# chaeyeongyun/VQ_SEG

Measured on AMD Instinct MI355X. Metric: train images/sec @512x512 vqreptunet1x1 K=512, higher is better.
Workload: dtype bf16; 1 GPU; CPS training iteration (2 x vqreptunet1x1, ResNet-50 encoder, K=[0,0,512,512,512], v1 recipe: 6 forwards + 4 backwards + 2 Adam steps) on 512x512x3 images -- BASELINE configs[2] (the metric's configuration): vqreptunet1x1 512x512, K = 512; labelled_per_gpu=32, unlabelled_per_gpu=32, parallelism=dp1, collectives=none (one process), conv_dtype=bf16

## Files before the change

### include/vqseg.h

```cpp
#ifndef VQSEG_H
#define VQSEG_H

#include <stddef.h>
#include <stdint.h>

#ifdef __cplusplus
extern "C" {
#endif

#define VQSEG_ABI_VERSION 1

#define VQSEG_EINVAL  (-1)
#define VQSEG_ENOSPC  (-2)
#define VQSEG_ENODEV  (-3)

int         vqseg_abi_version(void);
const char* vqseg_last_error(void);
const char* vqseg_kernel_name(const char* entry_point);

int vqseg_set_option(const char* key, int value);

int vqseg_profile_begin(int capacity);
int vqseg_profile_collect(int max_records, int64_t* n_rows_host, int* channels_host,
                          int* n_codes_host, float* ms_host,
                          int* kind_host );

int vqseg_conv_profile_begin(int capacity);
int vqseg_conv_profile_collect(int max_records, double* flops_host, int* kind_host, float* ms_host,
                               int* shape_host );

size_t vqseg_vq_workspace_bytes(int64_t n_rows, int channels, int n_codes);
int vqseg_vq_forward_f32(const float* x, const float* codebook, const void* prepared,
                         int64_t n_rows, int channels, int n_codes, int training,
                         float commitment_weight, float* quant, int64_t* idx, float* loss,
                         float* dead_pct, float* dmin, void* workspace, size_t workspace_bytes,
                         void* stream);

int vqseg_vq_forward_group(int n_levels, int bf16, const void* const* x, const float* const* codebook,
                           const void* const* prepared, const int64_t* n_rows, const int* channels, const int* n_codes,
                           int training, const float* commitment_weight, void* const* quant, int64_t* const* idx,
                           float* const* loss, float* const* dead_pct, void* const* workspace,
                           const size_t* workspace_bytes, void* stream);

size_t vqseg_vq_filter_counter_offset(int64_t n_rows, int channels, int n_codes);

int vqseg_vq_tiles_per_wave(int n_levels, const int64_t* n_rows_host, const int* n_codes_host);

int vqseg_vq_assign_f32(const float* x, const float* codebook, const void* prepared,
                        int64_t n_rows, int channels, int n_codes, int64_t* idx, float* dmin,
                        void* workspace, size_t workspace_bytes, void* stream);
int vqseg_vq_assign_bf16(const void* x, const float* codebook, const void* prepared,
                         int64_t n_rows, int channels, int n_codes, int64_t* idx, float* dmin,
                         void* workspace, size_t workspace_bytes, void* stream);

size_t vqseg_vq_prepared_bytes(int channels, int n_codes);
int vqseg_vq_prepare_f32(const float* codebook, int channels, int n_codes, void* prepared,
                         size_t prepared_bytes, void* stream);

int vqseg_vq_backward_f32(const float* grad_quant, const float* grad_loss, const float* x,
                          const float* quant, int64_t n_rows, int channels,
                          float commitment_weight, float* grad_x, void* stream);

int vqseg_vq_forward_bf16(const void* x, const float* codebook, const void* prepared, int64_t n_rows, int channels,
                          int n_codes, int training, float commitment_weight, void* quant, int64_t* idx, float* loss,
                          float* dead_pct, float* dmin, void* workspace, size_t workspace_bytes, void* stream);
int vqseg_vq_backward_bf16(const void* grad_quant, const float* grad_loss, const void* x, const int64_t* idx,
                           const float* codebook, int64_t n_rows, int channels, float commitment_weight,
                           void* grad_x, void* stream);

size_t vqseg_kmeans_workspace_bytes(int64_t n_rows, int channels, int n_codes);
int vqseg_kmeans_f32(const float* samples, float* means, int64_t* bins, int64_t n_rows,
                     int channels, int n_codes, int iters, void* workspace,
                     size_t workspace_bytes, void* stream);
int vqseg_kmeans_accumulate_f32(const float* samples, const float* means, int64_t n_rows,
                                int channels, int n_codes, float* sums, int64_t* counts,
                                void* workspace, size_t workspace_bytes, void* stream);
int vqseg_kmeans_finalize_f32(const float* sums, const int64_t* counts, float* means,
                              int channels, int n_codes, void* stream);


int vqseg_vq_code_sums(int bf16, const void* x, const int64_t* idx, int64_t n_rows, int channels, int n_codes,
                       float* sums, int64_t* counts, void* workspace, size_t workspace_bytes, void* stream);
int vqseg_vq_ema_update_f32(float* cluster_size, float* embed_avg, float* codebook, const float* sums,
                            const int64_t* counts, int channels, int n_codes, float decay, float eps, float* scratch,
                            void* stream);
int vqseg_vq_revive_candidates(int bf16, const void* x, int64_t n_rows, int channels, int n_codes, uint64_t seed,
                               const int64_t* counter, int rank, int world, float* cand, float* ok, void* stream);
int vqseg_vq_ema_update_revive_f32(float* cluster_size, float* embed_avg, float* codebook, const float* sums,
                                   const int64_t* counts, int channels, int n_codes, float decay, float eps, float* scratch,
                                   const float* cand, const float* ok, float threshold, int64_t* counter, int64_t* revived,
                                   void* stream);


size_t vqseg_conv_packed_elems(int cout, int cin, int kh, int kw, int transpose_flip);
int vqseg_conv_pack_weights_f32(const float* w, int cout, int cin, int kh, int kw, int transpose_flip,
                                void* hi, void* lo, void* stream);

int64_t vqseg_conv_stat_slots(int64_t m_rows, int cout);
int vqseg_conv2d_f(const void* x, const void* x2, int c1, const void* w_hi, const void* w_lo, void* y,
                   float* stat_partial, int n, int h, int w, int cin, int cout, int kh, int kw, int stride,
                   int pad, int reflect, int up, int ho, int wo, int precise, void* stream);

int vqseg_conv2d_affine_f(const void* x, const void* x2, int c1, const void* w_hi, const void* w_lo,
                          const float* scale, const float* shift, const void* res, int relu, void* y,
                          int n, int h, int w, int cin, int cout, int kh, int kw, int stride, int pad, int reflect,
                          int ho, int wo, int precise, void* stream);
int vqseg_conv2d_affine_bits_f(const void* x, const void* w_hi, const float* scale, const float* shift, const void* res,
                               const unsigned char* res_bits, void* y, int n, int h, int w, int cin, int cout, int kh, int kw,
                               int pad, int ho, int wo, void* stream);

size_t vqseg_conv2d_wgrad_workspace_bytes(int n, int h, int w, int cin, int ho, int wo, int cout, int kh, int kw);
int vqseg_conv2d_wgrad_f(const void* gy, const void* x, const void* x2, int c1, int n, int h, int w, int cin,
                         int ho, int wo, int cout, int kh, int kw, int stride, int pad, int reflect, int precise,
                         int cin_out, int im2col, int accumulate, void* workspace, size_t workspace_bytes, float* gw,
                         void* stream);
int vqseg_conv2d_wgrad2_f(const void* gy, const void* x, const void* x2, int n, const void* gy_b, const void* x_b, const void* x2_b,
                          int n_b, int c1, int h, int w, int cin, int ho, int wo, int cout, int kh, int kw, int stride, int pad,
                          int reflect, int precise, int cin_out, int im2col, int accumulate, void* workspace, size_t workspace_bytes,
                          float* gw, void* stream);

int vqseg_bn_sync_ints(int c);
int vqseg_bn_finalize_f(float* partial, int64_t m_rows, int c, const float* gamma, const float* beta,
                        float* run_mean, float* run_var, float momentum, float eps, int training,
                        float* scale, float* shift, float* save_mean, float* save_invstd,
                        int64_t* num_batches_tracked , int* sync, void* stream);
int vqseg_bn_apply_f(int bf16, const void* y, const void* res, const float* scale, const float* shift,
                     int64_t m_rows, int c, int relu, void* out, void* stream);
size_t vqseg_bn_backward_workspace_floats(int64_t m_rows, int c);
int vqseg_bn_backward_f(int bf16, const void* g_out, const void* out, const void* y, const float* mean,
                        const float* invstd, const float* gamma, const float* fwd_scale, const float* fwd_shift,
                        int64_t m_rows, int c, int relu, int training, int accumulate,
                        float* workspace, float* dgamma, float* dbeta, void* g_y, void* g_res, int* sync, void* stream);
int vqseg_bn_apply_bits_f(const void* y, const void* res, const float* scale, const float* shift, int64_t m_rows, int c,
                          void* out, unsigned char* bits, void* stream);
int vqseg_bn_backward_bits_f(const void* g_out, const unsigned char* bits, const void* y, const float* mean,
                             const float* invstd, const float* gamma, int64_t m_rows, int c, int training, int accumulate,
                             float* workspace, float* dgamma, float* dbeta, void* g_y, void* g_res, int* sync, void* stream);

int vqseg_maxpool3x3s2_f(int bf16, int backward, const void* x, const void* g, int n, int h, int w, int c,
                         void* out, unsigned char* idx, void* stream);

int vqseg_bilinear_f(int bf16, int backward, const void* src, int n, int h, int w, int c, int ho, int wo,
                     int align_corners, void* dst, void* stream);

int vqseg_head1x1_forward_f(int bf16, const void* x, const float* w, int64_t m_rows, int cin, int cout,
                            float* y, void* stream);
size_t vqseg_head1x1_backward_workspace_floats(int64_t m_rows, int cin, int cout);
int vqseg_head1x1_backward_f(int bf16, const void* x, const float* w, const float* g, int64_t m_rows, int cin,
                             int cout, void* gx, float* gw, float* workspace, void* stream);
int vqseg_head1x1_backward_add_f(int bf16, const void* x, const float* w, const float* g, int64_t m_rows, int cin,
                                 int cout, void* gx, float* gw, float* workspace, const void* gx_add, void* stream);
int vqseg_maxpool3x3s2_backward_add_f(int bf16, const void* g, const unsigned char* idx, const void* gx_add, int n, int h, int w,
                                      int c, void* gx, void* stream);

int vqseg_im2col_f(int out_bf16, const float* x, int n, int h, int w, int cin, int kh, int kw, int stride,
                   int pad, int reflect, int ho, int wo, int kp, void* out, void* stream);
int vqseg_reflect_fold_f(int bf16, const void* gp, int n, int h, int w, int c, void* gx, void* stream);
int vqseg_stem7_conv_f(int s3, const float* x, const void* w_img, void* y, float* stat_partial, const float* scale, const float* shift, int relu,
                       int n, int h, int w, int reflect, void* stream);
int vqseg_reflect_ring_f(const void* gy, const void* t_hi, void* ring, void* gx, int n, int h, int w, int cgy, int cgx, void* stream);

int vqseg_conv_pack_weights_s3_f32(const float* w, int cout, int cin, int c1, int kh, int kw, void* out, void* stream);

int vqseg_conv_pack_all_f32(const float* w, int cout, int cin, int k, int c1, void* fwd, void* tr, void* s3, void* stream);
size_t vqseg_conv_packed_s2_elems(int cout, int cin, int k);
int vqseg_conv_pack_weights_s2_f32(const float* w, int cout, int cin, int k, void* hi, void* lo, void* stream);
int vqseg_conv2d_dgrad_s2_f(const void* gy, const void* w_hi, const void* w_lo, void* gx, int n, int ho, int wo, int cout, int cin,
                            int k, int oh, int ow, int precise, int accumulate, void* stream);
int64_t vqseg_conv2d_dgrad_s2_fold_rows(int n, int h, int w, int reflect);
int vqseg_conv2d_dgrad_s2_fold_f(const void* gy, const void* w_hi, void* gx, int n, int ho, int wo, int cout, int cin, int h, int w,
                                 int reflect, void* stream);
int vqseg_s3_split_f(const float* x, int64_t rows, int channels, void* y, void* stream);
int vqseg_s3_merge_f(const void* x, int64_t rows, int channels, float* y, void* stream);
int vqseg_s3_maxpool3x3s2_f(const void* x, int n, int h, int w, int c, void* y, void* stream);
int vqseg_s3_bilinear_f(const void* x, int n, int h, int w, int c, int ho, int wo, int align_corners, void* y, void* stream);
int vqseg_cast_f(int to_bf16, const void* x, int64_t n, void* y, void* stream);

size_t vqseg_proto_loss_workspace_bytes(int64_t m_rows, int c, int k);
int vqseg_proto_loss_forward_f(int bf16, const void* x, const float* proto, const int64_t* labels,
                               const unsigned char* keep, const float* conf, int64_t m_rows, int c, int k,
                               int variant, float scale, float margin, int easy_margin,
                               void* workspace, size_t workspace_bytes, double* loss, void* stream);
int vqseg_proto_loss_backward_f(int bf16, const void* x, const float* proto, const int64_t* labels,
                                const unsigned char* keep, const float* conf, int64_t m_rows, int c, int k,
                                int variant, float scale, float margin, int easy_margin, const float* g_loss,
                                void* gx, float* gproto, void* workspace, size_t workspace_bytes, void* stream);

size_t vqseg_dice_workspace_bytes(int b, int c, int64_t hw);
int vqseg_dice_sums_forward_f(const float* logits, int64_t stride_b, int64_t stride_c, int64_t stride_px,
                              const int64_t* target, int b, int c, int64_t hw, int64_t ignore_index,
                              void* workspace, size_t workspace_bytes, float* inter, float* sets, void* stream);
int vqseg_dice_sums_backward_f(const float* logits, int64_t stride_b, int64_t stride_c, int64_t stride_px,
                               const int64_t* target, int b, int c, int64_t hw, int64_t ignore_index,
                               const float* g_inter, const float* g_sets, float* g_logits, void* stream);

int vqseg_dice_ce_sums_forward_f(const float* logits, int64_t stride_b, int64_t stride_c, int64_t stride_px,
                                 const int64_t* target, int b, int c, int64_t hw, int64_t ignore_index,
                                 void* workspace, size_t workspace_bytes, float* inter, float* sets, float* ce,
                                 void* stream);
int vqseg_dice_ce_sums_backward_f(const float* logits, int64_t stride_b, int64_t stride_c, int64_t stride_px,
                                  const int64_t* target, int b, int c, int64_t hw, int64_t ignore_index,
                                  const float* g_inter, const float* g_sets, const float* g_ce, float* g_logits,
                                  void* stream);

int vqseg_softmax_stats_f(const float* logits, int64_t stride_b, int64_t stride_c, int64_t stride_px, int b, int c,
                          int64_t hw, int64_t* label, float* entropy, float* top, void* stream);
// ... 79 lines not shown
```

### vq_seg_amd/_hip.py

```python
from __future__ import annotations

import ctypes
import os
from ctypes import c_char_p, c_double, c_float, c_int, c_int64, c_size_t, c_void_p
from typing import Optional, Tuple

import numpy as np
import torch

_HERE = os.path.dirname(os.path.abspath(__file__))
LIB_PATH = os.environ.get("VQSEG_LIB") or os.path.join(_HERE, "libvqseg_hip.so")

SYMBOLS = {
    "vqseg_abi_version": (c_int, []),
    "vqseg_last_error": (c_char_p, []),
    "vqseg_kernel_name": (c_char_p, [c_char_p]),
    "vqseg_set_option": (c_int, [c_char_p, c_int]),
    "vqseg_profile_begin": (c_int, [c_int]),
    "vqseg_profile_collect": (c_int, [c_int, c_void_p, c_void_p, c_void_p, c_void_p, c_void_p]),
    "vqseg_conv_profile_begin": (c_int, [c_int]),
    "vqseg_conv_profile_collect": (c_int, [c_int, c_void_p, c_void_p, c_void_p, c_void_p]),
    "vqseg_vq_workspace_bytes": (c_size_t, [c_int64, c_int, c_int]),
    "vqseg_vq_filter_counter_offset": (c_size_t, [c_int64, c_int, c_int]),
    "vqseg_vq_tiles_per_wave": (c_int, [c_int, c_void_p, c_void_p]),
    "vqseg_vq_forward_f32": (c_int, [c_void_p, c_void_p, c_void_p, c_int64, c_int, c_int, c_int, c_float, c_void_p,
                                     c_void_p, c_void_p, c_void_p, c_void_p, c_void_p, c_size_t, c_void_p]),
    "vqseg_vq_forward_bf16": (c_int, [c_void_p, c_void_p, c_void_p, c_int64, c_int, c_int, c_int, c_float, c_void_p,
                                      c_void_p, c_void_p, c_void_p, c_void_p, c_void_p, c_size_t, c_void_p]),
    "vqseg_vq_forward_group": (c_int, [c_int, c_int] + [c_void_p] * 6 + [c_int, c_void_p] + [c_void_p] * 6 + [c_void_p]),
    "vqseg_vq_backward_bf16": (c_int, [c_void_p, c_void_p, c_void_p, c_void_p, c_void_p, c_int64, c_int, c_float, c_void_p, c_void_p]),
    "vqseg_vq_assign_f32": (c_int, [c_void_p, c_void_p, c_void_p, c_int64, c_int, c_int, c_void_p, c_void_p, c_void_p,
                                    c_size_t, c_void_p]),
    "vqseg_vq_assign_bf16": (c_int, [c_void_p, c_void_p, c_void_p, c_int64, c_int, c_int, c_void_p, c_void_p, c_void_p,
                                     c_size_t, c_void_p]),
    "vqseg_vq_prepared_bytes": (c_size_t, [c_int, c_int]),
    "vqseg_vq_prepare_f32": (c_int, [c_void_p, c_int, c_int, c_void_p, c_size_t, c_void_p]),
    "vqseg_vq_backward_f32": (c_int, [c_void_p, c_void_p, c_void_p, c_void_p, c_int64, c_int, c_float, c_void_p,
                                      c_void_p]),
    "vqseg_kmeans_workspace_bytes": (c_size_t, [c_int64, c_int, c_int]),
    "vqseg_kmeans_f32": (c_int, [c_void_p, c_void_p, c_void_p, c_int64, c_int, c_int, c_int, c_void_p, c_size_t,
                                 c_void_p]),
    "vqseg_kmeans_accumulate_f32": (c_int, [c_void_p, c_void_p, c_int64, c_int, c_int, c_void_p, c_void_p, c_void_p,
                                            c_size_t, c_void_p]),
    "vqseg_kmeans_finalize_f32": (c_int, [c_void_p, c_void_p, c_void_p, c_int, c_int, c_void_p]),
    "vqseg_vq_code_sums": (c_int, [c_int, c_void_p, c_void_p, c_int64, c_int, c_int, c_void_p, c_void_p, c_void_p, c_size_t, c_void_p]),
    "vqseg_vq_ema_update_f32": (c_int, [c_void_p, c_void_p, c_void_p, c_void_p, c_void_p, c_int, c_int, c_float, c_float, c_void_p,
                                        c_void_p]),
    "vqseg_vq_revive_candidates": (c_int, [c_int, c_void_p, c_int64, c_int, c_int, ctypes.c_uint64, c_void_p, c_int, c_int, c_void_p, c_void_p,
                                           c_void_p]),
    "vqseg_vq_ema_update_revive_f32": (c_int, [c_void_p, c_void_p, c_void_p, c_void_p, c_void_p, c_int, c_int, c_float, c_float, c_void_p,
                                               c_void_p, c_void_p, c_float, c_void_p, c_void_p, c_void_p]),
    "vqseg_conv_packed_elems": (c_size_t, [c_int] * 5),
    "vqseg_conv_pack_weights_f32": (c_int, [c_void_p] + [c_int] * 5 + [c_void_p, c_void_p, c_void_p]),
    "vqseg_conv_stat_slots": (c_int64, [c_int64, c_int]),
    "vqseg_conv2d_f": (c_int, [c_void_p, c_void_p, c_int, c_void_p, c_void_p, c_void_p, c_void_p] + [c_int] * 14 + [c_void_p]),
    "vqseg_conv2d_affine_f": (c_int, [c_void_p, c_void_p, c_int, c_void_p, c_void_p, c_void_p, c_void_p, c_void_p, c_int, c_void_p] +
                              [c_int] * 13 + [c_void_p]),
    "vqseg_conv2d_wgrad_workspace_bytes": (c_size_t, [c_int] * 9),
    "vqseg_conv2d_wgrad_f": (c_int, [c_void_p, c_void_p, c_void_p] + [c_int] * 17 + [c_void_p, c_size_t, c_void_p, c_void_p]),
    "vqseg_conv2d_wgrad2_f": (c_int, [c_void_p, c_void_p, c_void_p, c_int, c_void_p, c_void_p, c_void_p, c_int] + [c_int] * 16 +
                              [c_void_p, c_size_t, c_void_p, c_void_p]),
    "vqseg_bn_sync_ints": (c_int, [c_int]),
    "vqseg_bn_finalize_f": (c_int, [c_void_p, c_int64, c_int, c_void_p, c_void_p, c_void_p, c_void_p, c_float, c_float, c_int,
                                   c_void_p, c_void_p, c_void_p, c_void_p, c_void_p, c_void_p, c_void_p]),
    "vqseg_bn_apply_f": (c_int, [c_int, c_void_p, c_void_p, c_void_p, c_void_p, c_int64, c_int, c_int, c_void_p, c_void_p]),
    "vqseg_bn_backward_workspace_floats": (c_size_t, [c_int64, c_int]),
    "vqseg_bn_backward_f": (c_int, [c_int] + [c_void_p] * 8 + [c_int64, c_int, c_int, c_int, c_int] + [c_void_p] * 7),
    "vqseg_conv2d_affine_bits_f": (c_int, [c_void_p] * 7 + [c_int] * 10 + [c_void_p]),
    "vqseg_bn_apply_bits_f": (c_int, [c_void_p] * 4 + [c_int64, c_int, c_void_p, c_void_p, c_void_p]),
    "vqseg_bn_backward_bits_f": (c_int, [c_void_p] * 6 + [c_int64, c_int, c_int, c_int] + [c_void_p] * 7),
    "vqseg_maxpool3x3s2_f": (c_int, [c_int, c_int, c_void_p, c_void_p, c_int, c_int, c_int, c_int, c_void_p, c_void_p, c_void_p]),
    "vqseg_bilinear_f": (c_int, [c_int, c_int, c_void_p] + [c_int] * 7 + [c_void_p, c_void_p]),
    "vqseg_head1x1_forward_f": (c_int, [c_int, c_void_p, c_void_p, c_int64, c_int, c_int, c_void_p, c_void_p]),
    "vqseg_head1x1_backward_workspace_floats": (c_size_t, [c_int64, c_int, c_int]),
    "vqseg_head1x1_backward_f": (c_int, [c_int, c_void_p, c_void_p, c_void_p, c_int64, c_int, c_int, c_void_p, c_void_p,
                                        c_void_p, c_void_p]),
    "vqseg_proto_loss_workspace_bytes": (c_size_t, [c_int64, c_int, c_int]),
    "vqseg_proto_loss_forward_f": (c_int, [c_int, c_void_p, c_void_p, c_void_p, c_void_p, c_void_p, c_int64, c_int, c_int, c_int,
                                           c_float, c_float, c_int, c_void_p, c_size_t, c_void_p, c_void_p]),
    "vqseg_proto_loss_backward_f": (c_int, [c_int, c_void_p, c_void_p, c_void_p, c_void_p, c_void_p, c_int64, c_int, c_int, c_int,
                                            c_float, c_float, c_int, c_void_p, c_void_p, c_void_p, c_void_p, c_size_t, c_void_p]),
    "vqseg_dice_workspace_bytes": (c_size_t, [c_int, c_int, c_int64]),
    "vqseg_dice_sums_forward_f": (c_int, [c_void_p, c_int64, c_int64, c_int64, c_void_p, c_int, c_int, c_int64, c_int64, c_void_p, c_size_t,
                                          c_void_p, c_void_p, c_void_p]),
    "vqseg_dice_sums_backward_f": (c_int, [c_void_p, c_int64, c_int64, c_int64, c_void_p, c_int, c_int, c_int64, c_int64, c_void_p,
                                           c_void_p, c_void_p, c_void_p]),
    "vqseg_dice_ce_sums_forward_f": (c_int, [c_void_p, c_int64, c_int64, c_int64, c_void_p, c_int, c_int, c_int64, c_int64, c_void_p,
                                             c_size_t, c_void_p, c_void_p, c_void_p, c_void_p]),
    "vqseg_dice_ce_sums_backward_f": (c_int, [c_void_p, c_int64, c_int64, c_int64, c_void_p, c_int, c_int, c_int64, c_int64, c_void_p,
                                              c_void_p, c_void_p, c_void_p, c_void_p]),
    "vqseg_focal_workspace_bytes": (c_size_t, [c_int, c_int64]),
    "vqseg_focal_forward_f": (c_int, [c_void_p, c_int64, c_int64, c_int64, c_void_p, c_int, c_int, c_int64, c_int64, c_void_p, c_float, c_float,
                                      c_int, c_void_p, c_size_t, c_void_p, c_void_p, c_void_p, c_void_p]),
    "vqseg_focal_backward_f": (c_int, [c_void_p, c_int64, c_int64, c_int64, c_void_p, c_int, c_int, c_int64, c_int64, c_void_p, c_float, c_float,
                                       c_int, c_void_p, c_float, c_void_p, c_void_p, c_void_p]),
    "vqseg_wce_sums_forward_f": (c_int, [c_void_p, c_int64, c_int64, c_int64, c_void_p, c_int, c_int, c_int64, c_int64, c_void_p, c_void_p,
                                         c_size_t, c_void_p, c_void_p]),
    "vqseg_wce_sums_backward_f": (c_int, [c_void_p, c_int64, c_int64, c_int64, c_void_p, c_int, c_int, c_int64, c_int64, c_void_p, c_void_p,
                                          c_void_p, c_void_p]),
    "vqseg_class_weight_f": (c_int, [c_void_p, c_int64, c_int, c_void_p, c_void_p, c_void_p]),
    "vqseg_softmax_stats_f": (c_int, [c_void_p, c_int64, c_int64, c_int64, c_int, c_int, c_int64, c_void_p, c_void_p, c_void_p, c_void_p]),
    "vqseg_confusion_counts_f": (c_int, [c_void_p, c_int64, c_int64, c_int64, c_void_p, c_int, c_int, c_int64, c_void_p, c_void_p]),
    "vqseg_order_stats_workspace_bytes": (c_size_t, []),
    "vqseg_order_stats_f": (c_int, [c_void_p, c_int64, c_int64, c_void_p, c_size_t, c_void_p, c_void_p]),
    "vqseg_im2col_f": (c_int, [c_int, c_void_p] + [c_int] * 12 + [c_void_p, c_void_p]),
    "vqseg_reflect_fold_f": (c_int, [c_int, c_void_p, c_int, c_int, c_int, c_int, c_void_p, c_void_p]),
    "vqseg_reflect_ring_f": (c_int, [c_void_p, c_void_p, c_void_p, c_void_p, c_int, c_int, c_int, c_int, c_int, c_void_p]),
    "vqseg_cast_f": (c_int, [c_int, c_void_p, c_int64, c_void_p, c_void_p]),
    "vqseg_conv_pack_all_f32": (c_int, [c_void_p, c_int, c_int, c_int, c_int, c_void_p, c_void_p, c_void_p, c_void_p]),
    "vqseg_conv_packed_s2_elems": (c_size_t, [c_int, c_int, c_int]),
    "vqseg_conv_pack_weights_s2_f32": (c_int, [c_void_p, c_int, c_int, c_int, c_void_p, c_void_p, c_void_p]),
    "vqseg_conv2d_dgrad_s2_f": (c_int, [c_void_p, c_void_p, c_void_p, c_void_p] + [c_int] * 10 + [c_void_p]),
    "vqseg_stem7_conv_f": (c_int, [c_int, c_void_p, c_void_p, c_void_p, c_void_p, c_void_p, c_void_p] + [c_int] * 5 + [c_void_p]),
    "vqseg_conv2d_dgrad_s2_fold_rows": (ctypes.c_int64, [c_int] * 4),
    "vqseg_cps_loss_combine_f": (c_int, [c_int, c_int, c_int, c_void_p, c_void_p, c_void_p, c_void_p, c_float, c_float, c_float, c_void_p, c_int, c_int,
                                         c_float, c_void_p, c_int, c_float, c_void_p, c_void_p, c_void_p, c_void_p, c_void_p]),
    "vqseg_conv2d_dgrad_s2_fold_f": (c_int, [c_void_p, c_void_p, c_void_p] + [c_int] * 8 + [c_void_p]),
    "vqseg_head1x1_backward_add_f": (c_int, [c_int, c_void_p, c_void_p, c_void_p, c_int64, c_int, c_int, c_void_p, c_void_p,
                                            c_void_p, c_void_p, c_void_p]),
    "vqseg_maxpool3x3s2_backward_add_f": (c_int, [c_int, c_void_p, c_void_p, c_void_p, c_int, c_int, c_int, c_int, c_void_p, c_void_p]),
    "vqseg_conv_pack_weights_s3_f32": (c_int, [c_void_p] + [c_int] * 5 + [c_void_p, c_void_p]),
    "vqseg_s3_split_f": (c_int, [c_void_p, c_int64, c_int, c_void_p, c_void_p]),
    "vqseg_s3_merge_f": (c_int, [c_void_p, c_int64, c_int, c_void_p, c_void_p]),
    "vqseg_s3_maxpool3x3s2_f": (c_int, [c_void_p, c_int, c_int, c_int, c_int, c_void_p, c_void_p]),
    "vqseg_s3_bilinear_f": (c_int, [c_void_p] + [c_int] * 7 + [c_void_p, c_void_p]),
    "vqseg_adam_work_items": (c_int64, [c_int64, c_int, c_int, c_int]),
    "vqseg_adam_step_f32": (c_int, [c_void_p, c_void_p, c_int, c_double, c_double, c_double, c_double, c_int64, c_void_p]),
    "vqseg_adam_ema_step_f32": (c_int, [c_void_p, c_void_p, c_void_p, c_int, c_double, c_double, c_double, c_double, c_int64, c_double, c_int,
                                        c_void_p]),
    "vqseg_batch_u8_f": (c_int, [c_int, c_void_p, c_void_p, c_void_p, c_void_p] + [c_int] * 4 + [c_void_p] * 6),
    "vqseg_box_mix_f": (c_int, [c_int, c_int, c_void_p, c_void_p] + [c_int] * 4 + [c_int64] * 3 + [c_void_p, ctypes.c_uint64, c_void_p]),
    "vqseg_affine_warp_f": (c_int, [c_int, c_int, c_void_p, c_void_p] + [c_int] * 4 + [c_int64] * 4 + [c_void_p, ctypes.c_uint64, c_void_p]),
    "vqseg_resize_argmax_f": (c_int, [c_void_p, c_void_p, c_int] + [c_int64] * 3 + [c_int] * 6 + [c_void_p] * 5),
}

_lib: Optional[ctypes.CDLL] = None


class HipLibraryError(RuntimeError):
    pass


def _bind_symbols(handle: ctypes.CDLL) -> ctypes.CDLL:
    for name, (res, args) in SYMBOLS.items():
        fn = getattr(handle, name)
        fn.restype, fn.argtypes = res, args
    return handle


def lib() -> ctypes.CDLL:
    global _lib
    if _lib is None:
        if not os.path.exists(LIB_PATH):
            raise HipLibraryError(
                f"{LIB_PATH} not found: build it with `python -c 'import __graft_entry__ as g; g.build()'` "
                f"(or `make -C vq_seg_amd/csrc`). There is no CPU fallback.")
        handle = _bind_symbols(ctypes.CDLL(LIB_PATH))
        if handle.vqseg_abi_version() != 1:
            raise HipLibraryError("libvqseg_hip.so ABI version mismatch")
        for kv in filter(None, os.environ.get("VQSEG_OPTS", "").split(",")):
            key, _, val = kv.partition("=")
            if key.strip().startswith("py_"):
                PY_OPTS[key.strip()] = int(val)
                continue
            if handle.vqseg_set_option(key.strip().encode(), int(val)) < 0:
                raise HipLibraryError(f"VQSEG_OPTS: unknown option {key!r}")
        _lib = handle
    return _lib


PY_OPTS: dict = {}
FILTER_DIAG = None


_BF_DTYPE = {0: torch.float32, 1: torch.bfloat16, 2: torch.bfloat16}


def tptr(t, name: str, dtype=None, numel: Optional[int] = None, bf: Optional[int] = None, at_least: bool = False, dense: bool = True):
    if t is None:
        return None
    if bf is not None:
        dtype = _BF_DTYPE[bf]
    try:
        if (dtype is None or t.dtype is dtype or (type(dtype) is tuple and t.dtype in dtype)) and t.is_cuda and \
                (numel is None or (t.numel() >= numel if at_least else t.numel() == numel)) and \
                (not dense or t.is_contiguous() or (t.dim() == 4 and t.is_contiguous(memory_format=torch.channels_last))):
            return t.data_ptr()
    except AttributeError:
        pass
    return _tptr_report(t, name, dtype, numel, at_least, dense)


def _tptr_report(t, name, dtype, numel, at_least, dense):
    def bad(msg):
        return HipLibraryError(f"{name}: {msg}")
    if not isinstance(t, torch.Tensor):
        raise bad(f"expected a tensor, got {type(t).__name__}")
    if dtype is not None and (t.dtype not in dtype if isinstance(dtype, tuple) else t.dtype != dtype):
        if dense:
            raise bad(f"expected {dtype}, got {t.dtype}")
        names = " or ".join(str(d).removeprefix("torch.") for d in (dtype if isinstance(dtype, tuple) else (dtype,)))
        raise bad(f"expected a {names} tensor, got {t.dtype}")
    if dense and not t.is_contiguous() and not (t.dim() == 4 and t.is_contiguous(memory_format=torch.channels_last)):
        raise bad(f"expected a dense (contiguous) tensor, got strides {tuple(t.stride())} for shape {tuple(t.shape)}")
    if numel is not None and (t.numel() < numel if at_least else t.numel() != numel):
        raise bad(f"the sizes passed along need {'at least ' if at_least else ''}{numel} elements, the tensor has {t.numel()} (shape {tuple(t.shape)})")
    if not t.is_cuda:
        return _NotOnGpu(f"{name}: the HIP path needs a tensor on a 'cuda' (ROCm) device; got {t.device}. There is no CPU fallback.")
    return t.data_ptr()


class _NotOnGpu:
    __slots__ = ("msg",)

    def __init__(self, msg: str):
        self.msg = msg

    def __add__(self, _offset):
        return self


def on_gpu(ptr):
    if type(ptr) is _NotOnGpu:
        raise HipLibraryError(ptr.msg)
    return ptr


def _dev(t: torch.Tensor, dtype: torch.dtype, name: str, numel: Optional[int] = None):
    if t is None:
        raise HipLibraryError(f"{name}: expected a tensor, got None")
    return tptr(t, name, dtype=dtype, numel=numel)


def _stream() -> int:
    return torch.cuda.current_stream().cuda_stream


def _failed(L, name: str, rc: int) -> HipLibraryError:
    return HipLibraryError(f"{name} failed (code {rc}): {L.vqseg_last_error().decode(errors='replace')}")


def launch(name: str, dev, *args, handle=None) -> None:
    L = handle or lib()
    if type(dev) is not torch.device:
        dev = torch.device(dev)
    if dev.type == "cuda":
        try:
            with torch.cuda.device(dev):
                rc = getattr(L, name)(*args, _stream())
        except ctypes.ArgumentError:
            for a in args:
                on_gpu(a)
            raise
        if rc != 0:
            raise _failed(L, name, rc)
        return
    for a in args:
        on_gpu(a)
    raise HipLibraryError(f"{name}: the HIP path needs tensors on a 'cuda' (ROCm) device; got {dev}. There is no CPU fallback.")


def _workspace(nbytes: int, device) -> torch.Tensor:
    return torch.empty(int(nbytes), dtype=torch.uint8, device=device)


def vq_prepare(codebook: torch.Tensor) -> torch.Tensor:
    L = lib()
    k, c = codebook.shape
    wp = _dev(codebook, torch.float32, "codebook")
    nbytes = L.vqseg_vq_prepared_bytes(c, k)
    blob = _workspace(nbytes, codebook.device)
    launch("vqseg_vq_prepare_f32", codebook.device, wp, c, k, blob.data_ptr(), nbytes)
    return blob


def vq_forward(rows: torch.Tensor, codebook: torch.Tensor, training: bool, commitment_weight: float,
               want_dmin: bool = False, prepared: Optional[torch.Tensor] = None):
    L = lib()
    n, c = rows.shape
    k = codebook.shape[0]
    bf16 = rows.dtype == torch.bfloat16
    xp, wp = tptr(rows, "rows", bf=int(bf16), numel=n * c), _dev(codebook, torch.float32, "codebook", k * c)
    dev = rows.device
    quant = torch.empty_like(rows)
    idx = torch.empty(n, dtype=torch.int64, device=dev)
    scal = torch.empty(2, dtype=torch.float32, device=dev)
    dmin = torch.empty(n, dtype=torch.float32, device=dev) if want_dmin else None
    nbytes = L.vqseg_vq_workspace_bytes(n, c, k)
    ws = _workspace(nbytes, dev)
    launch("vqseg_vq_forward_bf16" if bf16 else "vqseg_vq_forward_f32", dev, xp, wp,
           tptr(prepared, "prepared codebook", dtype=torch.uint8, numel=L.vqseg_vq_prepared_bytes(c, k)), n, c, k,
           int(bool(training)), float(commitment_weight), quant.data_ptr(), idx.data_ptr(), scal.data_ptr(), scal.data_ptr() + 4,
           dmin.data_ptr() if want_dmin else None, ws.data_ptr(), nbytes)
    out = (quant, idx, scal[0:1], scal[1])
    return out + (dmin,) if want_dmin else out


def bind(path: str) -> ctypes.CDLL:
    return _bind_symbols(ctypes.CDLL(path))


def vq_forward_group(rows_list, codebooks, prepared_list, training: bool, commitment_weights, handle=None):
    L = handle or lib()
    nl = len(rows_list)
    bf16 = rows_list[0].dtype == torch.bfloat16
    dev = rows_list[0].device
    ptr = lambda ps: (c_void_p * nl)(*map(on_gpu, ps))
    ns = np.array([r.shape[0] for r in rows_list], dtype=np.int64)
    cs = np.array([r.shape[1] for r in rows_list], dtype=np.int32)
    ks = np.array([w.shape[0] for w in codebooks], dtype=np.int32)
    cw = np.array([float(w) for w in commitment_weights], dtype=np.float32)
    xs, wps, preps, quants, idxs, scals, wss = [], [], [], [], [], [], []
    for r, w in zip(rows_list, codebooks):
        if r.dtype != rows_list[0].dtype:
            raise HipLibraryError("vq_forward_group: one row type per call")
        xs.append(tptr(r, "rows", bf=int(bf16)))
        wps.append(_dev(w, torch.float32, "codebook", w.shape[0] * r.shape[1]))
        quants.append(torch.empty_like(r))
        idxs.append(torch.empty(r.shape[0], dtype=torch.int64, device=dev))
        scals.append(torch.empty(2, dtype=torch.float32, device=dev))
        wss.append(_workspace(L.vqseg_vq_workspace_bytes(r.shape[0], r.shape[1], w.shape[0]), dev))
    for w, p_ in zip(codebooks, prepared_list):
        preps.append(tptr(p_, "prepared codebook", dtype=torch.uint8, numel=L.vqseg_vq_prepared_bytes(w.shape[1], w.shape[0])))
    wsb = (c_size_t * nl)(*[w.numel() for w in wss])
    launch("vqseg_vq_forward_group", dev, nl, int(bf16), ptr(xs), ptr(wps), ptr(preps), ns.ctypes.data, cs.ctypes.data, ks.ctypes.data,
           int(bool(training)), cw.ctypes.data, ptr(q.data_ptr() for q in quants), ptr(i.data_ptr() for i in idxs),
           ptr(s.data_ptr() for s in scals), ptr(s.data_ptr() + 4 for s in scals), ptr(w.data_ptr() for w in wss),
           ctypes.cast(wsb, c_void_p), handle=handle)
    if FILTER_DIAG is not None and bf16:
        for r, w, ws_ in zip(rows_list, codebooks, wss):
            off = L.vqseg_vq_filter_counter_offset(r.shape[0], r.shape[1], w.shape[0])
            FILTER_DIAG.append((r.shape[0], r.shape[1], w.shape[0], ws_[off:off + 256].view(torch.int32) if off else None))
    return [(q, i, s[0:1], s[1]) for q, i, s in zip(quants, idxs, scals)]


def set_option(key: str, value: int) -> int:
    prev = lib().vqseg_set_option(key.encode(), int(value))
    if prev < 0:
        raise HipLibraryError(f"vqseg_set_option: unknown option {key!r} or bad value {value}")
    return prev


def vq_tiles_per_wave(n_rows, n_codes) -> int:
    rows = [n_rows] if isinstance(n_rows, int) else list(n_rows)
    codes = [n_codes] if isinstance(n_codes, int) else list(n_codes)
    if len(rows) != len(codes):
        raise ValueError("vq_tiles_per_wave: one code count per row count")
    t = lib().vqseg_vq_tiles_per_wave(len(rows), (ctypes.c_int64 * len(rows))(*rows), (c_int * len(codes))(*codes))
    if t < 0:
        raise _failed(lib(), "vqseg_vq_tiles_per_wave", t)
    return t


def vq_assign(rows: torch.Tensor, codebook: torch.Tensor, want_dmin: bool = False,
              prepared: Optional[torch.Tensor] = None, want_filter_count: bool = False):
    L = lib()
    n, c = rows.shape
    k = codebook.shape[0]
    bf16 = rows.dtype == torch.bfloat16
    xp, wp = tptr(rows, "rows", bf=int(bf16), numel=n * c), _dev(codebook, torch.float32, "codebook", k * c)
    dev = rows.device
    idx = torch.empty(n, dtype=torch.int64, device=dev)
    dmin = torch.empty(n, dtype=torch.float32, device=dev) if want_dmin else None
    nbytes = L.vqseg_vq_workspace_bytes(n, c, k)
    ws = _workspace(nbytes, dev)
    launch("vqseg_vq_assign_bf16" if bf16 else "vqseg_vq_assign_f32", dev, xp, wp,
           tptr(prepared, "prepared codebook", dtype=torch.uint8, numel=L.vqseg_vq_prepared_bytes(c, k)), n, c, k,
           idx.data_ptr(), dmin.data_ptr() if want_dmin else None, ws.data_ptr(), nbytes)
    if want_filter_count:
        off = L.vqseg_vq_filter_counter_offset(n, c, k) if bf16 else 0
        amb = ws[off:off + 256].view(torch.int32).sum() if off else None
        return (idx, dmin, amb) if want_dmin else (idx, amb)
    return (idx, dmin) if want_dmin else idx


def vq_backward(grad_quant: torch.Tensor, grad_loss: Optional[torch.Tensor], rows: torch.Tensor, quant: torch.Tensor,
                commitment_weight: float) -> torch.Tensor:
    n, c = rows.shape
    gq = _dev(grad_quant, torch.float32, "grad_quant", n * c)
    gl = _dev(grad_loss, torch.float32, "grad_loss", 1) if grad_loss is not None else None
    gx = torch.empty_like(rows)
    launch("vqseg_vq_backward_f32", rows.device, gq, gl, _dev(rows, torch.float32, "rows", n * c), _dev(quant, torch.float32, "quant", n * c),
           n, c, float(commitment_weight), gx.data_ptr())
    return gx


def vq_backward_bf16(grad_quant: torch.Tensor, grad_loss: Optional[torch.Tensor], rows: torch.Tensor, idx: torch.Tensor,
                     codebook: torch.Tensor, commitment_weight: float) -> torch.Tensor:
    n, c = rows.shape
    gq = _dev(grad_quant, torch.bfloat16, "grad_quant", n * c)
    gl = _dev(grad_loss, torch.float32, "grad_loss", 1) if grad_loss is not None else None
    gx = torch.empty_like(rows)
    if codebook.dim() != 2 or codebook.shape[1] != c:
        raise HipLibraryError(f"codebook: expected (K, {c}), got {tuple(codebook.shape)}")
    launch("vqseg_vq_backward_bf16", rows.device, gq, gl, _dev(rows, torch.bfloat16, "rows", n * c), _dev(idx, torch.int64, "idx", n),
           _dev(codebook, torch.float32, "codebook"), n, c, float(commitment_weight), gx.data_ptr())
    return gx


def kmeans(samples: torch.Tensor, means: torch.Tensor, iters: int) -> Tuple[torch.Tensor, torch.Tensor]:
    L = lib()
    n, c = samples.shape
    k = means.shape[0]
    sp, mp = _dev(samples, torch.float32, "samples", n * c), _dev(means, torch.float32, "means", k * c)
    bins = torch.zeros(k, dtype=torch.int64, device=samples.device)
    nbytes = L.vqseg_kmeans_workspace_bytes(n, c, k)
    ws = _workspace(nbytes, samples.device)
    launch("vqseg_kmeans_f32", samples.device, sp, mp, bins.data_ptr(), n, c, k, int(iters), ws.data_ptr(), nbytes)
    return means, bins


def kmeans_accumulate(samples: torch.Tensor, means: torch.Tensor) -> Tuple[torch.Tensor, torch.Tensor]:
    L = lib()
    n, c = samples.shape
    k = means.shape[0]
    sp, mp = _dev(samples, torch.float32, "samples", n * c), _dev(means, torch.float32, "means", k * c)
    sums = torch.empty(k, c, dtype=torch.float32, device=samples.device)
    counts = torch.empty(k, dtype=torch.int64, device=samples.device)
    nbytes = L.vqseg_kmeans_workspace_bytes(n, c, k)
    ws = _workspace(nbytes, samples.device)
    launch("vqseg_kmeans_accumulate_f32", samples.device, sp, mp, n, c, k, sums.data_ptr(), counts.data_ptr(), ws.data_ptr(), nbytes)
    return sums, counts


def kmeans_finalize(sums: torch.Tensor, counts: torch.Tensor, means: torch.Tensor) -> torch.Tensor:
    k, c = means.shape
    launch("vqseg_kmeans_finalize_f32", means.device, _dev(sums, torch.float32, "sums", k * c), _dev(counts, torch.int64, "counts", k),
           _dev(means, torch.float32, "means", k * c), c, k)
    return means


def vq_code_sums(rows: torch.Tensor, idx: torch.Tensor, k: int, out: Optional[torch.Tensor] = None) -> Tuple[torch.Tensor, torch.Tensor]:
    L = lib()
    n, c = rows.shape
    if rows.dtype not in (torch.float32, torch.bfloat16):
        raise HipLibraryError(f"rows: expected torch.float32 or torch.bfloat16, got {rows.dtype}")
    ip = _dev(idx, torch.int64, "idx", n)
    sums = torch.empty(k, c, dtype=torch.float32, device=rows.device) if out is None else out
    counts = torch.empty(k, dtype=torch.int64, device=rows.device)
    nbytes = L.vqseg_kmeans_workspace_bytes(n, c, k)
    ws = _workspace(nbytes, rows.device)
    bf = int(rows.dtype == torch.bfloat16)
    launch("vqseg_vq_code_sums", rows.device, bf, tptr(rows, "rows", bf=bf, numel=n * c), ip, n, c, k,
           sums.data_ptr() if out is None else _dev(out, torch.float32, "out", k * c), counts.data_ptr(), ws.data_ptr(), nbytes)
    return sums, counts


def vq_revive_candidates(rows: torch.Tensor, seed: int, counter: torch.Tensor, k: int, rank: int, world: int, out=None):
    n, c = rows.shape
    if rows.dtype not in (torch.float32, torch.bfloat16):
        raise HipLibraryError(f"rows: expected torch.float32 or torch.bfloat16, got {rows.dtype}")
    bf = int(rows.dtype == torch.bfloat16)
    xp, tp = tptr(rows, "rows", bf=bf, numel=n * c), _dev(counter, torch.int64, "counter", 1)
    if out is None:
        out = (torch.empty(k, c, dtype=torch.float32, device=rows.device), torch.empty(k, dtype=torch.float32, device=rows.device))
    cand, ok = out
    launch("vqseg_vq_revive_candidates", rows.device, bf, xp, n, c, k, int(seed) & 0xFFFFFFFFFFFFFFFF, tp, int(rank), int(world),
           _dev(cand, torch.float32, "candidates", k * c), _dev(ok, torch.float32, "ok", k))
    return cand, ok


def vq_ema_update(cluster_size: torch.Tensor, embed_avg: torch.Tensor, codebook: torch.Tensor, sums: torch.Tensor,
                  counts: torch.Tensor, decay: float, eps: float, candidates: Optional[torch.Tensor] = None,
                  ok: Optional[torch.Tensor] = None, threshold: float = 0.0, counter: Optional[torch.Tensor] = None,
                  revived: Optional[torch.Tensor] = None) -> None:
    k, c = codebook.shape
    if cluster_size.shape != (k,) or embed_avg.shape != (k, c) or sums.shape != (k, c) or counts.shape != (k,):
        raise ValueError("vq_ema_update: shapes must be (K,), (K, C), (K, C), (K, C), (K,)")
    if threshold == 0:
        scratch = torch.empty(1, dtype=torch.float32, device=codebook.device)
        launch("vqseg_vq_ema_update_f32", codebook.device, _dev(cluster_size, torch.float32, "cluster_size"),
               _dev(embed_avg, torch.float32, "embed_avg"), _dev(codebook, torch.float32, "codebook"), _dev(sums, torch.float32, "sums"),
               _dev(counts, torch.int64, "counts"), c, k, float(decay), float(eps), scratch.data_ptr())
        return
    scratch = torch.empty(1 + k, dtype=torch.float32, device=codebook.device)
    launch("vqseg_vq_ema_update_revive_f32", codebook.device, _dev(cluster_size, torch.float32, "cluster_size"),
           _dev(embed_avg, torch.float32, "embed_avg"), _dev(codebook, torch.float32, "codebook"), _dev(sums, torch.float32, "sums"),
           _dev(counts, torch.int64, "counts"), c, k, float(decay), float(eps), scratch.data_ptr(),
           _dev(candidates, torch.float32, "candidates", k * c), _dev(ok, torch.float32, "ok", k), float(threshold),
           _dev(counter, torch.int64, "counter", 1), _dev(revived, torch.int64, "revived", 1))


def batch_u8(img_cache: torch.Tensor, img_offsets, hw: Tuple[int, int], f32_lut: torch.Tensor, img_out: torch.Tensor,
             mask_cache: Optional[torch.Tensor] = None, mask_offsets=None, mask_hw: Tuple[int, int] = (0, 0),
             label_lut: Optional[torch.Tensor] = None, target_out: Optional[torch.Tensor] = None,
             label_out: Optional[torch.Tensor] = None) -> None:
    n = len(img_offsets)
    (h, w), (mh, mw) = hw, mask_hw
    io = np.ascontiguousarray(img_offsets, dtype=np.int64)
    mo = np.ascontiguousarray(mask_offsets, dtype=np.int64) if mask_offsets is not None else None
    if n and (int(io.min()) < 0 or int(io.max()) + h * w * 3 > img_cache.numel()):
        raise HipLibraryError("batch_u8: an image offset lies outside the image cache")
    if mask_cache is not None:
        if mo is None or len(mo) != n:
            raise HipLibraryError("batch_u8: one mask offset per sample required")
        if n and (int(mo.min()) < 0 or int(mo.max()) + mh * mw > mask_cache.numel()):
            raise HipLibraryError("batch_u8: a mask offset lies outside the mask cache")
    if img_out.dim() != 4 or not img_out.is_contiguous(memory_format=torch.channels_last):
        raise HipLibraryError("batch_u8: img_out must be a channels_last (n, 3, h, w) tensor")
    launch("vqseg_batch_u8_f", img_out.device, n, tptr(img_cache, "img_cache", dtype=torch.uint8), tptr(mask_cache, "mask_cache", dtype=torch.uint8),
           io.ctypes.data, mo.ctypes.data if mo is not None else None, h, w, mh, mw,
           tptr(f32_lut, "f32_lut", dtype=torch.float32, numel=256), tptr(label_lut, "label_lut", dtype=torch.int64, numel=256),
           tptr(img_out, "img_out", dtype=torch.float32, numel=n * 3 * h * w),
           tptr(target_out, "target_out", dtype=torch.uint8, numel=n * mh * mw),
           tptr(label_out, "label_out", dtype=torch.int64, numel=n * mh * mw))


BOX_MIX_DTYPES = (torch.uint8, torch.bfloat16, torch.float32, torch.int64)
BOX_MIX_CALLS = 0


def box_mix(src: torch.Tensor, boxes, mode: str = "mix", fill=0, out: Optional[torch.Tensor] = None) -> torch.Tensor:
    global BOX_MIX_CALLS
    if mode not in ("mix", "fill"):
        raise HipLibraryError(f"box_mix: mode must be 'mix' or 'fill', got {mode!r}")
    if not isinstance(src, torch.Tensor) or src.dim() not in (3, 4):
        raise HipLibraryError("box_mix: src must be a (n, P, h, w) or (n, h, w) tensor")
    n, (h, w) = src.shape[0], src.shape[-2:]
    planes = src.shape[1] if src.dim() == 4 else 1
    bx = np.ascontiguousarray(boxes, dtype=np.int32)
    if bx.shape != (n, 4):
        raise HipLibraryError(f"box_mix: one (y1, x1, cut_h, cut_w) box per sample required: {n} samples, boxes of shape {bx.shape}")
    if n and (int(bx.min()) < 0 or int((bx[:, 0] + bx[:, 2]).max()) > h or int((bx[:, 1] + bx[:, 3]).max()) > w):
        raise HipLibraryError(f"box_mix: a box lies outside the {h} x {w} image")
    if out is None:
# ... 105 lines not shown
```

### vq_seg_amd/csrc/vq_assign.hip

```cpp
#include <hip/hip_runtime.h>
#include <stdint.h>

#include "vq_internal.h"

namespace vqseg {

constexpr int ROWS_PER_WAVE = 32;
constexpr int WAVES = 4;
static_assert(ROWS_PER_WG == ROWS_PER_WAVE * WAVES, "the host's workgroup count (vq_internal.h) is this kernel's row tile");
#ifndef VQ_TIMELINE
#define VQ_TIMELINE 0
#endif
struct VqGroup {
    VqLevel lv[VQ_MAX_LEVELS];
    int n;
#if VQ_TIMELINE
    unsigned long long* tl;
#endif
};
#ifndef VQ_BIG_STAGE
#define VQ_BIG_STAGE 0
#endif
#ifndef VQ_SHAPE16
#define VQ_SHAPE16 0
#endif
constexpr int stage_floats(int T) { return (VQ_BIG_STAGE && T >= 4) ? 8192 : 4096; }

__device__ __forceinline__ void glds16(const float* g, float* lds_wave_base) {
    __builtin_amdgcn_global_load_lds((const __attribute__((address_space(1))) void*)g,
                                     (__attribute__((address_space(3))) void*)lds_wave_base, 16, 0, 0);
}

template <typename TX> struct RawFrag { typedef f32x4 type; };
template <> struct RawFrag<__bf16> { typedef u32x2 type; };

#if VQ_TIMELINE
#define TL_STAMP(k_)                                                          \
    if (g.tl && threadIdx.x == 0) {                                           \
        tl_rt[k_] = __builtin_amdgcn_s_memrealtime();                         \
        tl_ck[k_] = __builtin_amdgcn_s_memtime();                             \
    }
#else
#define TL_STAMP(k_)
#endif

template <int T, typename TX = float>
__global__ __launch_bounds__(256, 2) void vq_assign_f32_kernel(const VqGroup g) {
#if VQ_TIMELINE
    unsigned long long tl_rt[6] = {0, 0, 0, 0, 0, 0}, tl_ck[6] = {0, 0, 0, 0, 0, 0};
    TL_STAMP(0)
#endif
    int lvl = 0;
    while (lvl + 1 < g.n && blockIdx.x >= g.lv[lvl].wg_end) ++lvl;
    const unsigned bid = blockIdx.x - (lvl ? g.lv[lvl - 1].wg_end : 0u);
    const TX* __restrict__ x = static_cast<const TX*>(g.lv[lvl].x);
    const float* __restrict__ E4 = g.lv[lvl].E4;
    const float* __restrict__ enorm = g.lv[lvl].enorm;
    unsigned long long* __restrict__ keys = g.lv[lvl].keys;
    if (g.lv[lvl].gate && *g.lv[lvl].gate <= g.lv[lvl].gate_cap) return;
    const long N = g.lv[lvl].N;
    const int C = g.lv[lvl].C, Cp = g.lv[lvl].C, Kp = g.lv[lvl].Kp;
    constexpr int CODES = 32 * T;
    constexpr int STAGE_FLOATS = stage_floats(T);
    constexpr int BK = STAGE_FLOATS / (32 * T);
    constexpr int JB = BK / 8;
    extern __shared__ __attribute__((aligned(16))) char smem[];
    float* Bs = reinterpret_cast<float*>(smem);
    float* xn_s = Bs + 2 * STAGE_FLOATS + 256;

    const int tid = threadIdx.x;
    const int lane = tid & 63;
    const int wave = __builtin_amdgcn_readfirstlane(tid >> 6);
    const int r = lane & 31, h = lane >> 5;
    const int n_stage = (Cp + BK - 1) / BK;
    const int chunks = Kp / CODES;
    const unsigned within = bid % (8u * chunks);
    const long row_tile = (long)(bid / (8u * chunks)) * 8 + (within & 7u);
    if (row_tile * ROWS_PER_WG >= N) return;
    const int code0 = (int)(within >> 3) * CODES;
    const long row0 = row_tile * ROWS_PER_WG + wave * ROWS_PER_WAVE;
    long row = row0 + r;
    if (row > N - 1) row = N - 1;
    const TX* xrow = x + row * (long)C + 4 * h;

    f32x16 acc[T];
#pragma unroll
    for (int t = 0; t < T; ++t)
#pragma unroll
        for (int i = 0; i < 16; ++i) acc[t][i] = 0.0f;
    float xn_part = 0.0f;

    auto fill = [&](int stage, int buf) {
        float* dst = Bs + buf * STAGE_FLOATS;
#pragma unroll
        for (int q = 0; q < STAGE_FLOATS / 1024; ++q) {
            const int piece = wave * (STAGE_FLOATS / 1024) + q;
            const int fl = piece * 256 + lane * 4;
            const int c4 = fl / (CODES * 4);
            const int code = (fl % (CODES * 4)) >> 2;
            int slab = stage * (BK / 4) + c4;
            if (slab > Cp / 4 - 1) slab = Cp / 4 - 1;
            const float* src = E4 + ((size_t)slab * Kp + code0 + code) * 4;
            glds16(src, dst + piece * 256);
        }
    };
    using RawA = typename RawFrag<TX>::type;
    auto load_a = [&](int stage, RawA (&a)[JB]) {
#pragma unroll
        for (int j = 0; j < JB; ++j) {
            const int col = stage * BK + 8 * j + 4 * h;
            if (col >= C) {
                a[j] = RawA{};
            } else {
                a[j] = *reinterpret_cast<const RawA*>(xrow + stage * BK + 8 * j);
            }
        }
    };

    f32x4 a_cur[JB];
    RawA a_nxt[JB];
    fill(0, 0);
    if (n_stage > 1) fill(1, 1);
    auto widen_a = [&](f32x4 (&dst)[JB], const RawA (&src)[JB]) {
#pragma unroll
        for (int j = 0; j < JB; ++j) {
            if constexpr (sizeof(TX) == 4) {
                dst[j] = src[j];
            } else {
                const unsigned lo = src[j][0], hi = src[j][1];
                dst[j] = f32x4{__builtin_bit_cast(float, lo << 16), __builtin_bit_cast(float, lo & 0xFFFF0000u),
                               __builtin_bit_cast(float, hi << 16), __builtin_bit_cast(float, hi & 0xFFFF0000u)};
            }
        }
    };
    load_a(0, a_nxt);
    widen_a(a_cur, a_nxt);
#pragma unroll
    for (int j = 0; j < JB; ++j) a_nxt[j] = RawA{};
    __syncthreads();
    TL_STAMP(1)

    const float* bs_lane = Bs + (h * CODES + r) * 4;
    f32x4 b_cur[T], b_nxt[T];
#pragma unroll
    for (int t = 0; t < T; ++t) b_cur[t] = *reinterpret_cast<const f32x4*>(bs_lane + t * 128);

    auto mfma_block = [&](int j) {
#pragma unroll
        for (int e = 0; e < 4; ++e) {
            const float a = a_cur[j][e];
            xn_part = __builtin_fmaf(a, a, xn_part);
#if VQ_SHAPE16
#pragma unroll
            for (int t = 0; t < T; ++t) {
                f32x4 q0 = {acc[t][0], acc[t][1], acc[t][2], acc[t][3]}, q1 = {acc[t][8], acc[t][9], acc[t][10], acc[t][11]};
                q0 = __builtin_amdgcn_mfma_f32_16x16x4f32(a, b_cur[t][e], q0, 0, 0, 0);
                q1 = __builtin_amdgcn_mfma_f32_16x16x4f32(a, b_cur[t][e], q1, 0, 0, 0);
                acc[t][0] = q0[0], acc[t][1] = q0[1], acc[t][2] = q0[2], acc[t][3] = q0[3];
                acc[t][8] = q1[0], acc[t][9] = q1[1], acc[t][10] = q1[2], acc[t][11] = q1[3];
            }
#else
#pragma unroll
            for (int t = 0; t < T; ++t) acc[t] = __builtin_amdgcn_mfma_f32_32x32x2f32(a, b_cur[t][e], acc[t], 0, 0, 0);
#endif
        }
#pragma unroll
        for (int t = 0; t < T; ++t) {
            __builtin_amdgcn_sched_group_barrier(0x008, 4, 0);
            __builtin_amdgcn_sched_group_barrier(0x100, 1, 0);
        }
    };

    for (int s = 0; s < n_stage; ++s) {
        const float* bsrc = bs_lane + (s & 1) * STAGE_FLOATS;
        if (s + 1 < n_stage) load_a(s + 1, a_nxt);
#pragma unroll
        for (int j = 0; j < JB - 1; ++j) {
#pragma unroll
            for (int t = 0; t < T; ++t)
                b_nxt[t] = *reinterpret_cast<const f32x4*>(bsrc + (2 * (j + 1)) * CODES * 4 + t * 128);
            mfma_block(j);
#pragma unroll
            for (int t = 0; t < T; ++t) b_cur[t] = b_nxt[t];
        }
        __syncthreads();
        if (s + 2 < n_stage) fill(s + 2, s & 1);
        if (s + 1 < n_stage) {
            const float* bnext = bs_lane + ((s + 1) & 1) * STAGE_FLOATS;
#pragma unroll
            for (int t = 0; t < T; ++t) b_nxt[t] = *reinterpret_cast<const f32x4*>(bnext + t * 128);
        }
        mfma_block(JB - 1);
#pragma unroll
        for (int t = 0; t < T; ++t) b_cur[t] = b_nxt[t];
        widen_a(a_cur, a_nxt);
    }

    float en[T];
#pragma unroll
    for (int t = 0; t < T; ++t) en[t] = enorm[code0 + t * 32 + r];
    float floor_t[T];
#pragma unroll
    for (int t = 0; t < T; ++t) floor_t[t] = code0 + t * 32 + r < g.lv[lvl].K ? 0.0f : __builtin_inff();
    TL_STAMP(2)
    {
        const float xn = xn_part + __shfl_xor(xn_part, 32);
        if (h == 0) xn_s[wave * 32 + r] = xn;
    }
    __builtin_amdgcn_s_waitcnt(0xc07f);
    __builtin_amdgcn_wave_barrier();
    float xnr[16];
#pragma unroll
    for (int g = 0; g < 4; ++g) {
        const f32x4 v = *reinterpret_cast<const f32x4*>(xn_s + wave * 32 + 8 * g + 4 * h);
#pragma unroll
        for (int e = 0; e < 4; ++e) xnr[4 * g + e] = v[e];
    }
    float best2[16];
    int best_i[16];
    const int code_r = code0 + r;
#pragma unroll
    for (int i = 0; i < 16; ++i) {
        float b2 = __builtin_inff(), thr = __builtin_inff();
        int bi = code_r;
        bool band = false;
#pragma unroll
        for (int t = 0; t < T; ++t) {
            float d2 = __builtin_fmaf(-2.0f, acc[t][i], xnr[i]);
            d2 = d2 + en[t];
            d2 = __builtin_fmaxf(d2, floor_t[t]);
            const bool clear = d2 < thr;
            band = band || (!clear && d2 < b2);
            bi = clear ? code_r + 32 * t : bi;
            b2 = clear ? d2 : b2;
            thr = clear ? d2 * 0.99999905f : thr;
        }
        if (__builtin_expect(__any(band), 0)) {
            b2 = __builtin_inff();
            thr = __builtin_inff();
            bi = code_r;
#pragma unroll
            for (int t = 0; t < T; ++t) {
                float d2 = __builtin_fmaf(-2.0f, acc[t][i], xnr[i]);
                d2 = d2 + en[t];
                d2 = __builtin_fmaxf(d2, floor_t[t]);
                const bool clear = d2 < thr;
                const bool near = !clear && d2 < b2;
                if (near) {
                    const bool better = __builtin_sqrtf(d2) < __builtin_sqrtf(b2);
                    bi = better ? code_r + 32 * t : bi;
                    b2 = d2;
                    thr = d2 * 0.99999905f;
                }
                bi = clear ? code_r + 32 * t : bi;
                b2 = clear ? d2 : b2;
                thr = clear ? d2 * 0.99999905f : thr;
            }
        }
        best2[i] = b2;
        best_i[i] = bi;
    }
    TL_STAMP(3)
    unsigned long long* ks = reinterpret_cast<unsigned long long*>(Bs) + wave * (32 * 33);
#pragma unroll
    for (int i = 0; i < 16; ++i) {
        const unsigned long long key =
            ((unsigned long long)__float_as_uint(__builtin_sqrtf(best2[i])) << 32) | (unsigned int)best_i[i];
        ks[(h * 16 + i) * 33 + r] = key;
    }
    __builtin_amdgcn_s_waitcnt(0xc07f);
    __builtin_amdgcn_wave_barrier();
    {
        const int rw = lane >> 1, part = lane & 1;
        unsigned long long m = ~0ull;
#pragma unroll
        for (int j = 0; j < 16; ++j) {
            const unsigned long long v = ks[rw * 33 + part * 16 + j];
            m = v < m ? v : m;
        }
        const unsigned long long o = __shfl_xor(m, 1);
        m = o < m ? o : m;
        const int hh = rw >> 4, ii = rw & 15;
        const long orow = row0 + (ii & 3) + 8 * (ii >> 2) + 4 * hh;
        TL_STAMP(4)
        if (part == 0 && orow < N) atomicMin(keys + orow, m);
    }
#if VQ_TIMELINE
    TL_STAMP(5)
    if (g.tl && threadIdx.x == 0) {
        unsigned long long* o = g.tl + (size_t)blockIdx.x * 16;
#pragma unroll
        for (int k = 0; k < 6; ++k) {
            o[2 * k] = tl_rt[k];
            o[2 * k + 1] = tl_ck[k];
        }
        o[12] = __builtin_amdgcn_s_getreg((31 << 11) | 4);
        o[13] = __builtin_amdgcn_s_getreg((31 << 11) | 20);
        o[14] = (unsigned long long)lvl;
        o[15] = (unsigned long long)row_tile;
    }
#endif
}

#if VQ_TIMELINE
static unsigned long long* g_timeline = nullptr;
#endif

template <int T, typename TX>
static void launch_assign_t(const VqGroup& g, hipStream_t st) {
    constexpr int STAGE_FLOATS = stage_floats(T);
    static_assert((size_t)WAVES * 32 * 33 * sizeof(unsigned long long) <= (2 * STAGE_FLOATS + 256) * sizeof(float), "key scratch aliases the B stages");
    const size_t lds = (size_t)(2 * STAGE_FLOATS + 256 + WAVES * 32) * sizeof(float);
    hipLaunchKernelGGL((vq_assign_f32_kernel<T, TX>), dim3(g.lv[g.n - 1].wg_end), dim3(256), lds, st, g);
}

void launch_assign_levels(const VqLevel* lv, int n, int T, int x_bf16, hipStream_t st) {
    VqGroup g;
    g.n = n;
    for (int q = 0; q < n; ++q) g.lv[q] = lv[q];
#if VQ_TIMELINE
    g.tl = g_timeline;
#endif
#define VQ_ASSIGN(T_)                                                 \
    if (x_bf16) launch_assign_t<T_, __bf16>(g, st);                   \
    else launch_assign_t<T_, float>(g, st)
    switch (T) {
        case 8: VQ_ASSIGN(8); break;
        case 4: VQ_ASSIGN(4); break;
        case 2: VQ_ASSIGN(2); break;
        default: VQ_ASSIGN(1); break;
    }
#undef VQ_ASSIGN
}

}

#if VQ_TIMELINE
extern "C" int vqseg_debug_timeline(void* buf) {
    vqseg::g_timeline = static_cast<unsigned long long*>(buf);
    return 0;
}
#endif
```

### vq_seg_amd/csrc/vq_filter.hip

```cpp
#include <hip/hip_runtime.h>
#include <math.h>
#include <stdint.h>

#include "vq_internal.h"

namespace vqseg {

typedef __bf16 bf16x8 __attribute__((ext_vector_type(8)));
constexpr int F_BK = 32;
constexpr int F_STAGE_BYTES = 2 * (F_BK / 8) * F_CODES * 16;

__device__ __forceinline__ void glds16b(const void* g, void* lds_wave_base) {
    __builtin_amdgcn_global_load_lds((const __attribute__((address_space(1))) void*)g, (__attribute__((address_space(3))) void*)lds_wave_base,
                                     16, 0, 0);
}

__device__ __forceinline__ int wave_excl_scan(int v, int& total) {
    int inc = v;
#pragma unroll
    for (int d = 1; d < 64; d <<= 1) {
        const int o = __shfl_up(inc, d);
        if ((int)(threadIdx.x & 63) >= d) inc += o;
    }
    total = __shfl(inc, 63);
    return inc - v;
}

struct FilterConsts {
    float c_s, c_r;
};

__global__ __launch_bounds__(256, 2) void vq_filter_bf16_kernel(const VqFilterGroup g, const FilterConsts fc0, const FilterConsts fc1,
                                                                const FilterConsts fc2, const FilterConsts fc3) {
    int lvl = 0;
    while (lvl + 1 < g.n && blockIdx.x >= g.lv[lvl].wg_end) ++lvl;
    const unsigned bid = blockIdx.x - (lvl ? g.lv[lvl - 1].wg_end : 0u);
    const FilterConsts fc = lvl == 0 ? fc0 : (lvl == 1 ? fc1 : (lvl == 2 ? fc2 : fc3));
    const unsigned short* __restrict__ x = static_cast<const unsigned short*>(g.lv[lvl].x);
    const unsigned short* __restrict__ Eb = g.lv[lvl].Eb;
    const long N = g.lv[lvl].N;
    const int C = g.lv[lvl].C, Kp = g.lv[lvl].Kp;
    extern __shared__ __attribute__((aligned(16))) char fsm[];
    char* Bs = fsm;
    float* en_s = reinterpret_cast<float*>(fsm + 2 * F_STAGE_BYTES);

    const int tid = threadIdx.x, lane = tid & 63;
    const int wave = __builtin_amdgcn_readfirstlane(tid >> 6);
    const int wp = wave & 1, wc = wave >> 1;
    const int r = lane & 31, h = lane >> 5;
    const int n_stage = C / F_BK;
    const int chunks = Kp / F_CODES;
    const unsigned within = bid % (8u * chunks);
    const long row_tile = (long)(bid / (8u * chunks)) * 8 + (within & 7u);
    if (row_tile * F_ROWS >= N) return;
    const int chunk = (int)(within >> 3);
    const int code0 = chunk * F_CODES;

    en_s[tid] = g.lv[lvl].enorm[code0 + tid];

    const unsigned short* xrow[2];
#pragma unroll
    for (int p = 0; p < 2; ++p) {
        long row = row_tile * F_ROWS + wp * 64 + p * 32 + r;
        if (row > N - 1) row = N - 1;
        xrow[p] = x + row * (long)C + 8 * h;
    }

    f32x16 acc[2][4];
#pragma unroll
    for (int p = 0; p < 2; ++p)
#pragma unroll
        for (int t = 0; t < 4; ++t)
#pragma unroll
            for (int i = 0; i < 16; ++i) acc[p][t][i] = 0.0f;
    float xn_part[2] = {0.0f, 0.0f};

    auto fill = [&](int stage, int buf) {
        char* dst = Bs + buf * F_STAGE_BYTES;
#pragma unroll
        for (int q = 0; q < 8; ++q) {
            const int piece = wave * 8 + q;
            const int hlslab = piece >> 2, quarter = piece & 3;
            const int hl = hlslab >> 2, slab = hlslab & 3;
            const unsigned short* src = Eb + (((size_t)hl * (C / 8) + (size_t)stage * 4 + slab) * Kp + code0 + quarter * 64 + lane) * 8;
            glds16b(src, dst + (hlslab * F_CODES + quarter * 64) * 16);
        }
    };
    auto load_x = [&](int stage, u32x4 (&xf)[2][2]) {
#pragma unroll
        for (int p = 0; p < 2; ++p)
#pragma unroll
            for (int q = 0; q < 2; ++q) xf[p][q] = *reinterpret_cast<const u32x4*>(xrow[p] + stage * F_BK + q * 16);
    };

    u32x4 xcur[2][2], xnxt[2][2];
    fill(0, 0);
    if (n_stage > 1) fill(1, 1);
    load_x(0, xcur);
#pragma unroll
    for (int p = 0; p < 2; ++p)
#pragma unroll
        for (int q = 0; q < 2; ++q) xnxt[p][q] = u32x4{0u, 0u, 0u, 0u};
    __syncthreads();

    const char* a_lane = Bs + ((h * F_CODES) + wc * 128 + r) * 16;
    for (int s = 0; s < n_stage; ++s) {
        const char* abase = a_lane + (s & 1) * F_STAGE_BYTES;
        if (s + 1 < n_stage) load_x(s + 1, xnxt);
#pragma unroll
        for (int q = 0; q < 2; ++q) {
            bf16x8 ah[4], al[4];
#pragma unroll
            for (int t = 0; t < 4; ++t) {
                ah[t] = *reinterpret_cast<const bf16x8*>(abase + ((0 * 4 + 2 * q) * F_CODES + 32 * t) * 16);
                al[t] = *reinterpret_cast<const bf16x8*>(abase + ((1 * 4 + 2 * q) * F_CODES + 32 * t) * 16);
            }
#pragma unroll
            for (int p = 0; p < 2; ++p) {
                const bf16x8 xb = __builtin_bit_cast(bf16x8, xcur[p][q]);
#pragma unroll
                for (int e = 0; e < 4; ++e) {
                    const float lo = __builtin_bit_cast(float, xcur[p][q][e] << 16), hi = __builtin_bit_cast(float, xcur[p][q][e] & 0xFFFF0000u);
                    xn_part[p] = __builtin_fmaf(lo, lo, xn_part[p]);
                    xn_part[p] = __builtin_fmaf(hi, hi, xn_part[p]);
                }
#pragma unroll
                for (int t = 0; t < 4; ++t) {
                    acc[p][t] = __builtin_amdgcn_mfma_f32_32x32x16_bf16(ah[t], xb, acc[p][t], 0, 0, 0);
                    acc[p][t] = __builtin_amdgcn_mfma_f32_32x32x16_bf16(al[t], xb, acc[p][t], 0, 0, 0);
                }
            }
        }
        __syncthreads();
        if (s + 2 < n_stage) fill(s + 2, s & 1);
#pragma unroll
        for (int p = 0; p < 2; ++p)
#pragma unroll
            for (int q = 0; q < 2; ++q) xcur[p][q] = xnxt[p][q];
    }

    const float en_max = *g.lv[lvl].en_max;
    const int sub = chunk * 2 + wc, n_sub = Kp / F_SUB;
    const float* en_l = en_s + wc * 128 + 4 * h;
#pragma unroll
    for (int p = 0; p < 2; ++p) {
        float m = __builtin_inff();
        int bi = 0;
#pragma unroll
        for (int t = 0; t < 4; ++t)
#pragma unroll
            for (int gq = 0; gq < 4; ++gq) {
                const f32x4 en4 = *reinterpret_cast<const f32x4*>(en_l + 32 * t + 8 * gq);
#pragma unroll
                for (int e = 0; e < 4; ++e) {
                    const float sc = __builtin_fmaf(-2.0f, acc[p][t][4 * gq + e], en4[e]);
                    acc[p][t][4 * gq + e] = sc;
                    const bool better = sc < m;
                    bi = better ? 32 * t + 8 * gq + e : bi;
                    m = better ? sc : m;
                }
            }
        bi += 4 * h;
        {
            const float mo = __shfl_xor(m, 32);
            const int bo = __shfl_xor(bi, 32);
            const bool take = mo < m || (mo == m && bo < bi);
            m = take ? mo : m;
            bi = take ? bo : bi;
        }
        const float xn = xn_part[p] + __shfl_xor(xn_part[p], 32);
        const float band = __builtin_fmaf(fc.c_s, __builtin_sqrtf(xn * en_max), fc.c_r * (xn + en_max));
        const float thr = m + band;
        unsigned lo = 0u, hi = 0u;
#pragma unroll
        for (int t = 0; t < 2; ++t)
#pragma unroll
            for (int i = 0; i < 16; ++i) lo |= acc[p][t][i] <= thr ? (1u << (16 * t + i)) : 0u;
#pragma unroll
        for (int t = 2; t < 4; ++t)
#pragma unroll
            for (int i = 0; i < 16; ++i) hi |= acc[p][t][i] <= thr ? (1u << (16 * (t - 2) + i)) : 0u;
        const int mine = __popc(lo) + __popc(hi);
        const int cnt = mine + __shfl_xor(mine, 32);
        const long row = row_tile * F_ROWS + wp * 64 + p * 32 + r;
        const bool live = row < N;
        if (h == 0 && live) {
            const unsigned hiw = (unsigned)(code0 + wc * 128 + bi) | ((unsigned)(cnt > 0xffff ? 0xffff : cnt) << 16);
            g.lv[lvl].summary[row * n_sub + sub] = ((unsigned long long)hiw << 32) | __float_as_uint(m);
            if (sub == 0) g.lv[lvl].brow[row] = band;
        }
        if ((bi & 4) == 4 * h) {
            const int bb = 16 * (bi >> 5) + 4 * ((bi >> 3) & 3) + (bi & 3);
            if (bb < 32) lo &= ~(1u << bb);
            else hi &= ~(1u << (bb - 32));
        }
        const int extra = live ? __popc(lo) + __popc(hi) : 0;
        if (__any(extra > 0)) {
            int total;
            const int before = wave_excl_scan(extra, total);
            const int list = blockIdx.x & (F_LISTS - 1), cap = g.lv[lvl].pair_cap;
            int base = 0;
            if (lane == 0) {
                base = atomicAdd(g.lv[lvl].pair_count + list, total);
                if (base + total > cap) g.lv[lvl].pair_count[F_LISTS] = 1;
            }
            base = __shfl(base, 0);
            if (extra > 0) {
                int slot = base + before;
                unsigned long long* out = g.lv[lvl].pair_rc + (size_t)list * cap;
                unsigned long long bits = ((unsigned long long)hi << 32) | lo;
                while (bits) {
                    const int b = __ffsll((long long)bits) - 1;
                    bits &= bits - 1;
                    const int cl = 32 * (b >> 4) + 8 * ((b >> 2) & 3) + 4 * h + (b & 3);
                    if (slot < cap) out[slot] = ((unsigned long long)row << 32) | (unsigned)(code0 + wc * 128 + cl);
                    ++slot;
                }
            }
        }
    }
}

constexpr int F_MAX_SUB = 16;
__global__ __launch_bounds__(256) void vq_resolve_kernel(const VqFilterGroup g, int force_all) {
    int lvl = 0;
    while (lvl + 1 < g.n && blockIdx.x >= g.lv[lvl].rblk_end) ++lvl;
    const VqFilterLevel& L = g.lv[lvl];
    const long N = L.N;
    const int n_sub = L.Kp / F_SUB;
    long row = (long)(blockIdx.x - (lvl ? g.lv[lvl - 1].rblk_end : 0u)) * 256 + threadIdx.x;
    const bool valid = row < N;
    if (!valid) row = N - 1;
    const unsigned long long* sm = L.summary + row * n_sub;
    unsigned long long v[F_MAX_SUB];
#pragma unroll
    for (int j = 0; j < F_MAX_SUB; j += 2)
        if (j < n_sub) {
            const u32x4 w = *reinterpret_cast<const u32x4*>(sm + j);
            v[j] = ((unsigned long long)w[1] << 32) | w[0];
            v[j + 1] = ((unsigned long long)w[3] << 32) | w[2];
        }
    float m = __builtin_inff();
    unsigned best = 0;
#pragma unroll
    for (int j = 0; j < F_MAX_SUB; ++j)
        if (j < n_sub) {
            const float mj = __uint_as_float((unsigned)(v[j] & 0xffffffffull));
            const unsigned cj = (unsigned)(v[j] >> 32) & 0xffffu;
            if (mj < m || (mj == m && cj < best)) m = mj, best = cj;
        }
    for (int j = F_MAX_SUB; j < n_sub; ++j) {
        const float mj = __uint_as_float((unsigned)(sm[j] & 0xffffffffull));
        const unsigned cj = (unsigned)(sm[j] >> 32) & 0xffffu;
        if (mj < m || (mj == m && cj < best)) m = mj, best = cj;
    }
    const float thr = m + L.brow[row];
    unsigned cnt = 0;
    int alive = 0;
#pragma unroll
    for (int j = 0; j < F_MAX_SUB; ++j)
        if (j < n_sub && __uint_as_float((unsigned)(v[j] & 0xffffffffull)) <= thr) cnt += (unsigned)(v[j] >> 48), ++alive;
    for (int j = F_MAX_SUB; j < n_sub; ++j)
        if (__uint_as_float((unsigned)(sm[j] & 0xffffffffull)) <= thr) cnt += (unsigned)(sm[j] >> 48), ++alive;
    const bool bad = valid && !(__builtin_fabsf(thr) < __builtin_inff());
    if (__any(bad) && (threadIdx.x & 63) == 0) L.pair_count[F_LISTS] = 1;
    const bool open = valid && (bad || !(cnt == 1 && !force_all));
    if (valid) {
        if (!open) L.keys[row] = (unsigned long long)best;
        L.brow[row] = open ? thr : -__builtin_inff();
    }
    if (!__any(open)) return;
    int total;
    const int before = wave_excl_scan(open ? alive : 0, total);
    const int list = blockIdx.x & (F_LISTS - 1), cap = L.pair_cap;
    int base = 0;
    if ((threadIdx.x & 63) == 0) {
        base = atomicAdd(L.pair_count + list, total);
        if (base + total > cap) L.pair_count[F_LISTS] = 1;
    }
    base = __shfl(base, 0);
    if (open) {
        int slot = base + before;
        unsigned long long* out = L.pair_rc + (size_t)list * cap;
        for (int j = 0; j < n_sub; ++j) {
            const unsigned long long vj = sm[j];
            if (__uint_as_float((unsigned)(vj & 0xffffffffull)) <= thr) {
                if (slot < cap) out[slot] = ((unsigned long long)row << 32) | ((unsigned)(vj >> 32) & 0xffffu);
                ++slot;
            }
        }
    }
}

struct RescoreTrip {
    u32x4 xw[4];
    f32x4 e0[4], e1[4];
};

template <bool ROWMAJOR>
__device__ __forceinline__ void rescore_load(RescoreTrip& t, const unsigned short* xr, const float* er, int c, int Kp) {
#pragma unroll
    for (int u = 0; u < 4; ++u) {
        t.xw[u] = *reinterpret_cast<const u32x4*>(xr + c + 8 * u);
        if (ROWMAJOR) {
            t.e0[u] = *reinterpret_cast<const f32x4*>(er + c + 8 * u);
            t.e1[u] = *reinterpret_cast<const f32x4*>(er + c + 8 * u + 4);
        } else {
            t.e0[u] = *reinterpret_cast<const f32x4*>(er + (size_t)((c + 8 * u) / 4) * Kp * 4);
            t.e1[u] = *reinterpret_cast<const f32x4*>(er + (size_t)((c + 8 * u) / 4 + 1) * Kp * 4);
        }
    }
}

__device__ __forceinline__ void rescore_fma(const RescoreTrip& t, float& dot, float& xa, float& xb) {
#pragma unroll
    for (int u = 0; u < 4; ++u) {
        const float xv[8] = {__builtin_bit_cast(float, t.xw[u][0] << 16), __builtin_bit_cast(float, t.xw[u][0] & 0xFFFF0000u),
                             __builtin_bit_cast(float, t.xw[u][1] << 16), __builtin_bit_cast(float, t.xw[u][1] & 0xFFFF0000u),
                             __builtin_bit_cast(float, t.xw[u][2] << 16), __builtin_bit_cast(float, t.xw[u][2] & 0xFFFF0000u),
                             __builtin_bit_cast(float, t.xw[u][3] << 16), __builtin_bit_cast(float, t.xw[u][3] & 0xFFFF0000u)};
#pragma unroll
        for (int e = 0; e < 4; ++e) {
            dot = __builtin_fmaf(xv[e], t.e0[u][e], dot);
            dot = __builtin_fmaf(xv[4 + e], t.e1[u][e], dot);
            xa = __builtin_fmaf(xv[e], xv[e], xa);
            xb = __builtin_fmaf(xv[4 + e], xv[4 + e], xb);
        }
    }
}

template <bool ROWMAJOR>
__device__ __forceinline__ void rescore_pairs(const VqFilterLevel& L, int list, int tid, int nthreads) {
    int n = L.pair_count[list];
    if (n > L.pair_cap) n = L.pair_cap;
    const int C = L.C, Kp = L.Kp;
    const unsigned short* __restrict__ x = static_cast<const unsigned short*>(L.x);
    const unsigned long long* pairs = L.pair_rc + (size_t)list * L.pair_cap;
    for (int i = tid; i < n; i += nthreads) {
        const unsigned long long rc = pairs[i];
        const long row = (long)(rc >> 32);
        const unsigned k = (unsigned)(rc & 0xffffffffull);
        if (L.brow[row] == -__builtin_inff()) continue;
        const unsigned short* xr = x + row * (long)C;
        const float* er = ROWMAJOR ? L.W + (size_t)k * C : L.E4 + (size_t)k * 4;
        float dot = 0.0f, xa = 0.0f, xb = 0.0f;
        RescoreTrip t0, t1, t2;
        rescore_load<ROWMAJOR>(t0, xr, er, 0, Kp);
        if (C > 32) rescore_load<ROWMAJOR>(t1, xr, er, 32, Kp);
        int c = 0;
        for (; c + 96 <= C; c += 96) {
            if (c + 64 < C) rescore_load<ROWMAJOR>(t2, xr, er, c + 64, Kp);
            rescore_fma(t0, dot, xa, xb);
            if (c + 96 < C) rescore_load<ROWMAJOR>(t0, xr, er, c + 96, Kp);
            rescore_fma(t1, dot, xa, xb);
            if (c + 128 < C) rescore_load<ROWMAJOR>(t1, xr, er, c + 128, Kp);
            rescore_fma(t2, dot, xa, xb);
        }
        if (c < C) {
            rescore_fma(t0, dot, xa, xb);
            if (c + 32 < C) rescore_fma(t1, dot, xa, xb);
        }
        float d2 = __builtin_fmaf(-2.0f, dot, xa + xb) + L.enorm[k];
        d2 = __builtin_fmaxf(d2, 0.0f);
        atomicMin(L.keys + row, ((unsigned long long)__float_as_uint(__builtin_sqrtf(d2)) << 32) | k);
    }
}

__global__ __launch_bounds__(256) void vq_rescore_kernel(const VqFilterGroup g) {
    int lvl = 0;
    while (lvl + 1 < g.n && blockIdx.x >= g.lv[lvl].sblk_end) ++lvl;
    const unsigned first = lvl ? g.lv[lvl - 1].sblk_end : 0u;
    const unsigned b = blockIdx.x - first, per_list = (g.lv[lvl].sblk_end - first) / F_LISTS;
    const int list = (int)(b % F_LISTS), tid = (int)(b / F_LISTS) * 256 + threadIdx.x, nthreads = (int)per_list * 256;
    if (g.lv[lvl].W) rescore_pairs<true>(g.lv[lvl], list, tid, nthreads);
    else rescore_pairs<false>(g.lv[lvl], list, tid, nthreads);
}

__global__ __launch_bounds__(256) void vq_exact_dist_kernel(const unsigned short* __restrict__ x, const float* __restrict__ E4, int Kp,
                                                            const float* __restrict__ enorm, const long long* __restrict__ idx, long N, int C,
                                                            float* __restrict__ dmin) {
    const long row = (long)blockIdx.x * 256 + threadIdx.x;
    if (row >= N) return;
    const unsigned short* xr = x + row * (long)C;
    const long long k = idx[row];
    float dot = 0.0f, xa = 0.0f, xb = 0.0f;
    for (int c = 0; c + 8 <= C; c += 8) {
        float xv[8];
#pragma unroll
        for (int e = 0; e < 8; ++e) xv[e] = __builtin_bit_cast(float, (unsigned)xr[c + e] << 16);
        const f32x4 e0 = *reinterpret_cast<const f32x4*>(E4 + ((size_t)(c / 4) * Kp + k) * 4);
        const f32x4 e1 = *reinterpret_cast<const f32x4*>(E4 + ((size_t)(c / 4 + 1) * Kp + k) * 4);
#pragma unroll
        for (int e = 0; e < 4; ++e) {
            dot = __builtin_fmaf(xv[e], e0[e], dot);
            dot = __builtin_fmaf(xv[4 + e], e1[e], dot);
            xa = __builtin_fmaf(xv[e], xv[e], xa);
            xb = __builtin_fmaf(xv[4 + e], xv[4 + e], xb);
        }
    }
    float d2 = __builtin_fmaf(-2.0f, dot, xa + xb) + enorm[k];
    d2 = __builtin_fmaxf(d2, 0.0f);
    dmin[row] = __builtin_sqrtf(d2);
}

__global__ __launch_bounds__(256) void vq_pack_codebook_bf16(const float* __restrict__ W, int K, int C, int Kp, unsigned short* __restrict__ Eb) {
    const long total = (long)(C / 8) * Kp;
    const size_t half = (size_t)C * Kp;
    for (long i = (long)blockIdx.x * 256 + threadIdx.x; i < total; i += (long)gridDim.x * 256) {
        const int k = (int)(i % Kp);
        const int c = (int)(i / Kp) * 8;
        u32x4 hi = {0u, 0u, 0u, 0u}, lo = {0u, 0u, 0u, 0u};
        if (k < K) {
            const f32x4 v0 = *reinterpret_cast<const f32x4*>(W + (size_t)k * C + c), v1 = *reinterpret_cast<const f32x4*>(W + (size_t)k * C + c + 4);
            const float v[8] = {v0[0], v0[1], v0[2], v0[3], v1[0], v1[1], v1[2], v1[3]};
#pragma unroll
            for (int e = 0; e < 4; ++e) {
                const __bf16 h0 = (__bf16)v[2 * e], h1 = (__bf16)v[2 * e + 1];
                const __bf16 l0 = (__bf16)(v[2 * e] - (float)h0), l1 = (__bf16)(v[2 * e + 1] - (float)h1);
                hi[e] = (unsigned)__builtin_bit_cast(unsigned short, h0) | ((unsigned)__builtin_bit_cast(unsigned short, h1) << 16);
                lo[e] = (unsigned)__builtin_bit_cast(unsigned short, l0) | ((unsigned)__builtin_bit_cast(unsigned short, l1) << 16);
            }
        }
        *reinterpret_cast<u32x4*>(Eb + (size_t)i * 8) = hi;
        *reinterpret_cast<u32x4*>(Eb + half + (size_t)i * 8) = lo;
    }
}

__device__ __forceinline__ float max_keep_nan(float a, float b) { return a != a ? a : (!(b <= a) ? b : a); }

__global__ __launch_bounds__(256) void vq_enorm_max(const float* __restrict__ enorm, int K, float* __restrict__ out) {
    __shared__ float sh[256];
    float m = 0.0f;
    for (int k = threadIdx.x; k < K; k += 256) m = max_keep_nan(m, enorm[k]);
    sh[threadIdx.x] = m;
    __syncthreads();
    for (int w = 128; w > 0; w >>= 1) {
        if ((int)threadIdx.x < w) sh[threadIdx.x] = max_keep_nan(sh[threadIdx.x], sh[threadIdx.x + w]);
        __syncthreads();
    }
    if (threadIdx.x == 0) out[0] = sh[0];
}

void launch_prepare_filter(const float* W, int K, int C, int Kp, const float* enorm, unsigned short* Eb, float* en_max, hipStream_t st) {
    long b2 = ((long)(C / 8) * Kp + 255) / 256;
    if (b2 > 4096) b2 = 4096;
    hipLaunchKernelGGL(vq_pack_codebook_bf16, dim3((unsigned)b2), dim3(256), 0, st, W, K, C, Kp, Eb);
    hipLaunchKernelGGL(vq_enorm_max, dim3(1), dim3(256), 0, st, enorm, K, en_max);
}

void launch_filter(const VqFilterGroup& fg, int force_all, hipStream_t st) {
    FilterConsts fc[VQ_MAX_LEVELS] = {};
    for (int q = 0; q < fg.n; ++q) {
        const double u = ldexp(1.0, -24), cc = (double)fg.lv[q].C;
        const double per_s = 2.0 * (cc * u + ldexp(1.0, -18) + (cc / 8.0) * 17.0 * u);
        const double tail = 2.0 * ldexp(1.0, -22) + ldexp(1.0, -20);
        fc[q].c_s = (float)(1.25 * (2.0 * per_s + 2.0 * tail));
        fc[q].c_r = (float)(1.25 * tail);
    }
    const VqFilterLevel& last = fg.lv[fg.n - 1];
    hipLaunchKernelGGL(vq_filter_bf16_kernel, dim3(last.wg_end), dim3(256), (size_t)(2 * F_STAGE_BYTES + F_CODES * sizeof(float)), st, fg, fc[0],
                       fc[1], fc[2], fc[3]);
    hipLaunchKernelGGL(vq_resolve_kernel, dim3(last.rblk_end), dim3(256), 0, st, fg, force_all);
    hipLaunchKernelGGL(vq_rescore_kernel, dim3(last.sblk_end), dim3(256), 0, st, fg);
}

void launch_exact_dist(const void* x, const float* E4, int Kp, const float* enorm, const int64_t* idx, int64_t N, int C, float* dmin,
                       hipStream_t st) {
    hipLaunchKernelGGL(vq_exact_dist_kernel, dim3((unsigned)((N + 255) / 256)), dim3(256), 0, st, static_cast<const unsigned short*>(x), E4, Kp,
                       enorm, reinterpret_cast<const long long*>(idx), (long)N, C, dmin);
}

}
```

### vq_seg_amd/csrc/vq_host.hip

```cpp
#include <hip/hip_runtime.h>
#include <stdint.h>

#include <vector>

#include "options.h"
#include "vq_internal.h"

namespace vqseg {

static inline int round_up(int v, int m) { return (v + m - 1) / m * m; }

static inline size_t up256(size_t v) { return (v + 255) & ~(size_t)255; }

static bool filter_shape_ok(int C, int K) { return K % 256 == 0 && C % 32 == 0 && K <= 65536; }

PreparedLayout prepared_layout(int C, int K) {
    const int Kp = round_up(K, 32);
    PreparedLayout l;
    l.off_e4 = 0;
    l.off_enorm = (size_t)C * Kp * sizeof(float);
    l.off_enmax = up256(l.off_enorm + (size_t)Kp * sizeof(float));
    l.off_eb = l.off_enmax + 256;
    l.bytes = filter_shape_ok(C, K) ? up256(l.off_eb + (size_t)2 * C * Kp * sizeof(unsigned short)) : l.off_eb;
    return l;
}

PreparedView prepared_view(const void* prepared, int C, int K) {
    const PreparedLayout l = prepared_layout(C, K);
    char* base = const_cast<char*>(static_cast<const char*>(prepared));
    return {reinterpret_cast<float*>(base + l.off_e4), reinterpret_cast<float*>(base + l.off_enorm),
            reinterpret_cast<float*>(base + l.off_enmax), reinterpret_cast<unsigned short*>(base + l.off_eb)};
}

size_t prepared_bytes(int C, int K) { return prepared_layout(C, K).bytes; }

static int g_vq_max_tiles = 8;
static int g_vq_fine_split = 1;
static int g_vq_bf16_filter = 1;
static int g_vq_filter_force_all = 0;
static int g_vq_filter_launches = 0;
static const Option VQ_OPTIONS[] = {
    {"vq_max_tiles_per_wave", &g_vq_max_tiles, OPT_POW2_FAIL, 1, 8},
    {"vq_fine_split", &g_vq_fine_split, OPT_FLAG},
    {"vq_bf16_filter", &g_vq_bf16_filter, OPT_FLAG},
    {"vq_filter_force_all", &g_vq_filter_force_all, OPT_FLAG},
    {"vq_filter_launches", &g_vq_filter_launches},
};

int vq_set_option(const char* key, int value) { return apply_option(VQ_OPTIONS, key, value); }

VqPlan vq_plan(int64_t N, int C, int K) {
    VqPlan p;
    p.Cp = C;
    p.Kp = round_up(K, 32);
    size_t off = 0;
    p.off_prepared = off;
    off += prepared_bytes(C, K);
    p.off_keys = off;
    off += up256((size_t)N * sizeof(unsigned long long));
    p.off_hist = off;
    off += up256((size_t)p.Kp * sizeof(int));
    p.off_partial = off;
    off += (size_t)GATHER_BLOCKS_MAX * sizeof(float);
    off = up256(off);
    p.off_summary = p.off_brow = p.off_amb = p.off_pair_rc = off;
    p.pair_cap = 0;
    if (filter_shape_ok(C, K)) {
        p.off_summary = off;
        off += up256((size_t)N * (p.Kp / F_SUB) * sizeof(unsigned long long));
        p.off_brow = off;
        off += up256((size_t)N * sizeof(float));
        p.off_amb = off;
        off += 512;
        const long total_cap = 4 * N < (1L << 30) ? 4 * N : (1L << 30);
        p.pair_cap = (int)((total_cap + F_LISTS - 1) / F_LISTS);
        if (p.pair_cap < 1024) p.pair_cap = 1024;
        p.off_pair_rc = off;
        off += up256((size_t)p.pair_cap * F_LISTS * sizeof(unsigned long long));
    }
    p.bytes = up256(off);
    long blocks = (N + GATHER_ROWS_PER_BLOCK - 1) / GATHER_ROWS_PER_BLOCK;
    p.gather_blocks = (int)(blocks < GATHER_BLOCKS_MAX ? (blocks > 0 ? blocks : 1) : GATHER_BLOCKS_MAX);
    const int k1 = K;
    p.T = vq_group_tiles(1, &N, &k1);
    return p;
}

hipError_t launch_prepare(const float* W, int K, int C, void* prepared, hipStream_t st) {
    const int Kp = round_up(K, 32);
    const PreparedView pv = prepared_view(prepared, C, K);
    launch_prepare_exact(W, K, C, Kp, pv.E4, pv.enorm, st);
    if (filter_shape_ok(C, K)) launch_prepare_filter(W, K, C, Kp, pv.enorm, pv.Eb, pv.en_max, st);
    return hipGetLastError();
}

struct ProfShape {
    int64_t n;
    int c, k;
    int slot, group;
    int kind;
};
struct Profile {
    bool enabled = false;
    int capacity = 0;
    std::vector<hipEvent_t> ev;
    std::vector<ProfShape> shape;
};
static Profile g_prof;

hipError_t profile_begin(int capacity) {
    profile_release();
    g_prof.ev.resize((size_t)capacity * 2);
    for (auto& e : g_prof.ev) {
        hipError_t rc = hipEventCreate(&e);
        if (rc != hipSuccess) return rc;
    }
    g_prof.shape.clear();
    g_prof.capacity = capacity;
    g_prof.enabled = true;
    return hipSuccess;
}

void profile_release() {
    for (auto& e : g_prof.ev) (void)hipEventDestroy(e);
    g_prof.ev.clear();
    g_prof.shape.clear();
    g_prof.enabled = false;
    g_prof.capacity = 0;
}

int profile_collect(int max_records, int64_t* n, int* c, int* k, float* ms, int* kind) {
    g_prof.enabled = false;
    const int cnt = (int)g_prof.shape.size();
    int out = 0;
    for (int i = 0; i < cnt && out < max_records; ++i) {
        const ProfShape& sh = g_prof.shape[i];
        if (hipEventSynchronize(g_prof.ev[2 * sh.slot + 1]) != hipSuccess) break;
        float t = 0.f;
        if (hipEventElapsedTime(&t, g_prof.ev[2 * sh.slot], g_prof.ev[2 * sh.slot + 1]) != hipSuccess) break;
        double mine = 2.0 * (double)sh.n * sh.c * sh.k, all = 0.0;
        for (int j = sh.slot; j < sh.slot + sh.group && j < cnt; ++j) all += 2.0 * (double)g_prof.shape[j].n * g_prof.shape[j].c * g_prof.shape[j].k;
        n[out] = sh.n;
        c[out] = sh.c;
        k[out] = sh.k;
        ms[out] = (float)(t * (all > 0 ? mine / all : 1.0));
        if (kind) kind[out] = sh.kind;
        ++out;
    }
    profile_release();
    return out;
}


static unsigned assign_workgroups(int64_t N, int Kp, int T) {
    const long row_tiles = (N + ROWS_PER_WG - 1) / ROWS_PER_WG;
    return (unsigned)((row_tiles + 7) / 8 * 8 * (Kp / (32 * T)));
}

constexpr long VQ_FINE_WGS = 4096;
static long vq_group_wgs(int n, const int64_t* N, const int* K, int t) {
    long wgs = 0;
    for (int i = 0; i < n; ++i) {
        const int tiles = round_up(K[i], 32) / 32;
        if (tiles % t) return -1;
        wgs += ((N[i] + ROWS_PER_WG - 1) / ROWS_PER_WG) * (tiles / t);
    }
    return wgs;
}
int vq_group_tiles(int n, const int64_t* N, const int* K) {
    if (g_vq_fine_split)
        for (int t = g_vq_max_tiles; t >= 4; t >>= 1)
            if (vq_group_wgs(n, N, K, t) >= VQ_FINE_WGS) return t;
    for (int t = g_vq_max_tiles; t >= 1; t >>= 1) {
        const long wgs = vq_group_wgs(n, N, K, t);
        if (wgs >= 0 && (wgs >= 512 || t == 1)) return t;
    }
    return 1;
}

hipError_t launch_assign_group(int n, const void* const* x, int x_bf16, const int64_t* N, const int* C, const int* K,
                               const void* const* prepared, const VqPlan* plans, char* const* ws, int64_t* const* idx,
                               float* const* dmin, int T, hipStream_t st, const float* const* codebooks) {
    if (n < 1 || n > VQ_MAX_LEVELS) return hipErrorInvalidValue;
    int order[VQ_MAX_LEVELS];
    for (int i = 0; i < n; ++i) order[i] = i;
    for (int i = 0; i < n; ++i)
        for (int j = i + 1; j < n; ++j)
            if (C[order[j]] > C[order[i]]) { const int t = order[i]; order[i] = order[j]; order[j] = t; }
    bool filter = x_bf16 && g_vq_bf16_filter;
    for (int i = 0; i < n; ++i) filter = filter && filter_shape_ok(C[i], K[i]);
    VqLevel lv[VQ_MAX_LEVELS];
    VqFilterGroup fg;
    fg.n = n;
    unsigned end = 0, fend = 0, rend = 0, send = 0, iend = 0;
    VqInitGroup ig;
    ig.n = n;
    for (int q = 0; q < n; ++q) {
        const int i = order[q];
        const PreparedView pv = prepared_view(prepared[i], C[i], K[i]);
        unsigned long long* keys = reinterpret_cast<unsigned long long*>(ws[i] + plans[i].off_keys);
        {
            long ib = (N[i] + 4095) / 4096;
            ib = ib < 1 ? 1 : (ib > 256 ? 256 : ib);
            iend += (unsigned)ib;
            ig.lv[q] = VqInitLevel{keys, (long)N[i], nullptr, reinterpret_cast<int*>(ws[i] + plans[i].off_hist), plans[i].Kp, iend};
        }
        end += assign_workgroups(N[i], plans[i].Kp, T);
        lv[q] = VqLevel{x[i], pv.E4, pv.enorm, keys, (long)N[i], C[i], plans[i].Kp, end};
        lv[q].K = K[i];
        if (filter) {
            int* amb = reinterpret_cast<int*>(ws[i] + plans[i].off_amb);
            ig.lv[q].amb = amb;
            lv[q].gate = amb + F_LISTS;
            lv[q].gate_cap = 0;
            const long row_tiles = (N[i] + F_ROWS - 1) / F_ROWS;
            fend += (unsigned)((row_tiles + 7) / 8 * 8 * (plans[i].Kp / F_CODES));
            rend += (unsigned)((N[i] + 255) / 256);
            {
                long per = (N[i] / 256 + F_LISTS - 1) / F_LISTS;
                if (per < 4) per = 4;
                if (per > 16) per = 16;
                send += (unsigned)(per * F_LISTS);
            }
            fg.lv[q] = VqFilterLevel{x[i], pv.Eb, pv.enorm, pv.en_max,
                                     reinterpret_cast<unsigned long long*>(ws[i] + plans[i].off_summary),
                                     reinterpret_cast<float*>(ws[i] + plans[i].off_brow),
                                     reinterpret_cast<unsigned long long*>(ws[i] + plans[i].off_pair_rc), amb, plans[i].pair_cap, keys,
                                     codebooks ? codebooks[i] : nullptr, pv.E4, (long)N[i], C[i], plans[i].Kp, fend, rend, send};
        }
    }
    launch_group_init(ig, st);
    const bool rec = g_prof.enabled && (int)g_prof.shape.size() + n <= g_prof.capacity;
    const size_t slot = g_prof.shape.size();
    if (rec) {
        for (int i = 0; i < n; ++i) g_prof.shape.push_back({N[i], C[i], K[i], (int)slot, n, filter ? 2 : (x_bf16 ? 1 : 0)});
        (void)hipEventRecord(g_prof.ev[2 * slot], st);
    }
    if (filter) {
        ++g_vq_filter_launches;
        launch_filter(fg, g_vq_filter_force_all, st);
    }
    launch_assign_levels(lv, n, T, x_bf16, st);
    if (rec) (void)hipEventRecord(g_prof.ev[2 * slot + 1], st);
    hipError_t e = hipGetLastError();
    if (e != hipSuccess) return e;
    for (int i = 0; i < n; ++i) {
        launch_unpack_level(i, N, K, plans, ws, idx, dmin, st);
        if (filter && dmin && dmin[i]) {
            const PreparedView pv = prepared_view(prepared[i], C[i], K[i]);
            launch_exact_dist(x[i], pv.E4, plans[i].Kp, pv.enorm, idx[i], N[i], C[i], dmin[i], st);
        }
    }
    return hipGetLastError();
}

hipError_t launch_assign(const void* x, int x_bf16, int64_t N, int C, int K, const void* prepared, const VqPlan& p, char* ws,
                         int64_t* idx, float* dmin, hipStream_t st, const float* codebook) {
    return launch_assign_group(1, &x, x_bf16, &N, &C, &K, &prepared, &p, &ws, &idx, &dmin, p.T, st, codebook ? &codebook : nullptr);
}

KmPlan km_plan(int64_t N, int C, int K) {
    KmPlan p;
    p.vq = vq_plan(N, C, K);
    size_t off = p.vq.bytes;
    p.off_idx = off;
    off += (size_t)N * sizeof(int64_t);
    p.off_counts = off;
    off += (size_t)round_up(K + 1, 64) * sizeof(int);
    p.off_offsets = off;
    off += (size_t)round_up(K + 1, 64) * sizeof(int);
    p.off_members = off;
    off += (size_t)N * sizeof(int);
    p.off_sums = off;
    off += (size_t)K * C * sizeof(float);
    p.off_counts64 = off;
    off += (size_t)round_up(K, 32) * sizeof(int64_t);
    p.row_blocks = (int)((N + KM_RB - 1) / KM_RB);
    p.max_segments = (int)(N / KM_SEG + K);
    p.off_hist = off;
    off += (size_t)round_up(p.row_blocks * K, 64) * sizeof(int);
    p.off_segoff = off;
    off += (size_t)round_up(K + 1, 64) * sizeof(int);
    p.off_partial = off;
    off += (size_t)p.max_segments * C * sizeof(float);
    p.bytes = up256(off);
    return p;
}

hipError_t launch_km_accumulate(const float* samples, const float* means, int64_t N, int C, int K, const KmPlan& p,
                                char* ws, float* sums, int64_t* counts64, hipStream_t st) {
    hipError_t e = launch_prepare(means, K, C, ws + p.vq.off_prepared, st);
    if (e != hipSuccess) return e;
    int64_t* idx = reinterpret_cast<int64_t*>(ws + p.off_idx);
    e = launch_assign(samples, 0, N, C, K, ws + p.vq.off_prepared, p.vq, ws, idx, nullptr, st);
    if (e != hipSuccess) return e;
    return launch_code_sums(samples, 0, idx, N, C, K, p, ws, sums, counts64, st);
}

}
```

### vq_seg_amd/csrc/vq_internal.h

```cpp
#pragma once
#include "vq_kernels.h"

namespace vqseg {

typedef float f32x16 __attribute__((ext_vector_type(16)));
typedef float f32x4 __attribute__((ext_vector_type(4)));
typedef unsigned int u32x2 __attribute__((ext_vector_type(2)));
typedef unsigned int u32x4 __attribute__((ext_vector_type(4)));

constexpr int ROWS_PER_WG = 128;
constexpr int F_ROWS = 128, F_CODES = 256, F_SUB = 128;
constexpr int F_LISTS = 64;
constexpr int GATHER_BLOCKS_MAX = 2048;
constexpr int GATHER_ROWS_PER_BLOCK = 16;
constexpr int KM_RB = 1024;
constexpr int KM_SEG = 128;

struct VqLevel {
    const void* x;
    const float* E4;
    const float* enorm;
    unsigned long long* keys;
    long N;
    int C, Kp;
    unsigned wg_end;
    const int* gate = nullptr;
    int gate_cap = 0;
    int K = 0;
};
struct VqFilterLevel {
    const void* x;
    const unsigned short* Eb;
    const float* enorm;
    const float* en_max;
    unsigned long long* summary;
    float* brow;
    unsigned long long* pair_rc;
    int* pair_count;
    int pair_cap;
    unsigned long long* keys;
    const float* W;
    const float* E4;
    long N;
    int C, Kp;
    unsigned wg_end;
    unsigned rblk_end;
    unsigned sblk_end;
};
struct VqFilterGroup {
    VqFilterLevel lv[VQ_MAX_LEVELS];
    int n;
};
struct VqInitLevel {
    unsigned long long* keys;
    long n;
    int* amb;
    int* hist;
    int kp;
    unsigned end;
};
struct VqInitGroup {
    VqInitLevel lv[VQ_MAX_LEVELS];
    int n;
};

struct PreparedView {
    float* E4;
    float* enorm;
    float* en_max;
    unsigned short* Eb;
};
PreparedView prepared_view(const void* prepared, int C, int K);

void launch_assign_levels(const VqLevel* lv, int n, int T, int x_bf16, hipStream_t st);
void launch_prepare_filter(const float* W, int K, int C, int Kp, const float* enorm, unsigned short* Eb, float* en_max, hipStream_t st);
void launch_filter(const VqFilterGroup& fg, int force_all, hipStream_t st);
void launch_exact_dist(const void* x, const float* E4, int Kp, const float* enorm, const int64_t* idx, int64_t N, int C, float* dmin,
                       hipStream_t st);
void launch_group_init(const VqInitGroup& ig, hipStream_t st);
void launch_unpack_level(int i, const int64_t* N, const int* K, const VqPlan* plans, char* const* ws, int64_t* const* idx,
                         float* const* dmin, hipStream_t st);
void launch_prepare_exact(const float* W, int K, int C, int Kp, float* E4, float* enorm, hipStream_t st);

}
```

### vq_seg_amd/csrc/vq_tail.hip

```cpp
#include <hip/hip_runtime.h>
#include <stdint.h>

#include "vq_internal.h"

namespace vqseg {

static_assert(F_LISTS + 1 <= 128, "the init launch zeroes 128 ints of a level's counter block");
__global__ __launch_bounds__(256) void vq_group_init_kernel(const VqInitGroup g) {
    int q = 0;
    while (q + 1 < g.n && blockIdx.x >= g.lv[q].end) ++q;
    const VqInitLevel& L = g.lv[q];
    const unsigned first = q ? g.lv[q - 1].end : 0u, nb = L.end - first, b = blockIdx.x - first;
    for (long i = (long)b * 256 + threadIdx.x; i < L.n; i += (long)nb * 256) L.keys[i] = ~0ull;
    if (b == 0) {
        if (L.amb && threadIdx.x < 128) L.amb[threadIdx.x] = 0;
        for (int k = threadIdx.x; k < L.kp; k += 256) L.hist[k] = 0;
    }
}

__global__ __launch_bounds__(256) void vq_unpack_keys(const unsigned long long* __restrict__ keys, long N,
                                                      long long* __restrict__ idx, float* __restrict__ dmin,
                                                      int* __restrict__ hist, int K, int lds_hist) {
    extern __shared__ int lh[];
    if (hist && lds_hist)
        for (int k = threadIdx.x; k < K; k += 256) lh[k] = 0;
    __syncthreads();
    for (long i = (long)blockIdx.x * 256 + threadIdx.x; i < N; i += (long)gridDim.x * 256) {
        const unsigned long long k = keys[i];
        unsigned code = (unsigned)(k & 0xffffffffull);
        if (code >= (unsigned)K) code = 0u;
        idx[i] = (long long)code;
        if (dmin) dmin[i] = __uint_as_float((unsigned int)(k >> 32));
        if (hist && code < (unsigned)K) atomicAdd((lds_hist ? lh : hist) + code, 1);
    }
    if (hist && lds_hist) {
        __syncthreads();
        for (int k = threadIdx.x; k < K; k += 256) {
            const int c = lh[k];
            if (c) atomicAdd(hist + k, c);
        }
    }
}

template <typename TA>
__device__ __forceinline__ f32x4 ld4(const TA* p, long v) {
    if constexpr (sizeof(TA) == 4) {
        return reinterpret_cast<const f32x4*>(p)[v];
    } else {
        const u32x2 r = reinterpret_cast<const u32x2*>(p)[v];
        return f32x4{__builtin_bit_cast(float, r[0] << 16), __builtin_bit_cast(float, r[0] & 0xFFFF0000u),
                     __builtin_bit_cast(float, r[1] << 16), __builtin_bit_cast(float, r[1] & 0xFFFF0000u)};
    }
}
template <typename TA>
__device__ __forceinline__ void st4(TA* p, long v, const f32x4& q) {
    if constexpr (sizeof(TA) == 4) {
        reinterpret_cast<f32x4*>(p)[v] = q;
    } else {
        u32x2 r;
#pragma unroll
        for (int e = 0; e < 2; ++e) {
            const __bf16 lo = (__bf16)q[2 * e], hi = (__bf16)q[2 * e + 1];
            r[e] = (unsigned)__builtin_bit_cast(unsigned short, lo) | ((unsigned)__builtin_bit_cast(unsigned short, hi) << 16);
        }
        reinterpret_cast<u32x2*>(p)[v] = r;
    }
}

template <typename TA>
__global__ __launch_bounds__(256) void vq_gather_kernel(const TA* __restrict__ x, const float* __restrict__ W,
                                                        const long long* __restrict__ idx, long N, int C,
                                                        int training, TA* __restrict__ quant,
                                                        float* __restrict__ partial) {
    const int lane = threadIdx.x & 63, wave = threadIdx.x >> 6;
    const int c4 = C >> 2;
    float sq = 0.0f;
    constexpr int RG = 4;
    for (long row0 = ((long)blockIdx.x * 4 + wave) * RG; row0 < N; row0 += (long)gridDim.x * 4 * RG) {
        long long k[RG];
#pragma unroll
        for (int j = 0; j < RG; ++j) k[j] = row0 + j < N ? idx[row0 + j] : 0;
        for (int v = lane; v < c4; v += 64) {
            f32x4 e[RG], xv[RG];
#pragma unroll
            for (int j = 0; j < RG; ++j) {
                if (row0 + j < N) {
                    e[j] = reinterpret_cast<const f32x4*>(W + k[j] * (long)C)[v];
                    if (training) xv[j] = ld4<TA>(x + (row0 + j) * (long)C, v);
                }
            }
#pragma unroll
            for (int j = 0; j < RG; ++j) {
                if (row0 + j < N) {
                    TA* qr = quant + (row0 + j) * (long)C;
                    if (training) {
                        f32x4 q;
#pragma unroll
                        for (int i = 0; i < 4; ++i) {
                            q[i] = xv[j][i] + (e[j][i] - xv[j][i]);
                            const float dlt = q[i] - xv[j][i];
                            sq = __builtin_fmaf(dlt, dlt, sq);
                        }
                        st4<TA>(qr, v, q);
                    } else {
                        st4<TA>(qr, v, e[j]);
                    }
                }
            }
        }
    }
#pragma unroll
    for (int m = 32; m >= 1; m >>= 1) sq += __shfl_xor(sq, m);
    __shared__ float wsum[4];
    if (lane == 0) wsum[wave] = sq;
    __syncthreads();
    if (threadIdx.x == 0) partial[blockIdx.x] = (wsum[0] + wsum[1]) + (wsum[2] + wsum[3]);
}

__global__ __launch_bounds__(256) void vq_finalize_kernel(const float* __restrict__ partial, int n_partial,
                                                          const int* __restrict__ hist, int K, int training,
                                                          float commitment_weight, double numel,
                                                          float* __restrict__ loss, float* __restrict__ dead_pct) {
    __shared__ double sd[256];
    __shared__ int sz[256];
    double s = 0.0;
    for (int i = threadIdx.x; i < n_partial; i += 256) s += (double)partial[i];
    int z = 0;
    for (int k = threadIdx.x; k < K; k += 256) z += (hist[k] == 0);
    sd[threadIdx.x] = s;
    sz[threadIdx.x] = z;
    __syncthreads();
    for (int m = 128; m >= 1; m >>= 1) {
        if (threadIdx.x < m) {
            sd[threadIdx.x] += sd[threadIdx.x + m];
            sz[threadIdx.x] += sz[threadIdx.x + m];
        }
        __syncthreads();
    }
    if (threadIdx.x == 0) {
        float l = 0.0f;
        if (training && commitment_weight > 0.0f) l = (float)(sd[0] / numel) * commitment_weight;
        loss[0] = l;
        dead_pct[0] = 100.0f * ((float)sz[0] / (float)K);
    }
}

__global__ __launch_bounds__(256) void vq_backward_kernel(const float* __restrict__ gq, const float* __restrict__ gloss,
                                                          const float* __restrict__ x, const float* __restrict__ q,
                                                          long n4, float coef, float* __restrict__ gx) {
    const float k = gloss ? gloss[0] * coef : 0.0f;
    for (long i = (long)blockIdx.x * 256 + threadIdx.x; i < n4; i += (long)gridDim.x * 256) {
        const f32x4 g = reinterpret_cast<const f32x4*>(gq)[i];
        const f32x4 xv = reinterpret_cast<const f32x4*>(x)[i];
        const f32x4 qv = reinterpret_cast<const f32x4*>(q)[i];
        f32x4 o;
#pragma unroll
        for (int j = 0; j < 4; ++j) o[j] = __builtin_fmaf(k, xv[j] - qv[j], g[j]);
        reinterpret_cast<f32x4*>(gx)[i] = o;
    }
}

__global__ __launch_bounds__(256) void vq_backward_idx_kernel(const __bf16* __restrict__ gq, const float* __restrict__ gloss,
                                                              const __bf16* __restrict__ x, const long long* __restrict__ idx,
                                                              const float* __restrict__ W, long N, int C, float coef,
                                                              __bf16* __restrict__ gx) {
    const float k = gloss ? gloss[0] * coef : 0.0f;
    const int c4 = C >> 2;
    const long n4 = N * c4;
    for (long i = (long)blockIdx.x * 256 + threadIdx.x; i < n4; i += (long)gridDim.x * 256) {
        const long row = i / c4;
        const int v = (int)(i - row * c4);
        const f32x4 g = ld4<__bf16>(gq, i), xv = ld4<__bf16>(x, i);
        const f32x4 e = reinterpret_cast<const f32x4*>(W + idx[row] * (long)C)[v];
        f32x4 o;
#pragma unroll
        for (int j = 0; j < 4; ++j) o[j] = __builtin_fmaf(k, xv[j] - e[j], g[j]);
        st4<__bf16>(gx, i, o);
    }
}

void launch_group_init(const VqInitGroup& ig, hipStream_t st) {
    hipLaunchKernelGGL(vq_group_init_kernel, dim3(ig.lv[ig.n - 1].end), dim3(256), 0, st, ig);
}

void launch_unpack_level(int i, const int64_t* N, const int* K, const VqPlan* plans, char* const* ws, int64_t* const* idx,
                         float* const* dmin, hipStream_t st) {
    int* hist = reinterpret_cast<int*>(ws[i] + plans[i].off_hist);
    long blocks = (N[i] + 1023) / 1024;
    if (blocks > 512) blocks = 512;
    if (blocks < 1) blocks = 1;
    const int lds_hist = K[i] <= 8192;
    hipLaunchKernelGGL(vq_unpack_keys, dim3((unsigned)blocks), dim3(256), lds_hist ? (size_t)K[i] * sizeof(int) : 0, st,
                       reinterpret_cast<unsigned long long*>(ws[i] + plans[i].off_keys), (long)N[i],
                       reinterpret_cast<long long*>(idx[i]), dmin ? dmin[i] : nullptr, hist, K[i], lds_hist);
}

hipError_t launch_gather(const void* x, int bf16, const float* W, const int64_t* idx, int64_t N, int C, int K, int training,
                         float cw, const VqPlan& p, char* ws, void* quant, float* loss, float* dead, hipStream_t st) {
    int* hist = reinterpret_cast<int*>(ws + p.off_hist);
    float* partial = reinterpret_cast<float*>(ws + p.off_partial);
    if (bf16)
        hipLaunchKernelGGL(vq_gather_kernel<__bf16>, dim3(p.gather_blocks), dim3(256), 0, st, static_cast<const __bf16*>(x), W,
                           reinterpret_cast<const long long*>(idx), (long)N, C, training, static_cast<__bf16*>(quant), partial);
    else
        hipLaunchKernelGGL(vq_gather_kernel<float>, dim3(p.gather_blocks), dim3(256), 0, st, static_cast<const float*>(x), W,
                           reinterpret_cast<const long long*>(idx), (long)N, C, training, static_cast<float*>(quant), partial);
    hipLaunchKernelGGL(vq_finalize_kernel, dim3(1), dim3(256), 0, st, partial, p.gather_blocks, hist, K, training, cw,
                       (double)N * (double)C, loss, dead);
    return hipGetLastError();
}

hipError_t launch_backward(const float* gq, const float* gloss, const float* x, const float* q, int64_t N, int C,
                           float cw, float* gx, hipStream_t st) {
    const long n4 = (long)N * C / 4;
    const float coef = (float)((double)cw * 2.0 / ((double)N * (double)C));
    long blocks = (n4 + 255) / 256;
    if (blocks > 4096) blocks = 4096;
    if (blocks < 1) blocks = 1;
    hipLaunchKernelGGL(vq_backward_kernel, dim3((unsigned)blocks), dim3(256), 0, st, gq, gloss, x, q, n4, coef, gx);
    return hipGetLastError();
}

hipError_t launch_backward_idx(const void* gq, const float* gloss, const void* x, const int64_t* idx, const float* W, int64_t N,
                               int C, float cw, void* gx, hipStream_t st) {
    const long n4 = (long)N * C / 4;
    const float coef = (float)((double)cw * 2.0 / ((double)N * (double)C));
    long blocks = (n4 + 255) / 256;
    if (blocks > 4096) blocks = 4096;
    if (blocks < 1) blocks = 1;
    hipLaunchKernelGGL(vq_backward_idx_kernel, dim3((unsigned)blocks), dim3(256), 0, st, static_cast<const __bf16*>(gq), gloss,
                       static_cast<const __bf16*>(x), reinterpret_cast<const long long*>(idx), W, (long)N, C, coef,
                       static_cast<__bf16*>(gx));
    return hipGetLastError();
}

}
```

### vq_seg_amd/csrc/vqseg_abi.hip

```cpp
#include <hip/hip_runtime.h>
#include <stdarg.h>
#include <stdio.h>
#include <string.h>

#include "../../include/vqseg.h"
#include "vq_kernels.h"

namespace {
thread_local char g_err[512] = "";

int fail(int code, const char* fmt, ...) {
    va_list ap;
    va_start(ap, fmt);
    vsnprintf(g_err, sizeof(g_err), fmt, ap);
    va_end(ap);
    return code;
}
int hip_fail(hipError_t e, const char* where) {
    snprintf(g_err, sizeof(g_err), "%s: %s", where, hipGetErrorString(e));
    return (int)e;
}
bool aligned16(const void* p) { return (reinterpret_cast<uintptr_t>(p) & 15u) == 0; }

int check_shape(int64_t n, int c, int k) {
    if (n <= 0 || c <= 0 || k <= 0) return fail(VQSEG_EINVAL, "n_rows, channels and n_codes must be positive (got %lld, %d, %d)", (long long)n, c, k);
    if (c % 4) return fail(VQSEG_EINVAL, "channels must be a multiple of 4 (got %d)", c);
    if (n > (int64_t)1 << 31) return fail(VQSEG_EINVAL, "n_rows too large (%lld)", (long long)n);
    return 0;
}
}

extern "C" {

int vqseg_set_error(int code, const char* msg) {
    snprintf(g_err, sizeof(g_err), "%s", msg);
    return code;
}

int vqseg_abi_version(void) { return VQSEG_ABI_VERSION; }
const char* vqseg_last_error(void) { return g_err; }

const char* vqseg_kernel_name(const char* entry) {
    if (!entry) return "";
    if (!strcmp(entry, "vqseg_vq_forward_f32") || !strcmp(entry, "vqseg_vq_assign_f32") ||
        !strcmp(entry, "vqseg_kmeans_f32") || !strcmp(entry, "vqseg_kmeans_accumulate_f32"))
        return "vq_assign_f32_kernel";
    if (!strcmp(entry, "vqseg_vq_backward_f32")) return "vq_backward_kernel";
    if (!strcmp(entry, "vqseg_kmeans_finalize_f32")) return "km_finalize_kernel";
    return "";
}

int vqseg_profile_begin(int capacity) {
    if (capacity <= 0 || capacity > (1 << 20)) return fail(VQSEG_EINVAL, "capacity out of range");
    hipError_t e = vqseg::profile_begin(capacity);
    if (e != hipSuccess) return hip_fail(e, "profile_begin");
    return 0;
}

int vqseg_profile_collect(int max_records, int64_t* n_rows_host, int* channels_host, int* n_codes_host, float* ms_host, int* kind_host) {
    if (max_records <= 0 || !n_rows_host || !channels_host || !n_codes_host || !ms_host)
        return fail(VQSEG_EINVAL, "bad argument");
    return vqseg::profile_collect(max_records, n_rows_host, channels_host, n_codes_host, ms_host, kind_host);
}

size_t vqseg_vq_workspace_bytes(int64_t n, int c, int k) {
    if (n <= 0 || c <= 0 || k <= 0) return 0;
    return vqseg::vq_plan(n, c, k).bytes;
}

size_t vqseg_vq_filter_counter_offset(int64_t n, int c, int k) {
    if (n <= 0 || c <= 0 || k <= 0) return 0;
    const vqseg::VqPlan p = vqseg::vq_plan(n, c, k);
    return p.off_amb == p.off_summary ? 0 : p.off_amb;
}

int vqseg_vq_tiles_per_wave(int n_levels, const int64_t* n_rows_host, const int* n_codes_host) {
    if (n_levels < 1 || n_levels > vqseg::VQ_MAX_LEVELS || !n_rows_host || !n_codes_host) return fail(VQSEG_EINVAL, "tiles_per_wave: bad argument");
    for (int i = 0; i < n_levels; ++i)
        if (n_rows_host[i] <= 0 || n_codes_host[i] <= 0) return fail(VQSEG_EINVAL, "tiles_per_wave: non-positive size");
    return vqseg::vq_group_tiles(n_levels, n_rows_host, n_codes_host);
}

size_t vqseg_vq_prepared_bytes(int c, int k) {
    if (c <= 0 || k <= 0) return 0;
    return vqseg::prepared_bytes(c, k);
}

int vqseg_vq_prepare_f32(const float* codebook, int c, int k, void* prepared, size_t prepared_bytes, void* stream) {
    if (int rc = check_shape(1, c, k)) return rc;
    if (!codebook || !prepared) return fail(VQSEG_EINVAL, "null pointer argument");
    if (!aligned16(codebook) || !aligned16(prepared)) return fail(VQSEG_EINVAL, "codebook and prepared must be 16-byte aligned");
    if (prepared_bytes < vqseg::prepared_bytes(c, k))
        return fail(VQSEG_ENOSPC, "prepared buffer %zu < %zu bytes", prepared_bytes, vqseg::prepared_bytes(c, k));
    hipError_t e = vqseg::launch_prepare(codebook, k, c, prepared, static_cast<hipStream_t>(stream));
    if (e != hipSuccess) return hip_fail(e, "vq codebook prepare");
    return 0;
}

static int vq_assign_any(const void* x, int x_bf16, const float* codebook, const void* prepared, int64_t n, int c, int k,
                         int64_t* idx, float* dmin, void* ws, size_t ws_bytes, void* stream) {
    if (int rc = check_shape(n, c, k)) return rc;
    if (x_bf16 && c % 8) return fail(VQSEG_EINVAL, "bf16 rows need channels %% 8 == 0");
    if (!x || !idx || !ws || (!codebook && !prepared)) return fail(VQSEG_EINVAL, "null pointer argument");
    if (!aligned16(x) || !aligned16(ws) || !aligned16(prepared) || !aligned16(codebook))
        return fail(VQSEG_EINVAL, "x, codebook, prepared and workspace must be 16-byte aligned");
    const vqseg::VqPlan p = vqseg::vq_plan(n, c, k);
    if (ws_bytes < p.bytes) return fail(VQSEG_ENOSPC, "workspace %zu < %zu bytes", ws_bytes, p.bytes);
    hipStream_t st = static_cast<hipStream_t>(stream);
    char* w = static_cast<char*>(ws);
    if (!prepared) {
        hipError_t e = vqseg::launch_prepare(codebook, k, c, w + p.off_prepared, st);
        if (e != hipSuccess) return hip_fail(e, "vq codebook prepare");
        prepared = w + p.off_prepared;
    }
    hipError_t e = vqseg::launch_assign(x, x_bf16, n, c, k, prepared, p, w, idx, dmin, st, codebook);
    if (e != hipSuccess) return hip_fail(e, "vq_assign_f32_kernel");
    return 0;
}

int vqseg_vq_assign_f32(const float* x, const float* codebook, const void* prepared, int64_t n, int c, int k,
                        int64_t* idx, float* dmin, void* ws, size_t ws_bytes, void* stream) {
    return vq_assign_any(x, 0, codebook, prepared, n, c, k, idx, dmin, ws, ws_bytes, stream);
}

int vqseg_vq_assign_bf16(const void* x, const float* codebook, const void* prepared, int64_t n, int c, int k,
                         int64_t* idx, float* dmin, void* ws, size_t ws_bytes, void* stream) {
    return vq_assign_any(x, 1, codebook, prepared, n, c, k, idx, dmin, ws, ws_bytes, stream);
}

static int vq_forward_any(const void* x, int bf16, const float* codebook, const void* prepared, int64_t n, int c, int k,
                          int training, float cw, void* quant, int64_t* idx, float* loss, float* dead_pct, float* dmin,
                          void* ws, size_t ws_bytes, void* stream) {
    if (!quant || !loss || !dead_pct || !codebook) return fail(VQSEG_EINVAL, "null pointer argument");
    if (!aligned16(quant)) return fail(VQSEG_EINVAL, "quant must be 16-byte aligned");
    if (int rc = vq_assign_any(x, bf16, codebook, prepared, n, c, k, idx, dmin, ws, ws_bytes, stream)) return rc;
    const vqseg::VqPlan p = vqseg::vq_plan(n, c, k);
    hipError_t e = vqseg::launch_gather(x, bf16, codebook, idx, n, c, k, training, cw, p, static_cast<char*>(ws), quant, loss,
                                        dead_pct, static_cast<hipStream_t>(stream));
    if (e != hipSuccess) return hip_fail(e, "vq_gather_kernel");
    return 0;
}

int vqseg_vq_forward_f32(const float* x, const float* codebook, const void* prepared, int64_t n, int c, int k,
                         int training, float cw, float* quant, int64_t* idx, float* loss, float* dead_pct, float* dmin,
                         void* ws, size_t ws_bytes, void* stream) {
    return vq_forward_any(x, 0, codebook, prepared, n, c, k, training, cw, quant, idx, loss, dead_pct, dmin, ws, ws_bytes, stream);
}

int vqseg_vq_forward_bf16(const void* x, const float* codebook, const void* prepared, int64_t n, int c, int k,
                          int training, float cw, void* quant, int64_t* idx, float* loss, float* dead_pct, float* dmin,
                          void* ws, size_t ws_bytes, void* stream) {
    return vq_forward_any(x, 1, codebook, prepared, n, c, k, training, cw, quant, idx, loss, dead_pct, dmin, ws, ws_bytes, stream);
}

int vqseg_vq_forward_group(int n_levels, int bf16, const void* const* x, const float* const* codebook, const void* const* prepared,
                           const int64_t* n, const int* c, const int* k, int training, const float* cw, void* const* quant,
                           int64_t* const* idx, float* const* loss, float* const* dead_pct, void* const* ws, const size_t* ws_bytes,
                           void* stream) {
    if (n_levels < 1 || n_levels > vqseg::VQ_MAX_LEVELS) return fail(VQSEG_EINVAL, "1 .. %d levels per grouped launch", vqseg::VQ_MAX_LEVELS);
    if (!x || !codebook || !n || !c || !k || !cw || !quant || !idx || !loss || !dead_pct || !ws || !ws_bytes)
        return fail(VQSEG_EINVAL, "null pointer argument");
    vqseg::VqPlan plans[vqseg::VQ_MAX_LEVELS];
    const void* prep[vqseg::VQ_MAX_LEVELS];
    char* wsp[vqseg::VQ_MAX_LEVELS];
    hipStream_t st = static_cast<hipStream_t>(stream);
    for (int i = 0; i < n_levels; ++i) {
        if (int rc = check_shape(n[i], c[i], k[i])) return rc;
        if (bf16 && c[i] % 8) return fail(VQSEG_EINVAL, "bf16 rows need channels %% 8 == 0");
        if (!x[i] || !codebook[i] || !quant[i] || !idx[i] || !loss[i] || !dead_pct[i] || !ws[i]) return fail(VQSEG_EINVAL, "null pointer argument");
        if (!aligned16(x[i]) || !aligned16(ws[i]) || !aligned16(codebook[i]) || !aligned16(quant[i]) || (prepared && !aligned16(prepared[i])))
            return fail(VQSEG_EINVAL, "x, codebook, prepared, quant and workspace must be 16-byte aligned");
        plans[i] = vqseg::vq_plan(n[i], c[i], k[i]);
        if (ws_bytes[i] < plans[i].bytes) return fail(VQSEG_ENOSPC, "workspace %zu < %zu bytes", ws_bytes[i], plans[i].bytes);
        wsp[i] = static_cast<char*>(ws[i]);
        prep[i] = prepared ? prepared[i] : nullptr;
        if (!prep[i]) {
            hipError_t e = vqseg::launch_prepare(codebook[i], k[i], c[i], wsp[i] + plans[i].off_prepared, st);
            if (e != hipSuccess) return hip_fail(e, "vq codebook prepare");
            prep[i] = wsp[i] + plans[i].off_prepared;
        }
    }
    const int T = vqseg::vq_group_tiles(n_levels, n, k);
    hipError_t e = vqseg::launch_assign_group(n_levels, x, bf16, n, c, k, prep, plans, wsp, idx, nullptr, T, st, codebook);
    if (e != hipSuccess) return hip_fail(e, "vq_assign_f32_kernel (grouped)");
    for (int i = 0; i < n_levels; ++i) {
        e = vqseg::launch_gather(x[i], bf16, codebook[i], idx[i], n[i], c[i], k[i], training, cw[i], plans[i], wsp[i], quant[i], loss[i],
                                 dead_pct[i], st);
        if (e != hipSuccess) return hip_fail(e, "vq_gather_kernel");
    }
    return 0;
}

int vqseg_vq_backward_bf16(const void* gq, const float* gloss, const void* x, const int64_t* idx, const float* codebook,
                           int64_t n, int c, float cw, void* gx, void* stream) {
    if (int rc = check_shape(n, c, 1)) return rc;
    if (!gq || !x || !idx || !codebook || !gx) return fail(VQSEG_EINVAL, "null pointer argument");
    if (c % 8) return fail(VQSEG_EINVAL, "bf16 rows need channels %% 8 == 0");
    if (!aligned16(gq) || !aligned16(x) || !aligned16(codebook) || !aligned16(gx)) return fail(VQSEG_EINVAL, "tensors must be 16-byte aligned");
    hipError_t e = vqseg::launch_backward_idx(gq, gloss, x, idx, codebook, n, c, cw, gx, static_cast<hipStream_t>(stream));
    if (e != hipSuccess) return hip_fail(e, "vq_backward_idx_kernel");
    return 0;
}

int vqseg_vq_backward_f32(const float* gq, const float* gloss, const float* x, const float* quant, int64_t n, int c,
                          float cw, float* gx, void* stream) {
    if (int rc = check_shape(n, c, 1)) return rc;
    if (!gq || !x || !quant || !gx) return fail(VQSEG_EINVAL, "null pointer argument");
    if (!aligned16(gq) || !aligned16(x) || !aligned16(quant) || !aligned16(gx))
        return fail(VQSEG_EINVAL, "tensors must be 16-byte aligned");
    hipError_t e = vqseg::launch_backward(gq, gloss, x, quant, n, c, cw, gx, static_cast<hipStream_t>(stream));
    if (e != hipSuccess) return hip_fail(e, "vq_backward_kernel");
    return 0;
}

size_t vqseg_kmeans_workspace_bytes(int64_t n, int c, int k) {
    if (n <= 0 || c <= 0 || k <= 0) return 0;
    return vqseg::km_plan(n, c, k).bytes;
}

int vqseg_kmeans_accumulate_f32(const float* samples, const float* means, int64_t n, int c, int k, float* sums,
                                int64_t* counts, void* ws, size_t ws_bytes, void* stream) {
    if (int rc = check_shape(n, c, k)) return rc;
    if (!samples || !means || !sums || !counts || !ws) return fail(VQSEG_EINVAL, "null pointer argument");
    if (!aligned16(samples) || !aligned16(ws)) return fail(VQSEG_EINVAL, "samples and workspace must be 16-byte aligned");
    const vqseg::KmPlan p = vqseg::km_plan(n, c, k);
    if (ws_bytes < p.bytes) return fail(VQSEG_ENOSPC, "workspace %zu < %zu bytes", ws_bytes, p.bytes);
    hipError_t e = vqseg::launch_km_accumulate(samples, means, n, c, k, p, static_cast<char*>(ws), sums, counts,
                                               static_cast<hipStream_t>(stream));
    if (e != hipSuccess) return hip_fail(e, "kmeans accumulate");
    return 0;
}

int vqseg_vq_code_sums(int bf16, const void* x, const int64_t* idx, int64_t n, int c, int k, float* sums, int64_t* counts, void* ws,
                       size_t ws_bytes, void* stream) {
    if (int rc = check_shape(n, c, k)) return rc;
    if (!x || !idx || !sums || !counts || !ws) return fail(VQSEG_EINVAL, "null pointer argument");
    if (!aligned16(ws)) return fail(VQSEG_EINVAL, "workspace must be 16-byte aligned");
    const vqseg::KmPlan p = vqseg::km_plan(n, c, k);
    if (ws_bytes < p.bytes) return fail(VQSEG_ENOSPC, "workspace %zu < %zu bytes", ws_bytes, p.bytes);
    hipError_t e = vqseg::launch_code_sums(x, bf16 != 0, idx, n, c, k, p, static_cast<char*>(ws), sums, counts,
                                           static_cast<hipStream_t>(stream));
    if (e != hipSuccess) return hip_fail(e, "code sums");
    return 0;
}

int vqseg_vq_ema_update_f32(float* cluster_size, float* embed_avg, float* codebook, const float* sums, const int64_t* counts, int c,
                            int k, float decay, float eps, float* scratch, void* stream) {
    if (c <= 0 || k <= 0 || !cluster_size || !embed_avg || !codebook || !sums || !counts || !scratch)
        return fail(VQSEG_EINVAL, "bad argument");
    if (!(decay >= 0.0f && decay <= 1.0f) || !(eps >= 0.0f)) return fail(VQSEG_EINVAL, "need 0 <= decay <= 1, eps >= 0");
    hipError_t e = vqseg::launch_ema_update(cluster_size, embed_avg, codebook, sums, counts, k, c, decay, eps, scratch,
                                            static_cast<hipStream_t>(stream));
    if (e != hipSuccess) return hip_fail(e, "ema_embed_kernel");
    return 0;
}

int vqseg_vq_revive_candidates(int bf16, const void* x, int64_t n, int c, int k, uint64_t seed, const int64_t* counter, int rank,
                               int world, float* cand, float* ok, void* stream) {
    if (!x || !counter || !cand || !ok) return fail(VQSEG_EINVAL, "revive candidates: null pointer argument");
    if (n < 1 || k < 1) return fail(VQSEG_EINVAL, "revive candidates: n_rows and n_codes must be positive (got %lld, %d)", (long long)n, k);
    if (n > (int64_t)1 << 31) return fail(VQSEG_EINVAL, "n_rows too large (%lld)", (long long)n);
    if (world < 1) return fail(VQSEG_EINVAL, "revive candidates: world must be >= 1 (got %d)", world);
    if (rank < 0 || rank >= world) return fail(VQSEG_EINVAL, "revive candidates: rank %d outside [0, %d)", rank, world);
    if (c <= 0 || c % 4) return fail(VQSEG_EINVAL, "channels must be a multiple of 4 (got %d)", c);
    if (bf16 && c % 8) return fail(VQSEG_EINVAL, "bf16 rows need channels %% 8 == 0");
    if (!aligned16(x) || !aligned16(cand)) return fail(VQSEG_EINVAL, "rows and cand must be 16-byte aligned");
    hipError_t e = vqseg::launch_revive_candidates(x, bf16 != 0, n, c, k, seed, counter, rank, world, cand, ok,
                                                   static_cast<hipStream_t>(stream));
    if (e != hipSuccess) return hip_fail(e, "revive_candidates_kernel");
    return 0;
}

int vqseg_vq_ema_update_revive_f32(float* cluster_size, float* embed_avg, float* codebook, const float* sums, const int64_t* counts,
                                   int c, int k, float decay, float eps, float* scratch, const float* cand, const float* ok,
                                   float threshold, int64_t* counter, int64_t* revived, void* stream) {
    if (c <= 0 || k <= 0 || !cluster_size || !embed_avg || !codebook || !sums || !counts || !scratch)
        return fail(VQSEG_EINVAL, "bad argument");
    if (!cand || !ok || !counter || !revived) return fail(VQSEG_EINVAL, "ema update with revival: null pointer argument");
    if (!(decay >= 0.0f && decay <= 1.0f) || !(eps >= 0.0f)) return fail(VQSEG_EINVAL, "need 0 <= decay <= 1, eps >= 0");
    if (!(threshold >= 0.0f) || threshold > 3.0e38f) return fail(VQSEG_EINVAL, "need a finite threshold >= 0");
    hipError_t e = vqseg::launch_ema_update_revive(cluster_size, embed_avg, codebook, sums, counts, k, c, decay, eps, scratch, cand, ok,
                                                   threshold, counter, revived, static_cast<hipStream_t>(stream));
    if (e != hipSuccess) return hip_fail(e, "ema_embed_revive_kernel");
    return 0;
}

int vqseg_kmeans_finalize_f32(const float* sums, const int64_t* counts, float* means, int c, int k, void* stream) {
    if (c <= 0 || k <= 0 || !sums || !counts || !means) return fail(VQSEG_EINVAL, "bad argument");
    hipError_t e = vqseg::launch_km_finalize(sums, counts, means, c, k, static_cast<hipStream_t>(stream));
    if (e != hipSuccess) return hip_fail(e, "km_finalize_kernel");
    return 0;
}

int vqseg_kmeans_f32(const float* samples, float* means, int64_t* bins, int64_t n, int c, int k, int iters, void* ws,
                     size_t ws_bytes, void* stream) {
    if (int rc = check_shape(n, c, k)) return rc;
    if (!samples || !means || !bins || !ws) return fail(VQSEG_EINVAL, "null pointer argument");
    if (iters < 0) return fail(VQSEG_EINVAL, "iters must be >= 0");
    const vqseg::KmPlan p = vqseg::km_plan(n, c, k);
    if (ws_bytes < p.bytes) return fail(VQSEG_ENOSPC, "workspace %zu < %zu bytes", ws_bytes, p.bytes);
    char* w = static_cast<char*>(ws);
    float* sums = reinterpret_cast<float*>(w + p.off_sums);
    hipStream_t st = static_cast<hipStream_t>(stream);
    for (int it = 0; it < iters; ++it) {
        if (int rc = vqseg_kmeans_accumulate_f32(samples, means, n, c, k, sums, bins, ws, ws_bytes, stream)) return rc;
        hipError_t e = vqseg::launch_km_finalize(sums, bins, means, c, k, st);
        if (e != hipSuccess) return hip_fail(e, "km_finalize_kernel");
    }
    return 0;
}

}
```

### vq_seg_amd/models/networks/modified_vqunet/net.py

```python
import torch
from torch import nn

from .... import nnf
from ....vector_quantizer import make_vq_module, Identity as _IdentityVQ, quantize_group as _quantize_group
from ...encoders import make_encoder
from ...modules.prototype import ReliablePrototypeLoss, ReliablePrototypeLossv2
from ..unet.decoder import UnetDecoder
from ..unet.net import _to_device_layout


class _Upsampling(nn.Module):

    def __init__(self, scale_factor):
        super().__init__()
        self.scale_factor = scale_factor

    def forward(self, x):
        return nnf.upsample_bilinear(x, scale_factor=self.scale_factor, align_corners=True)


class _Head1x1(nn.Conv2d):
    def forward(self, x):
        return nnf.head_conv1x1(x, self.weight)


class _VQRePTUnet1x1Base(nn.Module):
    _proto_cls = None

    def __init__(self, encoder_name: str, num_classes: int, vq_cfg: dict, margin=1.5, scale=1., use_feature=False,
                 encoder_weights=None, in_channels: int = 3, decoder_channels=None, depth: int = 5,
                 activation=nn.Identity, upsampling=2, pt_init="kmeans"):
        super().__init__()
        self.encoder = make_encoder(encoder_name, in_channels, depth, weights=encoder_weights, padding_mode="reflect")
        enc_ch = self.encoder.out_channels()
        self.codebook = make_vq_module(vq_cfg, enc_ch, depth)
        if decoder_channels is None:
            decoder_channels = [c // 2 for c in enc_ch[1:]][::-1]
        self.decoder = UnetDecoder(enc_ch, decoder_channels)
        self.segmentation_head = _Head1x1(decoder_channels[-1], num_classes, 1, bias=False)
        self.prototype_loss = self._proto_cls(num_classes, decoder_channels[-1], margin=margin, scale=scale, init=pt_init,
                                              use_feature=use_feature)
        self.device = None
        self.upsampling = _Upsampling(upsampling) if upsampling > 1 else nn.Identity()

    def encode(self, x):
        if self.device is None:
            self.device = x.device
        with nnf.s3_scope(not self.training and not torch.is_grad_enabled()):
            feats = self.encoder(_to_device_layout(x))[1:]
        if len(feats) != len(self.codebook):
            raise NotImplementedError
        return feats

    def quantize(self, feats):
        loss = torch.zeros(1, device=feats[0].device)
        usage = []
        levels = [i for i, vq in enumerate(self.codebook) if not isinstance(vq, _IdentityVQ)]
        for i in levels:
            if isinstance(feats[i], nnf.S3):
                feats[i] = feats[i].float()
        grouped = _quantize_group([self.codebook[i] for i in levels], [feats[i] for i in levels]) if nnf.py_opt("py_vq_group", 1) else None
        grouped = dict(zip(levels, grouped)) if grouped is not None else {}
        for i, vq in enumerate(self.codebook):
            quantize, _idx, commitment, dead = grouped[i] if i in grouped else vq(feats[i])
            feats[i] = quantize
            if commitment is not None:
                loss = loss + commitment
            if dead is not None:
                usage.append(dead.detach())
        return feats, loss / len(feats), usage

    def decode(self, feats):
        decoder_out = self.decoder(*feats)
        if self.training:
            nnf.fanin_tag(decoder_out)
        return decoder_out, self.segmentation_head(decoder_out)

    def _trunk(self, x):
        feats, loss, usage = self.quantize(self.encode(x))
        decoder_out, logits = self.decode(feats)
        return decoder_out, logits, loss, usage

    async_code_usage = False

    def _usage_to_host(self, usage, like):
        if not usage:
            return torch.tensor([])
        stacked = torch.stack(usage)
        if not (self.async_code_usage and stacked.is_cuda):
            return stacked.cpu()
        ring = self.__dict__.setdefault("_usage_ring", [])
        if len(ring) < 8:
            ring.append(torch.empty(stacked.shape, dtype=stacked.dtype, pin_memory=True))
        buf = ring[self.__dict__.setdefault("_usage_i", 0) % len(ring)]
        self.__dict__["_usage_i"] += 1
        buf.copy_(stacked, non_blocking=True)
        return buf

    @torch.no_grad()
    def pseudo_label(self, x):
        _, logits, _, _ = self._trunk(x)
        return torch.argmax(logits, dim=1).long()


class VQRePTUnet1x1(_VQRePTUnet1x1Base):
    _proto_cls = ReliablePrototypeLoss

    def forward(self, x, gt=None, code_usage_loss=False, percent=None):
        return self.finish(*self.quantize(self.encode(x)), gt=gt, code_usage_loss=code_usage_loss, percent=percent)

    def finish(self, feats, loss, usage, gt=None, code_usage_loss=False, percent=None):
        decoder_out, output = self.decode(feats)
        prototype_loss = None
        if self.training:
            with torch.no_grad():
                if nnf.softmax_stats_supported(output):
                    entropy = nnf.softmax_stats(output, want_label=False)[1].reshape(-1)
                else:
                    prob = torch.softmax(output.float().permute(0, 2, 3, 1).reshape(-1, output.shape[1]), dim=1)
                    entropy = -torch.sum(prob * torch.log(prob + 1e-10), dim=1)
            prototype_loss = self.prototype_loss(decoder_out, gt, percent=percent, entropy=entropy)
        output = self.upsampling(output)
        if code_usage_loss:
            return output, loss, self._usage_to_host(usage, output), torch.stack(usage).sum()[None] / len(self.codebook)
        return output, loss, self._usage_to_host(usage, output), prototype_loss


class VQRePTUnet1x1v2(_VQRePTUnet1x1Base):
    _proto_cls = ReliablePrototypeLossv2

    def forward(self, x, gt=None, code_usage_loss=False, th=None):
        return self.finish(*self.quantize(self.encode(x)), gt=gt, code_usage_loss=code_usage_loss, th=th)

    def finish(self, feats, loss, usage, gt=None, code_usage_loss=False, th=None):
        decoder_out, output = self.decode(feats)
        prototype_loss = self.prototype_loss(decoder_out, gt, th) if self.training else None
        output = self.upsampling(output)
        if code_usage_loss:
            return output, loss, self._usage_to_host(usage, output), torch.stack(usage).sum()[None] / len(self.codebook)
        return output, loss, self._usage_to_host(usage, output), prototype_loss
```

### vq_seg_amd/nnf.py

```python
from __future__ import annotations

from collections import namedtuple
import contextlib
import ctypes
from typing import Optional
import weakref

import torch
import torch.nn.functional as F

from . import _hip
from ._hip import lib
from ._wcache import cache_of as _cache_of, invalidate as invalidate_weight_caches


def _rows(x: torch.Tensor) -> torch.Tensor:
    v = x.permute(0, 2, 3, 1)
    return v if v.is_contiguous() else v.contiguous()


def _nchw(rows: torch.Tensor) -> torch.Tensor:
    return rows.permute(0, 3, 1, 2)


# ... 355 lines not shown

    def __init__(self):
        self.g = None
        self.closed = False
        self.leftover = None
        self.bits = None
        self.takes_bits = False


def _mask_with_bits(g, bits):
    sh = torch.arange(8, device=g.device, dtype=torch.uint8)
    keep = torch.bitwise_and(torch.bitwise_right_shift(bits.view(-1, 1), sh), 1).view(g.shape).to(torch.bool)
    return torch.where(keep, g, torch.zeros((), dtype=g.dtype, device=g.device))


_FANIN_ON = False
_FANIN_OPEN: set = set()


def set_fanin_fusion(on: bool) -> bool:
    global _FANIN_ON
    prev = _FANIN_ON
    _FANIN_ON = bool(on) and py_opt("py_fanin", 1) == 1
    return prev


def fanin_tag(t):
    if _FANIN_ON and torch.is_tensor(t) and t.requires_grad and torch.is_grad_enabled():
        t._vq_fanin = GradLink()
    return t


def _fanin_of(t):
    return getattr(t, "_vq_fanin", None) if (_FANIN_ON and torch.is_tensor(t)) else None


def _fanin_deposit(link, g_rows) -> bool:
    if link is None or link.closed or link.g is not None:
        return False
    link.g = g_rows
    _FANIN_OPEN.add(link)
    return True


def _fanin_take(link, shape, dtype):
    if link is None:
        return None
    link.closed = True
    g, link.g = link.g, None
    _FANIN_OPEN.discard(link)
    if g is None:
        return None
    if tuple(g.shape) == tuple(shape) and g.dtype == dtype and g.is_contiguous():
        return g
    link.leftover = g
    return None


def check_fanin_consumed() -> None:
    if _FANIN_OPEN:
        n = len(_FANIN_OPEN)
        for l_ in list(_FANIN_OPEN):
            l_.g = None
        _FANIN_OPEN.clear()
        raise RuntimeError(f"fan-in fusion: {n} deposited gradient(s) were never absorbed -- a consumer's backward did not run; "
                           f"switch the fusion off (VQSEG_OPTS=py_fanin=0) for graphs that use only part of the model's outputs")


_UNIT_AFFINE = {}


def _unit_affine(dev, c):
    key = (str(dev), c)
    if key not in _UNIT_AFFINE:
        _UNIT_AFFINE[key] = (torch.ones(c, dtype=torch.float32, device=dev), torch.zeros(c, dtype=torch.float32, device=dev))
        torch.cuda.current_stream(dev).synchronize()
    return _UNIT_AFFINE[key]


def _sink_ready(p) -> bool:
    g = getattr(p, "grad", None)
    return hasattr(p, "_vq_grad_sink") and g is not None and g.dtype == torch.float32 and g.is_contiguous() and g.is_cuda


def _sink_use(*params) -> None:
    if torch.is_grad_enabled():
        for p in params:
            if p.requires_grad and hasattr(p, "_vq_grad_sink"):
                p._vq_uses = getattr(p, "_vq_uses", 0) + 1


def _sink_done(p) -> None:
    p._vq_uses = getattr(p, "_vq_uses", 1) - 1
    cb = p._vq_grad_sink
    if cb is not None and p._vq_uses <= 0:
        cb(p)


class S3:
    __slots__ = ("rows", "c")

    def __init__(self, rows: torch.Tensor, c: int):
        self.rows, self.c = rows, c

    @property
    def shape(self):
        n, h, w, _ = self.rows.shape
        return torch.Size((n, self.c, h, w))

    dtype = torch.float32
    is_cuda = True
    requires_grad = False

    @property
    def device(self):
        return self.rows.device

    def float(self) -> torch.Tensor:
        n, h, w, _ = self.rows.shape
        out = torch.empty((n, h, w, self.c), dtype=torch.float32, device=self.rows.device)
        _launch("vqseg_s3_merge_f", out.device, _T(self.rows, "split-3 rows", bf=2, numel=n * h * w * 2 * self.c), n * h * w, self.c,
                _f32(out, "merged rows", n * h * w * self.c))
        return _nchw(out)


_S3_SCOPE = False


class s3_scope:

    def __init__(self, enabled: bool = True):
        self.enabled = bool(enabled) and py_opt("py_s3_eval", 1) == 1

    def __enter__(self):
        global _S3_SCOPE
        self.prev = _S3_SCOPE
        _S3_SCOPE = self.enabled
        return self

    def __exit__(self, *exc):
        global _S3_SCOPE
        _S3_SCOPE = self.prev
        return False


def to_s3(x) -> "S3":
    if isinstance(x, S3):
        return x
    xr = _rows(x.float())
    n, h, w, c = xr.shape
    out = torch.empty((n, h, w, 2 * c), dtype=torch.bfloat16, device=xr.device)
    _launch("vqseg_s3_split_f", xr.device, _f32(xr, "rows", n * h * w * c), n * h * w, c, _T(out, "split-3 rows", bf=2, numel=n * h * w * 2 * c))
    return S3(out, c)


def from_s3(x):
    return x.float() if isinstance(x, S3) else x


def _s3_weights(weight: torch.Tensor, c1: int, as_1x1_cols: int = 0) -> torch.Tensor:
    if not as_1x1_cols:
        img = _pack_all(weight, ("s3", c1))
        if img is not None:
            return img
    cache = _cache_of(weight)
    k = ("s3", c1, as_1x1_cols)
    if k not in cache:
        w = weight.detach()
        if as_1x1_cols:
            cout, cin, kh, kw = w.shape
            w2 = torch.zeros(cout, as_1x1_cols, 1, 1, dtype=torch.float32, device=w.device)
            w2[:, :kh * kw * cin, 0, 0] = w.permute(0, 2, 3, 1).reshape(cout, kh * kw * cin)
            w = w2
        w = w if w.is_contiguous() else w.contiguous()
        cout, cin, kh, kw = w.shape
        out = torch.empty(cout * kh * kw * 3 * cin, dtype=torch.int16, device=w.device)
        _launch("vqseg_conv_pack_weights_s3_f32", w.device, _f32(w, "weight", cout * cin * kh * kw), cout, cin, c1, kh, kw,
                _w16(out, "split-3 image", cout * kh * kw * 3 * cin))
        cache[k] = out
    return cache[k]


def _conv_bn_act_s3(x: "S3", x2, residual, conv, bn, relu, kernel_1x1_cols: int = 0) -> "S3":
    n, h, w, _ = x.rows.shape
    c1 = x.c
    x2s = to_s3(x2) if x2 is not None else None
    cin = c1 + (x2s.c if x2s is not None else 0)
    cout = conv.weight.shape[0]
    if kernel_1x1_cols:
        kh = kw = 1
        stride, pad, reflect = 1, 0, False
    else:
        kh, kw = conv.weight.shape[2], conv.weight.shape[3]
        stride, pad = conv.stride[0], conv.padding[0]
        reflect = conv.padding_mode == "reflect" and pad > 0
    g = ConvGeom(n, h, w, c1, cin, cout, kh, kw, stride, pad, reflect, _out_size(h, kh, stride, pad), _out_size(w, kw, stride, pad))
    wimg = _s3_weights(conv.weight, c1, kernel_1x1_cols)
    res = to_s3(residual) if residual is not None else None
    coef = _bn_finalize(None, g.m, cout, bn.weight, bn.bias, bn, False, x.rows.device)
    out = _conv_affine(x.rows, x2s.rows if x2s is not None else None, wimg, None, coef[0], coef[1], res.rows if res is not None else None,
                       relu, g, 2)
    return S3(out, cout)


def _residual_rows(residual, dtype):
    rr = _rows(residual) if residual is not None else None
    if rr is not None and rr.dtype != dtype:
        raise _hip.HipLibraryError("residual dtype differs from the activation dtype")
    return rr


def _forward_eval(xr, x2r, residual, w_hi, w_lo, gamma, beta, bn, relu, g: ConvGeom, bf, stem):
    rr = _residual_rows(residual, xr.dtype)
    coef = _bn_finalize(None, g.m, g.cout, gamma, beta, bn, False, xr.device)
    if stem is not None and stem.is_fused:
        return _stem7_conv(xr, w_hi, None, coef, relu, stem, g.cout)
    return _conv_affine(xr, x2r, w_hi, w_lo, coef[0], coef[1], rr, relu, g, int(not bf))


class _ConvBNAct(torch.autograd.Function):
    @staticmethod
    def forward(ctx, x, x2, residual, weight, gamma, beta, bn, stride, pad, reflect, relu, stem, fuse_eval=False,
                link_in=None, link_out=None, link_x=None, fan_x=None, fan_x2=None):
        xr = _rows(x)
        x2r = _rows(x2) if x2 is not None else None
        bf = _is_bf16(xr)
        n, h, w, c1 = xr.shape
        fused = stem is not None and stem.is_fused
        stem_x = None
        if fused:
            stem_x, _STEM_X_ARG[0] = _STEM_X_ARG[0], None
            (h, w, c1), bf = stem.fused, 1
        cin = c1 + (x2r.shape[3] if x2r is not None else 0)
        cout = weight.shape[0]
        kh, kw = (1, 1) if stem is not None else (weight.shape[2], weight.shape[3])
        g = ConvGeom(n, h, w, c1, cin, cout, kh, kw, stride, pad, bool(reflect), _out_size(h, kh, stride, pad), _out_size(w, kw, stride, pad))
        training = bool(bn.training)
        if fused:
            w_hi, w_lo = _stem_weights_fused(weight, False), None
        elif stem is not None:
            w_hi, w_lo = _stem_weights(weight, not bf, cin)
        else:
            w_hi, w_lo = packed_weights(weight, not bf, False)
        if bn.momentum is None:
            raise NotImplementedError("BatchNorm2d(momentum=None) (cumulative average) is not used by the path")
        if fuse_eval and not training:
            return _nchw(_forward_eval(xr, x2r, residual, w_hi, w_lo, gamma, beta, bn, relu, g, bf, stem))
        stat = torch.empty(_stat_elems(g.m, cout), dtype=torch.float32, device=xr.device) if training else None
        y = _stem7_conv(xr, w_hi, stat, None, False, stem, cout) if fused else _conv_raw(xr, x2r, w_hi, w_lo, stat, g)
        coef = _bn_finalize(stat, g.m, cout, gamma, beta, bn, training, xr.device)
        rr = _residual_rows(residual, y.dtype)
        if rr is not None and relu and bf and cout % 8 == 0 and training and any(ctx.needs_input_grad) and py_opt("py_bn_bits", 1):
            out, bits = _bn_apply_bits(y, rr, coef, g.m, cout)
        else:
            out, bits = _bn_apply(y, rr, coef, g.m, cout, relu), None
        ctx.mask_bits = bits is not None
        if link_in is not None:
            link_in.takes_bits = bool(bf and x2r is None and stride == 1 and not reflect and cin % 8 == 0 and py_opt("py_gres_bits", 1))
        ctx.save_for_backward(xr, x2r, y, bits if bits is not None else out, coef, weight, gamma)
        ctx.stem_x = stem_x
        ctx.params = (weight, gamma, beta)
        ctx.bn = bn
        ctx.links = (link_in, link_out, link_x)
        ctx.fans = (fan_x, fan_x2)
        ctx.geom, ctx.stem = g, stem
        ctx.relu, ctx.training, ctx.has_res = bool(relu), training, residual is not None
        return _nchw(out)

    @staticmethod
    def backward(ctx, g_out):
        xr, x2r, y, out, coef, weight, gamma = ctx.saved_tensors
        g, stem = ctx.geom, ctx.stem
        if stem is not None and stem.is_fused:
            img = xr
            xr = _shared_stem_patches(ctx.stem_x if ctx.stem_x is not None else img,
                                      (torch.bfloat16, stem.kh, stem.kw, stem.stride, stem.pad, stem.reflect),
                                      lambda: _stem_patches(img, torch.bfloat16, stem.kh, stem.kw, stem.stride, stem.pad, stem.reflect, g.ho, g.wo, g.cin))
        g_y, g_res, dgamma, dbeta = _bn_backward_step(ctx, g_out, y, out, coef, gamma)
        gw = _wgrad_step(ctx, g_y, xr, x2r, weight)
        gx = gx2 = None
        if (ctx.needs_input_grad[0] or ctx.needs_input_grad[1]) and stem is None:
            gx, gx2 = _dgrad_step(ctx, g_y, x2r, weight)
        g_res_out = _nchw(g_res) if (ctx.has_res and ctx.links[1] is None) else None
        return (gx, gx2, g_res_out, gw, dgamma, dbeta) + (None,) * (_ConvBNAct.forward.__code__.co_argcount - 7)


def _bn_backward_step(ctx, g_out, y, out, coef, gamma):
    g = ctx.geom
    gr = _rows(g_out)
    if gr.dtype != y.dtype:
        gr = gr.to(y.dtype)
    link_out = ctx.links[1]
    bits_to_link = bool(ctx.has_res and ctx.mask_bits and link_out is not None and link_out.takes_bits and not link_out.closed)
    g_res = torch.empty_like(y) if (ctx.has_res and not bits_to_link) else None
    _, p_g, p_b = ctx.params
    sink = _sink_ready(p_g) and _sink_ready(p_b) and ctx.needs_input_grad[4] and ctx.needs_input_grad[5]
    dgb = None if sink else torch.empty(2, g.cout, dtype=torch.float32, device=y.device)
    dgamma, dbeta = (p_g.grad, p_b.grad) if sink else (dgb[0], dgb[1])
    g_y = _bn_backward(gr, out if (ctx.has_res and not ctx.mask_bits) else None, out if ctx.mask_bits else None, y, coef, gamma,
                       g.m, g.cout, ctx.relu, ctx.training, sink, dgamma, dbeta, g_res, ctx.bn)
    if sink:
        _sink_done(p_g), _sink_done(p_b)
    if link_out is not None and ctx.has_res:
        link_out.g = gr if bits_to_link else g_res
        link_out.bits = out if bits_to_link else None
    return (g_y, g_res, None, None) if sink else (g_y, g_res, dgb[0], dgb[1])
# ... 911 lines not shown
```

### vq_seg_amd/vector_quantizer/vq_img.py

```python
from __future__ import annotations

import torch
from torch import nn

from .. import _hip
from .. import nnf
from .._wcache import cache_of as _cache_of, invalidate as _invalidate
from ..dist import collectives_on as _collectives_on, broadcast0 as _broadcast0, all_reduce_sum as _all_reduce_sum, rank as _rank, \
    world_size as _world_size


class _VQFunction(torch.autograd.Function):

    @staticmethod
    def forward(ctx, rows, codebook, training, commitment_weight, prepared=None):
        quant, idx, loss, dead = _hip.vq_forward(rows, codebook, training, commitment_weight, prepared=prepared)
        ctx.commitment_weight = float(commitment_weight)
        ctx.training = bool(training)
        ctx.bf16 = rows.dtype == torch.bfloat16
        if training:
            if ctx.bf16:
                ctx.save_for_backward(rows, idx, codebook)
            else:
                ctx.save_for_backward(rows, quant)
        ctx.mark_non_differentiable(idx, dead)
        return quant, idx, loss, dead

    @staticmethod
    def backward(ctx, g_quant, _g_idx, g_loss, _g_dead):
        if not ctx.training:
            return None, None, None, None, None
        gl = g_loss.contiguous() if (g_loss is not None and ctx.commitment_weight > 0) else None
        if ctx.bf16:
            rows, idx, codebook = ctx.saved_tensors
            g_quant = torch.zeros_like(rows) if g_quant is None else g_quant.to(torch.bfloat16).contiguous()
            return _hip.vq_backward_bf16(g_quant, gl, rows, idx, codebook, ctx.commitment_weight), None, None, None, None
        rows, quant = ctx.saved_tensors
        if g_quant is None:
            g_quant = torch.zeros_like(rows)
        g_quant = g_quant.contiguous()
        gx = _hip.vq_backward(g_quant, gl, rows, quant, ctx.commitment_weight)
        return gx, None, None, None, None


class _VQGroupFunction(torch.autograd.Function):

    @staticmethod
    def forward(ctx, training, weights, n, fans, *tensors):
        rows, codebooks, prepared = tensors[:n], tensors[n:2 * n], tensors[2 * n:3 * n]
        ctx.fans = fans
        outs = _hip.vq_forward_group(list(rows), list(codebooks), list(prepared), training, weights)
        ctx.n, ctx.training, ctx.weights = n, bool(training), [float(w) for w in weights]
        ctx.bf16 = rows[0].dtype == torch.bfloat16
        if training:
            saved = []
            for r, cb, (q, idx, _l, _d) in zip(rows, codebooks, outs):
                saved += [r, idx, cb] if ctx.bf16 else [r, q]
            ctx.save_for_backward(*saved)
        flat, nondiff = [], []
        for q, idx, loss, dead in outs:
            nondiff += [idx, dead]
            flat += [q, idx, loss, dead]
        ctx.mark_non_differentiable(*nondiff)
        return tuple(flat)

    @staticmethod
    def backward(ctx, *grads):
        n = ctx.n
        none = (None, None, None, None) + (None,) * (3 * n)
        if not ctx.training:
            return none
        saved = ctx.saved_tensors
        gxs = []
        for i in range(n):
            g_quant, g_loss = grads[4 * i], grads[4 * i + 2]
            w = ctx.weights[i]
            gl = g_loss.contiguous() if (g_loss is not None and w > 0) else None
            if ctx.bf16:
                rows, idx, codebook = saved[3 * i:3 * i + 3]
                g_quant = torch.zeros_like(rows) if g_quant is None else g_quant.to(torch.bfloat16).contiguous()
                gxs.append(_hip.vq_backward_bf16(g_quant, gl, rows, idx, codebook, w))
            else:
                rows, quant = saved[2 * i:2 * i + 2]
                g_quant = torch.zeros_like(rows) if g_quant is None else g_quant.contiguous()
                gxs.append(_hip.vq_backward(g_quant, gl, rows, quant, w))
            fan = ctx.fans[i] if ctx.fans is not None else None
            if fan is not None and gxs[-1].dtype == fan[2] and nnf._fanin_deposit(fan[0], gxs[-1].reshape(fan[1])):
                gxs[-1] = None
        return (None, None, None, None) + tuple(gxs) + (None,) * (2 * n)


def quantize_group(vqs, feats):
    if len(vqs) < 2 or len(vqs) > 4:
        return None
    rows = []
    for vq, f in zip(vqs, feats):
        cb = vq.codebook
        if not torch.is_tensor(f) or not f.is_cuda or cb.ema_update or (cb.kmeans_init and vq.training and not cb.initted):
            return None
        rows.append(_rows_of(f))
    if len({r.dtype for r in rows}) != 1 or len({vq.training for vq in vqs}) != 1:
        return None
    n = len(vqs)
    weights = [float(vq.commitment_weight) for vq in vqs]
    fans = None
    if vqs[0].training and torch.is_grad_enabled():
        fans = []
        for f, r in zip(feats, rows):
            link = nnf._fanin_of(f)
            b, c, h, w = f.shape
            fans.append((link, (b, h, w, c), f.dtype) if (link is not None and r.dtype == f.dtype and r.data_ptr() == f.data_ptr()) else None)
        if not any(fans):
            fans = None
    flat = _VQGroupFunction.apply(vqs[0].training, weights, n, fans, *rows, *[vq.codebook.embedding.weight.detach() for vq in vqs],
                                  *[vq.codebook.prepared() for vq in vqs])
    outs = []
    for i, f in enumerate(feats):
        b, c, h, w = f.shape
        quant, idx, loss, dead = flat[4 * i:4 * i + 4]
        outs.append((quant.reshape(b, h, w, c).permute(0, 3, 1, 2), idx.reshape(b, h, w), loss, dead))
    return outs


def _rows_of(x: torch.Tensor):
    b, c, h, w = x.shape
    if not (x.dtype == torch.bfloat16 and x.is_cuda and c % 8 == 0 and torch.is_autocast_enabled()):
        x = x.to(torch.float32)
    rows = x.permute(0, 2, 3, 1)
    if not rows.is_contiguous():
        rows = rows.contiguous()
    return rows.reshape(b * h * w, c)


def kmeans_init_means(rows: torch.Tensor, num_clusters: int) -> torch.Tensor:
    n = rows.shape[0]
    if n >= num_clusters:
        pick = torch.randperm(n, device=rows.device)[:num_clusters]
    else:
        pick = torch.randint(0, n, (num_clusters,), device=rows.device)
    return rows[pick].contiguous()


def kmeans(rows: torch.Tensor, num_clusters: int, num_iters: int, init_means: torch.Tensor = None):
    means = (kmeans_init_means(rows, num_clusters) if init_means is None else init_means.clone()).contiguous()
    if not _collectives_on():
        return _hip.kmeans(rows, means, num_iters)
    _broadcast0(means)
    counts = torch.zeros(num_clusters, dtype=torch.int64, device=rows.device)
    for _ in range(num_iters):
        sums, counts = _hip.kmeans_accumulate(rows, means)
        _all_reduce_sum(sums)
        _all_reduce_sum(counts)
        _hip.kmeans_finalize(sums, counts, means)
    return means, counts


class EuclideanCodebook(nn.Module):
    def __init__(self, embedding_dim, num_embeddings, kmeans_init, kmeans_iters, decay, eps, num_codebook, ema_update=False,
                 threshold_ema_dead_code: float = 0.0, revive_seed: int = 0):
        super().__init__()
        if threshold_ema_dead_code < 0:
            raise ValueError(f"threshold_ema_dead_code must be >= 0, got {threshold_ema_dead_code}")
        if threshold_ema_dead_code > 0 and not ema_update:
            raise ValueError("threshold_ema_dead_code > 0 revives codes of the EMA update: it needs ema_update=True")
        self.kmeans_init = kmeans_init
        self.kmeans_iters = kmeans_iters
        self.initted = False
        self.num_codebook = num_codebook
        self.decay = decay
        self.eps = eps
        self.ema_update = bool(ema_update)
        self.embedding = nn.Embedding(num_embeddings, embedding_dim)
        self.num_embeddings = num_embeddings
        self.embedding_dim = embedding_dim
        if not kmeans_init:
            self.embedding.weight.data.uniform_(-1 / num_embeddings, 1 / num_embeddings)
            self.initted = True
        if self.ema_update:
            self.register_buffer("cluster_size", torch.zeros(num_embeddings))
            self.register_buffer("embed_avg", self.embedding.weight.detach().clone())
        self.threshold_ema_dead_code = float(threshold_ema_dead_code)
        self.revive_seed = int(revive_seed)
        self.revived = None
        if self.threshold_ema_dead_code > 0:
            self.register_buffer("ema_updates", torch.zeros((), dtype=torch.int64))

    def prepared(self) -> torch.Tensor:
        w = self.embedding.weight
        cache = _cache_of(w)
        if "vq_prepared" not in cache:
            cache["vq_prepared"] = _hip.vq_prepare(w.detach())
        return cache["vq_prepared"]

    @torch.no_grad()
    def _kmeans_init(self, rows: torch.Tensor):
        if self.initted:
            return
        means, bins = kmeans(rows, self.num_embeddings, self.kmeans_iters)
        self.embedding.weight.copy_(means)
        _invalidate(self.embedding.weight)
        if self.ema_update:
            self.embed_avg.copy_(means)
            self.cluster_size.copy_(bins.to(self.cluster_size.dtype))
        self.initted = True

    @torch.no_grad()
    def ema_step(self, rows: torch.Tensor, idx: torch.Tensor):
        if self.threshold_ema_dead_code > 0:
            return self._ema_revive_step(rows, idx)
        sums, counts = _hip.vq_code_sums(rows, idx.reshape(-1), self.num_embeddings)
        if _collectives_on():
            _all_reduce_sum(sums)
            _all_reduce_sum(counts)
        _hip.vq_ema_update(self.cluster_size, self.embed_avg, self.embedding.weight.detach(), sums, counts, self.decay, self.eps)
        _invalidate(self.embedding.weight)

    def _ema_revive_step(self, rows: torch.Tensor, idx: torch.Tensor):
        k, c = self.num_embeddings, self.embedding_dim
        flat = torch.empty(2 * k * c + k, dtype=torch.float32, device=rows.device)
        sums, cand, ok = flat[:k * c].view(k, c), flat[k * c:2 * k * c].view(k, c), flat[2 * k * c:]
        _, counts = _hip.vq_code_sums(rows, idx.reshape(-1), k, out=sums)
        _hip.vq_revive_candidates(rows, self.revive_seed, self.ema_updates, k, _rank(), _world_size(), out=(cand, ok))
        if _collectives_on():
            _all_reduce_sum(flat)
            _all_reduce_sum(counts)
        if self.revived is None or self.revived.device != rows.device:
            self.revived = torch.zeros((), dtype=torch.int64, device=rows.device)
        _hip.vq_ema_update(self.cluster_size, self.embed_avg, self.embedding.weight.detach(), sums, counts, self.decay, self.eps,
                           candidates=cand, ok=ok, threshold=self.threshold_ema_dead_code, counter=self.ema_updates, revived=self.revived)
        _invalidate(self.embedding.weight)

    def forward(self, x: torch.Tensor):
        b, hw, c = x.shape
        rows = x.float().reshape(b * hw, c).contiguous()
        if self.kmeans_init and self.training:
            self._kmeans_init(rows.detach())
        quant, idx, _loss, dead = _VQFunction.apply(rows.detach(), self.embedding.weight.detach(), False, 0.0,
                                                    self.prepared())
        return quant.reshape(b, hw, c), idx.reshape(b, hw), dead


class VectorQuantizer(nn.Module):
    def __init__(self, dim, num_embeddings, embedding_dim=None, decay=0.8, eps=1e-5, kmeans_init=False,
                 kmeans_iters=10, distance="euclidean", commitment_weight=1, num_codebook=1, ema_update=False,
                 threshold_ema_dead_code: float = 0.0, revive_seed: int = 0):
        super().__init__()
        embedding_dim = embedding_dim if embedding_dim is not None else dim
        self.num_embeddings = num_embeddings
        self.eps = eps
        self.commitment_weight = commitment_weight
        if distance != "euclidean":
            raise NotImplementedError(
                f"distance={distance!r}: only the euclidean codebook is on the accelerated path (SURVEY 2 #1; the "
                "cosine codebook is unused by the target configs)")
        self.codebook = EuclideanCodebook(embedding_dim=embedding_dim, num_embeddings=num_embeddings,
                                          kmeans_init=kmeans_init, kmeans_iters=kmeans_iters, decay=decay, eps=eps,
                                          num_codebook=num_codebook, ema_update=ema_update,
                                          threshold_ema_dead_code=threshold_ema_dead_code, revive_seed=revive_seed)

    def forward(self, x: torch.Tensor):
        b, c, h, w = x.shape
        rows = _rows_of(x)
        cb = self.codebook
        if cb.kmeans_init and self.training and not cb.initted:
            cb._kmeans_init(rows.detach().float())
        ema = cb.ema_update and self.training
        weight = cb.embedding.weight.detach()
        if ema:
            weight = weight.clone()
        quant, idx, loss, dead = _VQFunction.apply(rows, weight, self.training, float(self.commitment_weight), cb.prepared())
        if ema:
            cb.ema_step(rows.detach(), idx)
        quantize = quant.reshape(b, h, w, c).permute(0, 3, 1, 2)
# ... 2 lines not shown
```

Before: 439.2 images/sec.

## Quantize split-3 bf16 rows directly in grouped VQ eval path

```diff
diff --git a/include/vqseg.h b/include/vqseg.h
--- a/include/vqseg.h
+++ b/include/vqseg.h
@@ -52,6 +52,10 @@
 int vqseg_vq_assign_bf16(const void* x, const float* codebook, const void* prepared,
                          int64_t n_rows, int channels, int n_codes, int64_t* idx, float* dmin,
                          void* workspace, size_t workspace_bytes, void* stream);
+
+int vqseg_vq_assign_s3(const void* x, const float* codebook, const void* prepared,
+                       int64_t n_rows, int channels, int n_codes, int64_t* idx, float* dmin,
+                       void* workspace, size_t workspace_bytes, void* stream);
 
 size_t vqseg_vq_prepared_bytes(int channels, int n_codes);
 int vqseg_vq_prepare_f32(const float* codebook, int channels, int n_codes, void* prepared,
diff --git a/vq_seg_amd/_hip.py b/vq_seg_amd/_hip.py
--- a/vq_seg_amd/_hip.py
+++ b/vq_seg_amd/_hip.py
@@ -33,6 +33,8 @@
                                     c_size_t, c_void_p]),
     "vqseg_vq_assign_bf16": (c_int, [c_void_p, c_void_p, c_void_p, c_int64, c_int, c_int, c_void_p, c_void_p, c_void_p,
                                      c_size_t, c_void_p]),
+    "vqseg_vq_assign_s3": (c_int, [c_void_p, c_void_p, c_void_p, c_int64, c_int, c_int, c_void_p, c_void_p, c_void_p,
+                                   c_size_t, c_void_p]),
     "vqseg_vq_prepared_bytes": (c_size_t, [c_int, c_int]),
     "vqseg_vq_prepare_f32": (c_int, [c_void_p, c_int, c_int, c_void_p, c_size_t, c_void_p]),
     "vqseg_vq_backward_f32": (c_int, [c_void_p, c_void_p, c_void_p, c_void_p, c_int64, c_int, c_float, c_void_p,
@@ -300,37 +302,41 @@
     return _bind_symbols(ctypes.CDLL(path))
 
 
-def vq_forward_group(rows_list, codebooks, prepared_list, training: bool, commitment_weights, handle=None):
+def vq_forward_group(rows_list, codebooks, prepared_list, training: bool, commitment_weights, handle=None, s3: bool = False):
     L = handle or lib()
     nl = len(rows_list)
-    bf16 = rows_list[0].dtype == torch.bfloat16
+    bf16 = 2 if s3 else int(rows_list[0].dtype == torch.bfloat16)
+    if s3 and training:
+        raise HipLibraryError("vq_forward_group: split-3 rows are an eval-mode format (training must be False)")
     dev = rows_list[0].device
     ptr = lambda ps: (c_void_p * nl)(*map(on_gpu, ps))
     ns = np.array([r.shape[0] for r in rows_list], dtype=np.int64)
-    cs = np.array([r.shape[1] for r in rows_list], dtype=np.int32)
+    cs = np.array([w.shape[1] for w in codebooks], dtype=np.int32)
     ks = np.array([w.shape[0] for w in codebooks], dtype=np.int32)
     cw = np.array([float(w) for w in commitment_weights], dtype=np.float32)
     xs, wps, preps, quants, idxs, scals, wss = [], [], [], [], [], [], []
     for r, w in zip(rows_list, codebooks):
         if r.dtype != rows_list[0].dtype:
             raise HipLibraryError("vq_forward_group: one row type per call")
-        xs.append(tptr(r, "rows", bf=int(bf16)))
-        wps.append(_dev(w, torch.float32, "codebook", w.shape[0] * r.shape[1]))
+        if w.dim() != 2 or r.dim() != 2 or r.shape[1] != (2 if s3 else 1) * w.shape[1]:
+            raise HipLibraryError(f"vq_forward_group: rows {tuple(r.shape)} do not match a codebook {tuple(w.shape)}" + (" (split-3 rows: 2C columns)" if s3 else ""))
+        xs.append(tptr(r, "rows", bf=bf16, numel=r.shape[0] * r.shape[1]))
+        wps.append(_dev(w, torch.float32, "codebook", w.shape[0] * w.shape[1]))
         quants.append(torch.empty_like(r))
         idxs.append(torch.empty(r.shape[0], dtype=torch.int64, device=dev))
         scals.append(torch.empty(2, dtype=torch.float32, device=dev))
-        wss.append(_workspace(L.vqseg_vq_workspace_bytes(r.shape[0], r.shape[1], w.shape[0]), dev))
+        wss.append(_workspace(L.vqseg_vq_workspace_bytes(r.shape[0], w.shape[1], w.shape[0]), dev))
     for w, p_ in zip(codebooks, prepared_list):
         preps.append(tptr(p_, "prepared codebook", dtype=torch.uint8, numel=L.vqseg_vq_prepared_bytes(w.shape[1], w.shape[0])))
     wsb = (c_size_t * nl)(*[w.numel() for w in wss])
-    launch("vqseg_vq_forward_group", dev, nl, int(bf16), ptr(xs), ptr(wps), ptr(preps), ns.ctypes.data, cs.ctypes.data, ks.ctypes.data,
+    launch("vqseg_vq_forward_group", dev, nl, bf16, ptr(xs), ptr(wps), ptr(preps), ns.ctypes.data, cs.ctypes.data, ks.ctypes.data,
            int(bool(training)), cw.ctypes.data, ptr(q.data_ptr() for q in quants), ptr(i.data_ptr() for i in idxs),
            ptr(s.data_ptr() for s in scals), ptr(s.data_ptr() + 4 for s in scals), ptr(w.data_ptr() for w in wss),
            ctypes.cast(wsb, c_void_p), handle=handle)
     if FILTER_DIAG is not None and bf16:
         for r, w, ws_ in zip(rows_list, codebooks, wss):
-            off = L.vqseg_vq_filter_counter_offset(r.shape[0], r.shape[1], w.shape[0])
-            FILTER_DIAG.append((r.shape[0], r.shape[1], w.shape[0], ws_[off:off + 256].view(torch.int32) if off else None))
+            off = L.vqseg_vq_filter_counter_offset(r.shape[0], w.shape[1], w.shape[0])
+            FILTER_DIAG.append((r.shape[0], w.shape[1], w.shape[0], ws_[off:off + 256].view(torch.int32) if off else None))
     return [(q, i, s[0:1], s[1]) for q, i, s in zip(quants, idxs, scals)]
 
 
@@ -353,24 +359,32 @@
 
 
 def vq_assign(rows: torch.Tensor, codebook: torch.Tensor, want_dmin: bool = False,
-              prepared: Optional[torch.Tensor] = None, want_filter_count: bool = False):
+              prepared: Optional[torch.Tensor] = None, want_filter_count: bool = False, s3: bool = False, want_filter_state: bool = False):
     L = lib()
     n, c = rows.shape
     k = codebook.shape[0]
     bf16 = rows.dtype == torch.bfloat16
-    xp, wp = tptr(rows, "rows", bf=int(bf16), numel=n * c), _dev(codebook, torch.float32, "codebook", k * c)
+    if s3:
+        if c != 2 * codebook.shape[1]:
+            raise HipLibraryError(f"vq_assign: split-3 rows {tuple(rows.shape)} do not match a codebook {tuple(codebook.shape)} (2C columns)")
+        c //= 2
+    xp, wp = tptr(rows, "rows", bf=2 if s3 else int(bf16), numel=n * c * (2 if s3 else 1)), _dev(codebook, torch.float32, "codebook", k * c)
     dev = rows.device
     idx = torch.empty(n, dtype=torch.int64, device=dev)
     dmin = torch.empty(n, dtype=torch.float32, device=dev) if want_dmin else None
     nbytes = L.vqseg_vq_workspace_bytes(n, c, k)
     ws = _workspace(nbytes, dev)
-    launch("vqseg_vq_assign_bf16" if bf16 else "vqseg_vq_assign_f32", dev, xp, wp,
+    launch("vqseg_vq_assign_s3" if s3 else "vqseg_vq_assign_bf16" if bf16 else "vqseg_vq_assign_f32", dev, xp, wp,
            tptr(prepared, "prepared codebook", dtype=torch.uint8, numel=L.vqseg_vq_prepared_bytes(c, k)), n, c, k,
            idx.data_ptr(), dmin.data_ptr() if want_dmin else None, ws.data_ptr(), nbytes)
     if want_filter_count:
         off = L.vqseg_vq_filter_counter_offset(n, c, k) if bf16 else 0
         amb = ws[off:off + 256].view(torch.int32).sum() if off else None
         return (idx, dmin, amb) if want_dmin else (idx, amb)
+    if want_filter_state:
+        off = L.vqseg_vq_filter_counter_offset(n, c, k) if bf16 else 0
+        state = ws[off:off + 260].view(torch.int32).clone() if off else None
+        return (idx, dmin, state) if want_dmin else (idx, state)
     return (idx, dmin) if want_dmin else idx
 
 
diff --git a/vq_seg_amd/csrc/vq_assign.hip b/vq_seg_amd/csrc/vq_assign.hip
--- a/vq_seg_amd/csrc/vq_assign.hip
+++ b/vq_seg_amd/csrc/vq_assign.hip
@@ -33,6 +33,7 @@
 
 template <typename TX> struct RawFrag { typedef f32x4 type; };
 template <> struct RawFrag<__bf16> { typedef u32x2 type; };
+template <> struct RawFrag<S3Row> { typedef u32x4 type; };
 
 #if VQ_TIMELINE
 #define TL_STAMP(k_)                                                          \
@@ -81,7 +82,8 @@
     const long row0 = row_tile * ROWS_PER_WG + wave * ROWS_PER_WAVE;
     long row = row0 + r;
     if (row > N - 1) row = N - 1;
-    const TX* xrow = x + row * (long)C + 4 * h;
+    constexpr bool S3 = __is_same(TX, S3Row);
+    const TX* xrow = x + row * (S3 ? 2L * C : (long)C) + 4 * h;
 
     f32x16 acc[T];
 #pragma unroll
@@ -111,6 +113,9 @@
             const int col = stage * BK + 8 * j + 4 * h;
             if (col >= C) {
                 a[j] = RawA{};
+            } else if constexpr (S3) {
+                const u32x2 hi = *reinterpret_cast<const u32x2*>(xrow + stage * BK + 8 * j), lo = *reinterpret_cast<const u32x2*>(xrow + C + stage * BK + 8 * j);
+                a[j] = RawA{hi[0], hi[1], lo[0], lo[1]};
             } else {
                 a[j] = *reinterpret_cast<const RawA*>(xrow + stage * BK + 8 * j);
             }
@@ -130,6 +135,11 @@
                 const unsigned lo = src[j][0], hi = src[j][1];
                 dst[j] = f32x4{__builtin_bit_cast(float, lo << 16), __builtin_bit_cast(float, lo & 0xFFFF0000u),
                                __builtin_bit_cast(float, hi << 16), __builtin_bit_cast(float, hi & 0xFFFF0000u)};
+                if constexpr (S3) {
+                    const unsigned l0 = src[j][2], l1 = src[j][3];
+                    dst[j] += f32x4{__builtin_bit_cast(float, l0 << 16), __builtin_bit_cast(float, l0 & 0xFFFF0000u),
+                                    __builtin_bit_cast(float, l1 << 16), __builtin_bit_cast(float, l1 & 0xFFFF0000u)};
+                }
             }
         }
     };
@@ -314,7 +324,7 @@
     hipLaunchKernelGGL((vq_assign_f32_kernel<T, TX>), dim3(g.lv[g.n - 1].wg_end), dim3(256), lds, st, g);
 }
 
-void launch_assign_levels(const VqLevel* lv, int n, int T, int x_bf16, hipStream_t st) {
+void launch_assign_levels(const VqLevel* lv, int n, int T, int row_type, hipStream_t st) {
     VqGroup g;
     g.n = n;
     for (int q = 0; q < n; ++q) g.lv[q] = lv[q];
@@ -322,7 +332,8 @@
     g.tl = g_timeline;
 #endif
 #define VQ_ASSIGN(T_)                                                 \
-    if (x_bf16) launch_assign_t<T_, __bf16>(g, st);                   \
+    if (row_type == VQ_ROWS_S3) launch_assign_t<T_, S3Row>(g, st);    \
+    else if (row_type) launch_assign_t<T_, __bf16>(g, st);            \
     else launch_assign_t<T_, float>(g, st)
     switch (T) {
         case 8: VQ_ASSIGN(8); break;
diff --git a/vq_seg_amd/csrc/vq_filter.hip b/vq_seg_amd/csrc/vq_filter.hip
--- a/vq_seg_amd/csrc/vq_filter.hip
+++ b/vq_seg_amd/csrc/vq_filter.hip
@@ -30,8 +30,10 @@
     float c_s, c_r;
 };
 
+template <bool S3>
 __global__ __launch_bounds__(256, 2) void vq_filter_bf16_kernel(const VqFilterGroup g, const FilterConsts fc0, const FilterConsts fc1,
                                                                 const FilterConsts fc2, const FilterConsts fc3) {
+    constexpr int NH = S3 ? 2 : 1;
     int lvl = 0;
     while (lvl + 1 < g.n && blockIdx.x >= g.lv[lvl].wg_end) ++lvl;
     const unsigned bid = blockIdx.x - (lvl ? g.lv[lvl - 1].wg_end : 0u);
@@ -63,7 +65,7 @@
     for (int p = 0; p < 2; ++p) {
         long row = row_tile * F_ROWS + wp * 64 + p * 32 + r;
         if (row > N - 1) row = N - 1;
-        xrow[p] = x + row * (long)C + 8 * h;
+        xrow[p] = x + row * (long)(NH * C) + 8 * h;
     }
 
     f32x16 acc[2][4];
@@ -86,21 +88,25 @@
             glds16b(src, dst + (hlslab * F_CODES + quarter * 64) * 16);
         }
     };
-    auto load_x = [&](int stage, u32x4 (&xf)[2][2]) {
+    auto load_x = [&](int stage, u32x4 (&xf)[2][2][NH]) {
 #pragma unroll
         for (int p = 0; p < 2; ++p)
 #pragma unroll
-            for (int q = 0; q < 2; ++q) xf[p][q] = *reinterpret_cast<const u32x4*>(xrow[p] + stage * F_BK + q * 16);
+            for (int q = 0; q < 2; ++q)
+#pragma unroll
+                for (int w = 0; w < NH; ++w) xf[p][q][w] = *reinterpret_cast<const u32x4*>(xrow[p] + w * C + stage * F_BK + q * 16);
     };
 
-    u32x4 xcur[2][2], xnxt[2][2];
+    u32x4 xcur[2][2][NH], xnxt[2][2][NH];
     fill(0, 0);
     if (n_stage > 1) fill(1, 1);
     load_x(0, xcur);
 #pragma unroll
     for (int p = 0; p < 2; ++p)
 #pragma unroll
-        for (int q = 0; q < 2; ++q) xnxt[p][q] = u32x4{0u, 0u, 0u, 0u};
+        for (int q = 0; q < 2; ++q)
+#pragma unroll
+            for (int w = 0; w < NH; ++w) xnxt[p][q][w] = u32x4{0u, 0u, 0u, 0u};
     __syncthreads();
 
     const char* a_lane = Bs + ((h * F_CODES) + wc * 128 + r) * 16;
@@ -117,10 +123,14 @@
             }
 #pragma unroll
             for (int p = 0; p < 2; ++p) {
-                const bf16x8 xb = __builtin_bit_cast(bf16x8, xcur[p][q]);
+                const bf16x8 xb = __builtin_bit_cast(bf16x8, xcur[p][q][0]);
 #pragma unroll
                 for (int e = 0; e < 4; ++e) {
-                    const float lo = __builtin_bit_cast(float, xcur[p][q][e] << 16), hi = __builtin_bit_cast(float, xcur[p][q][e] & 0xFFFF0000u);
+                    float lo = __builtin_bit_cast(float, xcur[p][q][0][e] << 16), hi = __builtin_bit_cast(float, xcur[p][q][0][e] & 0xFFFF0000u);
+                    if constexpr (S3) {
+                        lo += __builtin_bit_cast(float, xcur[p][q][NH - 1][e] << 16);
+                        hi += __builtin_bit_cast(float, xcur[p][q][NH - 1][e] & 0xFFFF0000u);
+                    }
                     xn_part[p] = __builtin_fmaf(lo, lo, xn_part[p]);
                     xn_part[p] = __builtin_fmaf(hi, hi, xn_part[p]);
                 }
@@ -129,6 +139,11 @@
                     acc[p][t] = __builtin_amdgcn_mfma_f32_32x32x16_bf16(ah[t], xb, acc[p][t], 0, 0, 0);
                     acc[p][t] = __builtin_amdgcn_mfma_f32_32x32x16_bf16(al[t], xb, acc[p][t], 0, 0, 0);
                 }
+                if constexpr (S3) {
+                    const bf16x8 xl = __builtin_bit_cast(bf16x8, xcur[p][q][NH - 1]);
+#pragma unroll
+                    for (int t = 0; t < 4; ++t) acc[p][t] = __builtin_amdgcn_mfma_f32_32x32x16_bf16(ah[t], xl, acc[p][t], 0, 0, 0);
+                }
             }
         }
         __syncthreads();
@@ -136,7 +151,9 @@
 #pragma unroll
         for (int p = 0; p < 2; ++p)
 #pragma unroll
-            for (int q = 0; q < 2; ++q) xcur[p][q] = xnxt[p][q];
+            for (int q = 0; q < 2; ++q)
+#pragma unroll
+                for (int w = 0; w < NH; ++w) xcur[p][q][w] = xnxt[p][q][w];
     }
 
     const float en_max = *g.lv[lvl].en_max;
@@ -292,16 +309,18 @@
     }
 }
 
+template <bool S3>
 struct RescoreTrip {
-    u32x4 xw[4];
+    u32x4 xw[4][S3 ? 2 : 1];
     f32x4 e0[4], e1[4];
 };
 
-template <bool ROWMAJOR>
-__device__ __forceinline__ void rescore_load(RescoreTrip& t, const unsigned short* xr, const float* er, int c, int Kp) {
+template <bool ROWMAJOR, bool S3>
+__device__ __forceinline__ void rescore_load(RescoreTrip<S3>& t, const unsigned short* xr, const float* er, int c, int Kp, int C) {
 #pragma unroll
     for (int u = 0; u < 4; ++u) {
-        t.xw[u] = *reinterpret_cast<const u32x4*>(xr + c + 8 * u);
+        t.xw[u][0] = *reinterpret_cast<const u32x4*>(xr + c + 8 * u);
+        if constexpr (S3) t.xw[u][1] = *reinterpret_cast<const u32x4*>(xr + C + c + 8 * u);
         if (ROWMAJOR) {
             t.e0[u] = *reinterpret_cast<const f32x4*>(er + c + 8 * u);
             t.e1[u] = *reinterpret_cast<const f32x4*>(er + c + 8 * u + 4);
@@ -312,13 +331,20 @@
     }
 }
 
-__device__ __forceinline__ void rescore_fma(const RescoreTrip& t, float& dot, float& xa, float& xb) {
+template <bool S3>
+__device__ __forceinline__ void rescore_fma(const RescoreTrip<S3>& t, float& dot, float& xa, float& xb) {
 #pragma unroll
     for (int u = 0; u < 4; ++u) {
-        const float xv[8] = {__builtin_bit_cast(float, t.xw[u][0] << 16), __builtin_bit_cast(float, t.xw[u][0] & 0xFFFF0000u),
-                             __builtin_bit_cast(float, t.xw[u][1] << 16), __builtin_bit_cast(float, t.xw[u][1] & 0xFFFF0000u),
-                             __builtin_bit_cast(float, t.xw[u][2] << 16), __builtin_bit_cast(float, t.xw[u][2] & 0xFFFF0000u),
-                             __builtin_bit_cast(float, t.xw[u][3] << 16), __builtin_bit_cast(float, t.xw[u][3] & 0xFFFF0000u)};
+        float xv[8];
+#pragma unroll
+        for (int e = 0; e < 4; ++e) {
+            xv[2 * e] = __builtin_bit_cast(float, t.xw[u][0][e] << 16);
+            xv[2 * e + 1] = __builtin_bit_cast(float, t.xw[u][0][e] & 0xFFFF0000u);
+            if constexpr (S3) {
+                xv[2 * e] += __builtin_bit_cast(float, t.xw[u][1][e] << 16);
+                xv[2 * e + 1] += __builtin_bit_cast(float, t.xw[u][1][e] & 0xFFFF0000u);
+            }
+        }
 #pragma unroll
         for (int e = 0; e < 4; ++e) {
             dot = __builtin_fmaf(xv[e], t.e0[u][e], dot);
@@ -329,7 +355,7 @@
     }
 }
 
-template <bool ROWMAJOR>
+template <bool ROWMAJOR, bool S3>
 __device__ __forceinline__ void rescore_pairs(const VqFilterLevel& L, int list, int tid, int nthreads) {
     int n = L.pair_count[list];
     if (n > L.pair_cap) n = L.pair_cap;
@@ -341,19 +367,19 @@
         const long row = (long)(rc >> 32);
         const unsigned k = (unsigned)(rc & 0xffffffffull);
         if (L.brow[row] == -__builtin_inff()) continue;
-        const unsigned short* xr = x + row * (long)C;
+        const unsigned short* xr = x + row * (long)(S3 ? 2 * C : C);
         const float* er = ROWMAJOR ? L.W + (size_t)k * C : L.E4 + (size_t)k * 4;
         float dot = 0.0f, xa = 0.0f, xb = 0.0f;
-        RescoreTrip t0, t1, t2;
-        rescore_load<ROWMAJOR>(t0, xr, er, 0, Kp);
-        if (C > 32) rescore_load<ROWMAJOR>(t1, xr, er, 32, Kp);
+        RescoreTrip<S3> t0, t1, t2;
+        rescore_load<ROWMAJOR>(t0, xr, er, 0, Kp, C);
+        if (C > 32) rescore_load<ROWMAJOR>(t1, xr, er, 32, Kp, C);
         int c = 0;
         for (; c + 96 <= C; c += 96) {
-            if (c + 64 < C) rescore_load<ROWMAJOR>(t2, xr, er, c + 64, Kp);
+            if (c + 64 < C) rescore_load<ROWMAJOR>(t2, xr, er, c + 64, Kp, C);
             rescore_fma(t0, dot, xa, xb);
-            if (c + 96 < C) rescore_load<ROWMAJOR>(t0, xr, er, c + 96, Kp);
+            if (c + 96 < C) rescore_load<ROWMAJOR>(t0, xr, er, c + 96, Kp, C);
             rescore_fma(t1, dot, xa, xb);
-            if (c + 128 < C) rescore_load<ROWMAJOR>(t1, xr, er, c + 128, Kp);
+            if (c + 128 < C) rescore_load<ROWMAJOR>(t1, xr, er, c + 128, Kp, C);
             rescore_fma(t2, dot, xa, xb);
         }
         if (c < C) {
@@ -366,28 +392,30 @@
     }
 }
 
+template <bool S3>
 __global__ __launch_bounds__(256) void vq_rescore_kernel(const VqFilterGroup g) {
     int lvl = 0;
     while (lvl + 1 < g.n && blockIdx.x >= g.lv[lvl].sblk_end) ++lvl;
     const unsigned first = lvl ? g.lv[lvl - 1].sblk_end : 0u;
     const unsigned b = blockIdx.x - first, per_list = (g.lv[lvl].sblk_end - first) / F_LISTS;
     const int list = (int)(b % F_LISTS), tid = (int)(b / F_LISTS) * 256 + threadIdx.x, nthreads = (int)per_list * 256;
-    if (g.lv[lvl].W) rescore_pairs<true>(g.lv[lvl], list, tid, nthreads);
-    else rescore_pairs<false>(g.lv[lvl], list, tid, nthreads);
-}
-
+    if (g.lv[lvl].W) rescore_pairs<true, S3>(g.lv[lvl], list, tid, nthreads);
+    else rescore_pairs<false, S3>(g.lv[lvl], list, tid, nthreads);
+}
+
+template <bool S3>
 __global__ __launch_bounds__(256) void vq_exact_dist_kernel(const unsigned short* __restrict__ x, const float* __restrict__ E4, int Kp,
                                                             const float* __restrict__ enorm, const long long* __restrict__ idx, long N, int C,
                                                             float* __restrict__ dmin) {
     const long row = (long)blockIdx.x * 256 + threadIdx.x;
     if (row >= N) return;
-    const unsigned short* xr = x + row * (long)C;
+    const unsigned short* xr = x + row * (long)(S3 ? 2 * C : C);
     const long long k = idx[row];
     float dot = 0.0f, xa = 0.0f, xb = 0.0f;
     for (int c = 0; c + 8 <= C; c += 8) {
         float xv[8];
 #pragma unroll
-        for (int e = 0; e < 8; ++e) xv[e] = __builtin_bit_cast(float, (unsigned)xr[c + e] << 16);
+        for (int e = 0; e < 8; ++e) xv[e] = S3 ? s3_elem(xr, C, c + e) : __builtin_bit_cast(float, (unsigned)xr[c + e] << 16);
         const f32x4 e0 = *reinterpret_cast<const f32x4*>(E4 + ((size_t)(c / 4) * Kp + k) * 4);
         const f32x4 e1 = *reinterpret_cast<const f32x4*>(E4 + ((size_t)(c / 4 + 1) * Kp + k) * 4);
 #pragma unroll
@@ -448,26 +476,33 @@
     hipLaunchKernelGGL(vq_enorm_max, dim3(1), dim3(256), 0, st, enorm, K, en_max);
 }
 
-void launch_filter(const VqFilterGroup& fg, int force_all, hipStream_t st) {
+void launch_filter(const VqFilterGroup& fg, int row_type, int force_all, hipStream_t st) {
+    const bool s3 = row_type == VQ_ROWS_S3;
     FilterConsts fc[VQ_MAX_LEVELS] = {};
     for (int q = 0; q < fg.n; ++q) {
         const double u = ldexp(1.0, -24), cc = (double)fg.lv[q].C;
-        const double per_s = 2.0 * (cc * u + ldexp(1.0, -18) + (cc / 8.0) * 17.0 * u);
+        const double per_s = s3 ? 2.0 * (cc * u + u + 2.0 * ldexp(1.0, -16) + (3.0 * cc / 16.0) * 17.0 * u)
+                                : 2.0 * (cc * u + ldexp(1.0, -18) + (cc / 8.0) * 17.0 * u);
         const double tail = 2.0 * ldexp(1.0, -22) + ldexp(1.0, -20);
         fc[q].c_s = (float)(1.25 * (2.0 * per_s + 2.0 * tail));
         fc[q].c_r = (float)(1.25 * tail);
     }
     const VqFilterLevel& last = fg.lv[fg.n - 1];
-    hipLaunchKernelGGL(vq_filter_bf16_kernel, dim3(last.wg_end), dim3(256), (size_t)(2 * F_STAGE_BYTES + F_CODES * sizeof(float)), st, fg, fc[0],
-                       fc[1], fc[2], fc[3]);
+    const size_t lds = (size_t)(2 * F_STAGE_BYTES + F_CODES * sizeof(float));
+    if (s3) hipLaunchKernelGGL(vq_filter_bf16_kernel<true>, dim3(last.wg_end), dim3(256), lds, st, fg, fc[0], fc[1], fc[2], fc[3]);
+    else hipLaunchKernelGGL(vq_filter_bf16_kernel<false>, dim3(last.wg_end), dim3(256), lds, st, fg, fc[0], fc[1], fc[2], fc[3]);
     hipLaunchKernelGGL(vq_resolve_kernel, dim3(last.rblk_end), dim3(256), 0, st, fg, force_all);
-    hipLaunchKernelGGL(vq_rescore_kernel, dim3(last.sblk_end), dim3(256), 0, st, fg);
-}
-
-void launch_exact_dist(const void* x, const float* E4, int Kp, const float* enorm, const int64_t* idx, int64_t N, int C, float* dmin,
-                       hipStream_t st) {
-    hipLaunchKernelGGL(vq_exact_dist_kernel, dim3((unsigned)((N + 255) / 256)), dim3(256), 0, st, static_cast<const unsigned short*>(x), E4, Kp,
-                       enorm, reinterpret_cast<const long long*>(idx), (long)N, C, dmin);
-}
-
-}
+    if (s3) hipLaunchKernelGGL(vq_rescore_kernel<true>, dim3(last.sblk_end), dim3(256), 0, st, fg);
+    else hipLaunchKernelGGL(vq_rescore_kernel<false>, dim3(last.sblk_end), dim3(256), 0, st, fg);
+}
+
+void launch_exact_dist(const void* x, int row_type, const float* E4, int Kp, const float* enorm, const int64_t* idx, int64_t N, int C,
+                       float* dmin, hipStream_t st) {
+    const dim3 grid((unsigned)((N + 255) / 256));
+    const unsigned short* xr = static_cast<const unsigned short*>(x);
+    const long long* ix = reinterpret_cast<const long long*>(idx);
+    if (row_type == VQ_ROWS_S3) hipLaunchKernelGGL(vq_exact_dist_kernel<true>, grid, dim3(256), 0, st, xr, E4, Kp, enorm, ix, (long)N, C, dmin);
+    else hipLaunchKernelGGL(vq_exact_dist_kernel<false>, grid, dim3(256), 0, st, xr, E4, Kp, enorm, ix, (long)N, C, dmin);
+}
+
+}
diff --git a/vq_seg_amd/csrc/vq_host.hip b/vq_seg_amd/csrc/vq_host.hip
--- a/vq_seg_amd/csrc/vq_host.hip
+++ b/vq_seg_amd/csrc/vq_host.hip
@@ -39,12 +39,14 @@
 static int g_vq_bf16_filter = 1;
 static int g_vq_filter_force_all = 0;
 static int g_vq_filter_launches = 0;
+static int g_vq_s3_filter = 1;
 static const Option VQ_OPTIONS[] = {
     {"vq_max_tiles_per_wave", &g_vq_max_tiles, OPT_POW2_FAIL, 1, 8},
     {"vq_fine_split", &g_vq_fine_split, OPT_FLAG},
     {"vq_bf16_filter", &g_vq_bf16_filter, OPT_FLAG},
     {"vq_filter_force_all", &g_vq_filter_force_all, OPT_FLAG},
     {"vq_filter_launches", &g_vq_filter_launches},
+    {"vq_s3_filter", &g_vq_s3_filter, OPT_FLAG},
 };
 
 int vq_set_option(const char* key, int value) { return apply_option(VQ_OPTIONS, key, value); }
@@ -187,7 +189,7 @@
     for (int i = 0; i < n; ++i)
         for (int j = i + 1; j < n; ++j)
             if (C[order[j]] > C[order[i]]) { const int t = order[i]; order[i] = order[j]; order[j] = t; }
-    bool filter = x_bf16 && g_vq_bf16_filter;
+    bool filter = x_bf16 == VQ_ROWS_S3 ? g_vq_s3_filter != 0 : (x_bf16 && g_vq_bf16_filter);
     for (int i = 0; i < n; ++i) filter = filter && filter_shape_ok(C[i], K[i]);
     VqLevel lv[VQ_MAX_LEVELS];
     VqFilterGroup fg;
@@ -233,12 +235,12 @@
     const bool rec = g_prof.enabled && (int)g_prof.shape.size() + n <= g_prof.capacity;
     const size_t slot = g_prof.shape.size();
     if (rec) {
-        for (int i = 0; i < n; ++i) g_prof.shape.push_back({N[i], C[i], K[i], (int)slot, n, filter ? 2 : (x_bf16 ? 1 : 0)});
+        for (int i = 0; i < n; ++i) g_prof.shape.push_back({N[i], C[i], K[i], (int)slot, n, filter ? 2 : (x_bf16 == VQ_ROWS_BF16 ? 1 : 0)});
         (void)hipEventRecord(g_prof.ev[2 * slot], st);
     }
     if (filter) {
         ++g_vq_filter_launches;
-        launch_filter(fg, g_vq_filter_force_all, st);
+        launch_filter(fg, x_bf16, g_vq_filter_force_all, st);
     }
     launch_assign_levels(lv, n, T, x_bf16, st);
     if (rec) (void)hipEventRecord(g_prof.ev[2 * slot + 1], st);
@@ -248,7 +250,7 @@
         launch_unpack_level(i, N, K, plans, ws, idx, dmin, st);
         if (filter && dmin && dmin[i]) {
             const PreparedView pv = prepared_view(prepared[i], C[i], K[i]);
-            launch_exact_dist(x[i], pv.E4, plans[i].Kp, pv.enorm, idx[i], N[i], C[i], dmin[i], st);
+            launch_exact_dist(x[i], x_bf16, pv.E4, plans[i].Kp, pv.enorm, idx[i], N[i], C[i], dmin[i], st);
         }
     }
     return hipGetLastError();
diff --git a/vq_seg_amd/csrc/vq_internal.h b/vq_seg_amd/csrc/vq_internal.h
--- a/vq_seg_amd/csrc/vq_internal.h
+++ b/vq_seg_amd/csrc/vq_internal.h
@@ -1,4 +1,5 @@
 #pragma once
+#include "nn_device.h"
 #include "vq_kernels.h"
 
 namespace vqseg {
@@ -15,6 +16,11 @@
 constexpr int GATHER_ROWS_PER_BLOCK = 16;
 constexpr int KM_RB = 1024;
 constexpr int KM_SEG = 128;
+
+constexpr int VQ_ROWS_F32 = 0, VQ_ROWS_BF16 = 1, VQ_ROWS_S3 = 2;
+__device__ __forceinline__ float s3_elem(const unsigned short* row, int C, int c) {
+    return __builtin_bit_cast(float, (unsigned)row[c] << 16) + __builtin_bit_cast(float, (unsigned)row[C + c] << 16);
+}
 
 struct VqLevel {
     const void* x;
@@ -72,10 +78,10 @@
 };
 PreparedView prepared_view(const void* prepared, int C, int K);
 
-void launch_assign_levels(const VqLevel* lv, int n, int T, int x_bf16, hipStream_t st);
+void launch_assign_levels(const VqLevel* lv, int n, int T, int row_type, hipStream_t st);
 void launch_prepare_filter(const float* W, int K, int C, int Kp, const float* enorm, unsigned short* Eb, float* en_max, hipStream_t st);
-void launch_filter(const VqFilterGroup& fg, int force_all, hipStream_t st);
-void launch_exact_dist(const void* x, const float* E4, int Kp, const float* enorm, const int64_t* idx, int64_t N, int C, float* dmin,
+void launch_filter(const VqFilterGroup& fg, int row_type, int force_all, hipStream_t st);
+void launch_exact_dist(const void* x, int row_type, const float* E4, int Kp, const float* enorm, const int64_t* idx, int64_t N, int C, float* dmin,
                        hipStream_t st);
 void launch_group_init(const VqInitGroup& ig, hipStream_t st);
 void launch_unpack_level(int i, const int64_t* N, const int* K, const VqPlan* plans, char* const* ws, int64_t* const* idx,
diff --git a/vq_seg_amd/csrc/vq_tail.hip b/vq_seg_amd/csrc/vq_tail.hip
--- a/vq_seg_amd/csrc/vq_tail.hip
+++ b/vq_seg_amd/csrc/vq_tail.hip
@@ -80,6 +80,24 @@
         long long k[RG];
 #pragma unroll
         for (int j = 0; j < RG; ++j) k[j] = row0 + j < N ? idx[row0 + j] : 0;
+        if constexpr (__is_same(TA, S3Row)) {
+            for (int v = lane; v < (C >> 3); v += 64) {
+                f32x4 e0[RG], e1[RG];
+#pragma unroll
+                for (int j = 0; j < RG; ++j)
+                    if (row0 + j < N) {
+                        e0[j] = reinterpret_cast<const f32x4*>(W + k[j] * (long)C)[2 * v];
+                        e1[j] = reinterpret_cast<const f32x4*>(W + k[j] * (long)C)[2 * v + 1];
+                    }
+#pragma unroll
+                for (int j = 0; j < RG; ++j)
+                    if (row0 + j < N) {
+                        const float q[8] = {e0[j][0], e0[j][1], e0[j][2], e0[j][3], e1[j][0], e1[j][1], e1[j][2], e1[j][3]};
+                        s3_store8(reinterpret_cast<unsigned short*>(quant) + (row0 + j) * 2L * C, C, 8 * v, q);
+                    }
+            }
+            continue;
+        }
         for (int v = lane; v < c4; v += 64) {
             f32x4 e[RG], xv[RG];
 #pragma unroll
@@ -199,7 +217,10 @@
                          float cw, const VqPlan& p, char* ws, void* quant, float* loss, float* dead, hipStream_t st) {
     int* hist = reinterpret_cast<int*>(ws + p.off_hist);
     float* partial = reinterpret_cast<float*>(ws + p.off_partial);
-    if (bf16)
+    if (bf16 == VQ_ROWS_S3)
+        hipLaunchKernelGGL(vq_gather_kernel<S3Row>, dim3(p.gather_blocks), dim3(256), 0, st, static_cast<const S3Row*>(x), W,
+                           reinterpret_cast<const long long*>(idx), (long)N, C, 0, static_cast<S3Row*>(quant), partial);
+    else if (bf16)
         hipLaunchKernelGGL(vq_gather_kernel<__bf16>, dim3(p.gather_blocks), dim3(256), 0, st, static_cast<const __bf16*>(x), W,
                            reinterpret_cast<const long long*>(idx), (long)N, C, training, static_cast<__bf16*>(quant), partial);
     else
diff --git a/vq_seg_amd/csrc/vqseg_abi.hip b/vq_seg_amd/csrc/vqseg_abi.hip
--- a/vq_seg_amd/csrc/vqseg_abi.hip
+++ b/vq_seg_amd/csrc/vqseg_abi.hip
@@ -100,7 +100,7 @@
 static int vq_assign_any(const void* x, int x_bf16, const float* codebook, const void* prepared, int64_t n, int c, int k,
                          int64_t* idx, float* dmin, void* ws, size_t ws_bytes, void* stream) {
     if (int rc = check_shape(n, c, k)) return rc;
-    if (x_bf16 && c % 8) return fail(VQSEG_EINVAL, "bf16 rows need channels %% 8 == 0");
+    if (x_bf16 && c % 8) return fail(VQSEG_EINVAL, "%s rows need channels %% 8 == 0", x_bf16 == 2 ? "split-3" : "bf16");
     if (!x || !idx || !ws || (!codebook && !prepared)) return fail(VQSEG_EINVAL, "null pointer argument");
     if (!aligned16(x) || !aligned16(ws) || !aligned16(prepared) || !aligned16(codebook))
         return fail(VQSEG_EINVAL, "x, codebook, prepared and workspace must be 16-byte aligned");
@@ -128,6 +128,11 @@
     return vq_assign_any(x, 1, codebook, prepared, n, c, k, idx, dmin, ws, ws_bytes, stream);
 }
 
+int vqseg_vq_assign_s3(const void* x, const float* codebook, const void* prepared, int64_t n, int c, int k,
+                       int64_t* idx, float* dmin, void* ws, size_t ws_bytes, void* stream) {
+    return vq_assign_any(x, 2, codebook, prepared, n, c, k, idx, dmin, ws, ws_bytes, stream);
+}
+
 static int vq_forward_any(const void* x, int bf16, const float* codebook, const void* prepared, int64_t n, int c, int k,
                           int training, float cw, void* quant, int64_t* idx, float* loss, float* dead_pct, float* dmin,
                           void* ws, size_t ws_bytes, void* stream) {
@@ -158,6 +163,8 @@
                            int64_t* const* idx, float* const* loss, float* const* dead_pct, void* const* ws, const size_t* ws_bytes,
                            void* stream) {
     if (n_levels < 1 || n_levels > vqseg::VQ_MAX_LEVELS) return fail(VQSEG_EINVAL, "1 .. %d levels per grouped launch", vqseg::VQ_MAX_LEVELS);
+    if (bf16 < 0 || bf16 > 2) return fail(VQSEG_EINVAL, "row type must be 0 (f32), 1 (bf16) or 2 (split-3), got %d", bf16);
+    if (bf16 == 2 && training) return fail(VQSEG_EINVAL, "split-3 rows are an eval-mode format: training must be 0");
     if (!x || !codebook || !n || !c || !k || !cw || !quant || !idx || !loss || !dead_pct || !ws || !ws_bytes)
         return fail(VQSEG_EINVAL, "null pointer argument");
     vqseg::VqPlan plans[vqseg::VQ_MAX_LEVELS];
@@ -166,7 +173,7 @@
     hipStream_t st = static_cast<hipStream_t>(stream);
     for (int i = 0; i < n_levels; ++i) {
         if (int rc = check_shape(n[i], c[i], k[i])) return rc;
-        if (bf16 && c[i] % 8) return fail(VQSEG_EINVAL, "bf16 rows need channels %% 8 == 0");
+        if (bf16 && c[i] % 8) return fail(VQSEG_EINVAL, "%s rows need channels %% 8 == 0", bf16 == 2 ? "split-3" : "bf16");
         if (!x[i] || !codebook[i] || !quant[i] || !idx[i] || !loss[i] || !dead_pct[i] || !ws[i]) return fail(VQSEG_EINVAL, "null pointer argument");
         if (!aligned16(x[i]) || !aligned16(ws[i]) || !aligned16(codebook[i]) || !aligned16(quant[i]) || (prepared && !aligned16(prepared[i])))
             return fail(VQSEG_EINVAL, "x, codebook, prepared, quant and workspace must be 16-byte aligned");
diff --git a/vq_seg_amd/models/networks/modified_vqunet/net.py b/vq_seg_amd/models/networks/modified_vqunet/net.py
--- a/vq_seg_amd/models/networks/modified_vqunet/net.py
+++ b/vq_seg_amd/models/networks/modified_vqunet/net.py
@@ -56,10 +56,16 @@
         loss = torch.zeros(1, device=feats[0].device)
         usage = []
         levels = [i for i, vq in enumerate(self.codebook) if not isinstance(vq, _IdentityVQ)]
-        for i in levels:
-            if isinstance(feats[i], nnf.S3):
-                feats[i] = feats[i].float()
-        grouped = _quantize_group([self.codebook[i] for i in levels], [feats[i] for i in levels]) if nnf.py_opt("py_vq_group", 1) else None
+        vqs = [self.codebook[i] for i in levels]
+        group = nnf.py_opt("py_vq_group", 1)
+        grouped = None
+        if group and nnf.py_opt("py_vq_s3", 1) and any(isinstance(feats[i], nnf.S3) for i in levels):
+            grouped = _quantize_group(vqs, [feats[i] for i in levels])
+        if grouped is None:
+            for i in levels:
+                if isinstance(feats[i], nnf.S3):
+                    feats[i] = feats[i].float()
+            grouped = _quantize_group(vqs, [feats[i] for i in levels]) if group else None
         grouped = dict(zip(levels, grouped)) if grouped is not None else {}
         for i, vq in enumerate(self.codebook):
             quantize, _idx, commitment, dead = grouped[i] if i in grouped else vq(feats[i])
diff --git a/vq_seg_amd/nnf.py b/vq_seg_amd/nnf.py
--- a/vq_seg_amd/nnf.py
+++ b/vq_seg_amd/nnf.py
@@ -531,6 +531,12 @@
     out = torch.empty((n, h, w, 2 * c), dtype=torch.bfloat16, device=xr.device)
     _launch("vqseg_s3_split_f", xr.device, _f32(xr, "rows", n * h * w * c), n * h * w, c, _T(out, "split-3 rows", bf=2, numel=n * h * w * 2 * c))
     return S3(out, c)
+
+
+def s3_from_rows(rows: torch.Tensor, c: int) -> "S3":
+    if rows.dim() != 4 or rows.dtype != torch.bfloat16 or rows.shape[-1] != 2 * c or not rows.is_contiguous():
+        raise ValueError(f"split-3 rows must be contiguous (N, H, W, {2 * c}) bf16, got {tuple(rows.shape)} {rows.dtype}")
+    return S3(rows, c)
 
 
 def from_s3(x):
diff --git a/vq_seg_amd/vector_quantizer/vq_img.py b/vq_seg_amd/vector_quantizer/vq_img.py
--- a/vq_seg_amd/vector_quantizer/vq_img.py
+++ b/vq_seg_amd/vector_quantizer/vq_img.py
@@ -93,6 +93,8 @@
 def quantize_group(vqs, feats):
     if len(vqs) < 2 or len(vqs) > 4:
         return None
+    if any(isinstance(f, nnf.S3) for f in feats):
+        return _quantize_group_s3(vqs, feats)
     rows = []
     for vq, f in zip(vqs, feats):
         cb = vq.codebook
@@ -119,6 +121,26 @@
         b, c, h, w = f.shape
         quant, idx, loss, dead = flat[4 * i:4 * i + 4]
         outs.append((quant.reshape(b, h, w, c).permute(0, 3, 1, 2), idx.reshape(b, h, w), loss, dead))
+    return outs
+
+
+def _quantize_group_s3(vqs, feats):
+    if not all(isinstance(f, nnf.S3) for f in feats) or torch.is_grad_enabled():
+        return None
+    L = _hip.lib()
+    for vq, f in zip(vqs, feats):
+        cb = vq.codebook
+        b, c, h, w = f.shape
+        if vq.training or cb.ema_update or not f.rows.is_cuda or c != cb.embedding_dim or \
+                not L.vqseg_vq_filter_counter_offset(b * h * w, c, cb.num_embeddings):
+            return None
+    rows = [f.rows.reshape(-1, 2 * f.c) for f in feats]
+    res = _hip.vq_forward_group(rows, [vq.codebook.embedding.weight.detach() for vq in vqs], [vq.codebook.prepared() for vq in vqs],
+                                False, [float(vq.commitment_weight) for vq in vqs], s3=True)
+    outs = []
+    for f, (quant, idx, loss, dead) in zip(feats, res):
+        b, c, h, w = f.shape
+        outs.append((nnf.s3_from_rows(quant.reshape(b, h, w, 2 * c), c), idx.reshape(b, h, w), loss, dead))
     return outs
 
 
```

Measured after the change: 444.5 images/sec (median of 6 runs). 1.2% higher.
